# kaist-ina/BWA-MEME

Measured on AMD Instinct MI355X. Metric: seeding_reads_per_sec, higher is better.
Workload: dtype u64; 1 GPU; learned-index seeding (rounds 1-3 + hit gather), 150 bp SE reads vs 3100 Mbp synthetic genome (fwd+rc suffix array of 6200000000 entries), index and reads resident in HBM; genome_bp=3100000000, sa_entries=6200000000, read_len=150, rmi_leaves_log2=28

## Files before the change

bwa-meme_amd/csrc/meme_common.h:

```cpp
#pragma once
#include <hip/hip_runtime.h>
#include <stdint.h>
#include <stdio.h>
#include <string>
#include <type_traits>
#include <utility>
#include <vector>

#include "meme_hip.h"

typedef uint64_t u64;
typedef int64_t i64;

struct __attribute__((aligned(16))) SaEnt {
    u64 key;
    u64 pos;
};

struct RmiRec {
    double icpt;
    double slope;
    u64 err;
};

struct Rmi32 {
    double icpt;
    double slope;
    u64 err;
    u64 pad;
};

struct DevIndex {
    i64 n = 0;
    const SaEnt* sa = nullptr;
    const u64* pac = nullptr;
    const Rmi32* l2 = nullptr;
    const Rmi32* l1 = nullptr;
    i64 n_l2 = 0, n_l1 = 0;
    int shift = 64;
    const uint8_t* plcp = nullptr;
};

template <bool HOST> struct Buf {
    void* p = nullptr;
    size_t cap = 0;
    Buf() = default;
    Buf(const Buf&) = delete; Buf& operator=(const Buf&) = delete;
    ~Buf() { if (p) (void)(HOST ? hipHostFree(p) : hipFree(p)); }
    template <class T> T* as() const { return (T*)p; }
};
typedef Buf<false> DevBuf;
typedef Buf<true> HostBuf;
static_assert(!std::is_copy_constructible<DevBuf>::value && !std::is_copy_assignable<DevBuf>::value && !std::is_copy_constructible<HostBuf>::value &&
              !std::is_copy_assignable<HostBuf>::value, "a workspace owns its memory: a copy would free it twice");
template <int N> struct Events {
    hipEvent_t e[N] = {};
    Events() = default;
    Events(const Events&) = delete; Events& operator=(const Events&) = delete;
    ~Events() { for (hipEvent_t x : e) if (x) (void)hipEventDestroy(x); }
    hipEvent_t& operator[](int i) { return e[i]; }
    hipError_t ensure() { for (hipEvent_t& x : e) if (!x) { const hipError_t r = hipEventCreate(&x); if (r != hipSuccess) return r; } return hipSuccess; }
};
struct Stream {
    hipStream_t s = nullptr;
    Stream() = default;
    Stream(const Stream&) = delete; Stream& operator=(const Stream&) = delete;
    ~Stream() { if (s) (void)hipStreamDestroy(s); }
    operator hipStream_t() const { return s; }
};

struct Carve {
    unsigned char* base;
    size_t bytes = 0;
    explicit Carve(void* b) : base((unsigned char*)b) {}
    template <class T> T* take(size_t count, size_t align = 1) { bytes = (bytes + align - 1) / align * align; T* q = base ? (T*)(base + bytes) : nullptr; bytes += count * sizeof(T); return q; }
    i64* col(i64 n) { return take<i64>((size_t)n + 1); }
};
struct ContigTab {
    i64* off; int* len; unsigned char* alt; size_t bytes;
    ContigTab(void* base, i64 n) { Carve c(base); off = c.take<i64>(n); len = c.take<int>(n); alt = c.take<unsigned char>(n + 64); bytes = c.bytes; }
};
struct ChainCounts {
    i64 *chain_off, *seed_off, *nch, *nsd; int* tree; unsigned char* fb; unsigned long long* route; size_t bytes;
    ChainCounts(void* base, i64 n) { Carve c(base); chain_off = c.col(n); seed_off = c.col(n); nch = c.col(n); nsd = c.col(n); tree = c.take<int>(n); fb = c.take<unsigned char>(n + 64);
                                     route = c.take<unsigned long long>(8, 16); bytes = c.bytes; }
};
struct ChainLists {
    i64 *list[5], *work[5], *woff[5]; unsigned char* cls; size_t bytes;
    ChainLists(void* base, i64 n) { Carve c(base); for (int k = 0; k < 5; ++k) { list[k] = c.col(n); work[k] = c.col(n); woff[k] = c.col(n); } cls = c.take<unsigned char>(n + 64); bytes = c.bytes; }
};
enum { EXT_L = 0, EXT_R = 1, EXT_B = 2 };
struct ExtCounts {
    i64 *cnt[3], *off[3], *cntS, *offS; size_t bytes;
    ExtCounts(void* base, i64 n) { Carve c(base); for (i64*& q : cnt) q = c.col(n); for (i64*& q : off) q = c.col(n); cntS = c.col(n); offS = c.col(n); bytes = c.bytes; }
    bool adjacent(i64 n) const { return off[1] == off[0] + (n + 1) && off[2] == off[1] + (n + 1); }
};
struct CountScan {
    i64 *cnt, *off; size_t bytes;
    CountScan(void* base, i64 n) { Carve c(base); cnt = c.col(n); off = c.col(n); bytes = c.bytes; }
};
struct ExtRetry {
    meme_seqpair* half[2]; size_t bytes;
    ExtRetry(void* base, i64 nmax) { Carve c(base); for (meme_seqpair*& q : half) q = c.take<meme_seqpair>((size_t)nmax + 1); bytes = c.bytes; }
};
struct ExtRounds {
    int4* state; uint8_t* act; uint8_t* sel; size_t bytes;
    ExtRounds(void* base, i64 n, i64 seeds) { Carve c(base); state = c.take<int4>(n + 1); act = c.take<uint8_t>(n + 1); sel = c.take<uint8_t>(seeds + 64); bytes = c.bytes; }
};
struct GcigCols {
    i64 *zsz, *csz, *zoff, *coff, *ncig, *ooff, *msz, *moff, *psz, *poff, *isdp, *dpoff, *dplist, *is16, *o16, *is32, *o32, *is64, *o64, *bad; size_t bytes;
    GcigCols(void* base, i64 n) { Carve c(base); zsz = c.col(n); csz = c.col(n); zoff = c.col(n); coff = c.col(n); ncig = c.col(n); ooff = c.col(n); msz = c.col(n); moff = c.col(n);
        psz = c.col(n); poff = c.col(n); isdp = c.col(n); dpoff = c.col(n); dplist = c.col(n); is16 = c.col(n); o16 = c.col(n); is32 = c.col(n); o32 = c.col(n); is64 = c.col(n);
        o64 = c.col(n); bad = c.take<i64>(8); bytes = c.bytes; }
};
struct BswSort {
    int *hist, *offs, *cursor, *maxq; unsigned int* tickets; size_t bytes;
    BswSort(void* base, int keys) { Carve c(base); hist = c.take<int>(keys); offs = c.take<int>(keys + 1); cursor = c.take<int>(keys); maxq = c.take<int>(1); tickets = c.take<unsigned int>(30); bytes = c.bytes; }
};
struct MateCounts {
    i64 *cntQ, *cntJ, *cntR, *cntY, *offQ, *offJ, *offR, *offY; size_t bytes;
    MateCounts(void* base, i64 n) { Carve c(base); cntQ = c.col(n); cntJ = c.col(n); cntR = c.col(n); cntY = c.col(n); offQ = c.col(n); offJ = c.col(n); offR = c.col(n); offY = c.col(n); bytes = c.bytes; }
};
struct SamCols {
    i64 *bound, *soff, *len, *toff, *bad; size_t bytes;
    SamCols(void* base, i64 n) { Carve c(base); bound = c.col(n); soff = c.col(n); len = c.col(n); toff = c.col(n); bad = c.take<i64>(8); bytes = c.bytes; }
};
struct ResidentBatch {
    DevBuf reads, read_off, packed, smems, hits, smem_off, hit_off;
    i64 last_seed_reads = 0;
    i64 last_seed_max_len = 0;
    i64 packed_reads = 0;
    int packed_geom[3] = {0, 0, 0};
    bool reads_resident = false;
};
enum { SEED_CTR_SLOT = 0, SEED_CTR_SEARCHES = 1, SEED_CTR_OVERFLOW = 2, SEED_CTR_WINDOWS = 3, SEED_CTR_PROF = 4, SEED_CTR_LANE = 12, SEED_CTR_PEND = 13, SEED_CTR_BLK = 14, SEED_CTR_BLK_OUT = 15,
       SEED_CTR_RS_ROUND = 16, SEED_CTR_RS_STAGE = 24, SEED_CTR_RS_NOINTV = 27, SEED_CTR_RS_WALKED = 28, SEED_CTR_RS_NBPROBE = 29, SEED_CTRS = 32 };
constexpr int RESEED_MAX_ROUNDS = SEED_CTR_RS_STAGE - SEED_CTR_RS_ROUND;
enum { SEED_EV_PACK0, SEED_EV_PACK1, SEED_EV_SEARCH0, SEED_EV_SEARCH1, SEED_EV_RESEED0, SEED_EV_GATHER0, SEED_EV_GATHER1, SEED_EVS };
struct SeedWs {
    DevBuf slots[3], ovf[2];
    DevBuf slot_cnt, slot_hits, slot_loc, counters, pend, blk;
    long long reseed_counts[SEED_CTRS - SEED_CTR_RS_ROUND] = {0};
    int reseed_rounds = 0;
    HostBuf h_smems, h_hits, h_smem_off, h_hit_off;
    unsigned long long* counter_set(int cset) { return (unsigned long long*)counters.p + SEED_CTRS * cset; }
    Events<SEED_EVS> ev;
    Stream emit; Events<2> emit_ev;
};
struct ChainWs {
    DevBuf ch1, sd1, hdr, frac, counts, chains, seeds, lists;
    DevBuf wave[5];
    HostBuf h_chain_off, h_chains, h_seed_off, h_seeds, h_tree, h_frac, h_fallback;
    Events<5> ev;
    const i64* chain_off() const { return (const i64*)counts.p; }
    const i64* seed_off(i64 n) const { return ChainCounts(counts.p, n).seed_off; }
};
enum { EXT_CTR_RETRY = 0, EXT_CTR_FLT_JOBS = 2, EXT_CTR_CENSUS = 8, EXT_CTR_HEAVY = 24, EXT_CTR_BYTES = 256 };
struct ExtWs {
    DevBuf rmax, regs, order, counts, pairs_l, pairs_r, retry, seq, counters;
    DevBuf flt_sc, flt_jobs, flt_cnt, flt_seeds, flt_score, flt_hsp;
    DevBuf live_cnt, live_regs, rounds, heavy;
    HostBuf h_reg_off, h_regs; Events<2> ev;
};
struct BswWs { DevBuf pairs, refb, qerb, order, ws, hist; Events<2> ev; };
struct GcigWs {
    DevBuf jobs, cols, z, cig, res, ops, md, nm, md_packed, cjobs, cres; HostBuf h_res, h_ops, h_md; Events<2> ev;
};
struct KswvWs {
    DevBuf jobs, order, ref, qer, res, rowmax, rm_off; HostBuf h_res; Events<2> ev;
};
struct MateWs {
    DevBuf regs, reg_off, counts, gar, aux, batch_off; HostBuf h_gar, h_batch_off, h_jobs;
};
struct SamWs {
    DevBuf names, name_off, quals, recs, blob, cols, scratch, text, contigs; HostBuf h_text_off, h_text; Events<2> ev;
};

struct PrimaryWs {
    DevBuf regs, reg_off, out, n_pri, mapq, status, sorted, rank, list, counter, logtab; HostBuf h_regs, h_n_pri, h_mapq, h_status; Events<2> ev;
    bool log_ready = false;
};

struct PairWs {
    DevBuf regs, reg_off, n_pri, res, status, counter, keys, list, tab; HostBuf h_res, h_status, h_tab; Events<2> ev; Events<1> tab_ev;
    bool tab_in_flight = false;
};

struct FinishWs {
    DevBuf regs, reg_off, out, reg_off_out, ums, status, counters, stage, cnt, live, first, list, cols_l, cols_c;
    HostBuf h_regs, h_reg_off, h_ums, h_status; Events<2> ev;
};

struct ContigCache {
    DevBuf dev; HostBuf host;
    std::vector<meme_contig> from; i64 l_pac = -1;
};

struct SideStreams {
    Stream st[3];
    Events<3> done;
    Events<1> fork;
};

struct meme_ctx {
    int device = 0;
    int n_cus = 256;
    DevIndex idx;
    bool owns_index = false;
    std::vector<std::pair<void*, size_t>> owned;
    void* plcp_aux = nullptr;
    ResidentBatch batch;
    DevBuf scan_tmp;
    ContigCache contigs;
    HostBuf h_ctr;
    ChainWs chain; ExtWs ext; BswWs bsw; GcigWs gcig; KswvWs kswv; MateWs mate; SamWs sam; PrimaryWs primary; PairWs pair; FinishWs finish; SeedWs seed;
    Stream stream;
    SideStreams side;
    i64 seed_blocks = 0;
    i64 helper_blocks = 0;
    i64 smem_cap = 128;
    i64 group_lanes = 4;
    i64 seed_blocks_per_cu = 5;
    i64 max_batch = 0;
    i64 ext_slab_jobs = 8 << 20;
    i64 ext_slab_bytes = (i64)3 << 29;
    i64 ext_split = 1;
    i64 bsw_circ = 1;
    i64 sam_max_batch = 0;
    i64 primary_split = 8;
    i64 primary_blocks = 0;
    i64 pair_split = 8;
    i64 pair_blocks = 0;
    i64 pair_lds_keys = 0;
    i64 finish_blocks = 0;
    i64 finish_lds_recs = 0;
    i64 ext_live_only = 0;
    i64 ext_rounds = 1;
    i64 gcig_groups = 1;
    i64 gcig_zcap = -1;
    i64 ext_census = 0;
    i64 seed_defer = 1;
    i64 chain_light_hits = 32;
    i64 chain_lane_hits = 256;
    i64 chain_wave_tiers = 1;
    i64 sa_chunk = (i64)1 << 28;
    i64 sa_piece = (i64)1 << 28;
    i64 bsw_blocks = 0;
    i64 bsw_lane_min_pairs = 32768;
    bool sa_stats_valid = false;
    long long sa_stats[MEME_SA_STATS] = {0};
    i64 sam_text_reads = 0;
    bool sam_has_quals = false;
    meme_timings tm = {};
};

void meme_set_error(const char* fmt, ...);
int meme_buf_reserve(meme_ctx* ctx, DevBuf& b, size_t bytes);
int meme_side_stream(meme_ctx* ctx, int i);
int meme_hostbuf_reserve(meme_ctx* ctx, HostBuf& b, size_t bytes);
inline unsigned grid_blocks(i64 items, int per, i64 cap = 256 * 64) { i64 b = (items + per - 1) / per; return (unsigned)(b < cap ? (b < 1 ? 1 : b) : cap); }
int meme_contigs(meme_ctx* ctx, const char* prefix, const meme_contig* contigs, int32_t n_contigs, i64 l_pac, ContigTab* out);
int meme_scan_exclusive(meme_ctx* ctx, const i64* d_in, i64* d_out, i64 n);
int meme_scan_total(meme_ctx* ctx, const i64* d_in, i64* d_out, i64 n, i64* h_total);
inline bool meme_fits_free_hbm(size_t need, size_t have, size_t* free_b) { size_t total_b = 0; return need <= have || hipMemGetInfo(free_b, &total_b) != hipSuccess || need <= *free_b / 2 + have; }
int meme_bsw_launch(meme_ctx* ctx, meme_seqpair* d_pairs, const uint8_t* d_ref, const uint8_t* d_qer, int npairs, int w, const meme_bsw_opt* opt,
                    int host_maxq);
hipError_t meme_bsw_last_ms(meme_ctx* ctx, float* ms);
constexpr int MEME_SEEDSW_MAX = 200;
struct meme_seedsw_job { i64 rb; i64 qoff; int seed; short tlen, qlen; };
int meme_seedsw_launch(meme_ctx* ctx, const meme_seedsw_job* d_jobs, const unsigned long long* d_njobs, i64 max_jobs, int* d_sc, const meme_ext_opt* o);
int meme_kswv_run(meme_ctx* ctx, const meme_kswv_job* jobs, int64_t njobs, const uint8_t* ref, int64_t ref_bytes, const uint8_t* qer, int64_t qer_bytes, const meme_bsw_opt* opt,
                  bool staged, meme_kswv_host_result* out);
int meme_chain_reserve(meme_ctx* ctx, i64 n);
int meme_chain_run(meme_ctx* ctx, const meme_contig* contigs, int32_t n_contigs, const meme_chain_opt* opt, i64* totals);

#define HIP_TRY(expr)                                                                          \
    do {                                                                                       \
        hipError_t _e = (expr);                                                                \
        if (_e != hipSuccess) {                                                                \
            meme_set_error("%s failed: %s (%s:%d)", #expr, hipGetErrorString(_e), __FILE__, __LINE__); \
            return MEME_E_HIP;                                                                 \
        }                                                                                      \
    } while (0)

__device__ __forceinline__ u64 load_pos5(const uint8_t* pos5, i64 i) {
    const i64 bo = i * 5;
    const uint32_t* pd = reinterpret_cast<const uint32_t*>(pos5 + (bo & ~3ll));
    const u64 two = (u64)pd[0] | ((u64)pd[1] << 32);
    const u64 v5 = (two >> (8 * (int)(bo & 3))) & 0xffffffffffull;
    return ((v5 & 0xffffffffull) << 8) | (v5 >> 32);
}
__device__ __forceinline__ int text_base(const u64* pac, i64 p) { return (int)(pac[p >> 5] >> (62 - 2 * (int)(p & 31))) & 3; }
__device__ __forceinline__ u64 extract32(const u64* w, i64 s) {
    i64 k = s >> 5;
    int sh = (int)(s & 31) * 2;
    u64 a = w[k], b = w[k + 1];
    return sh ? (a << sh) | (b >> (64 - sh)) : a;
}
```

bwa-meme_amd/csrc/meme_ctx.hip:

```cpp
#include <fcntl.h>
#include <stdarg.h>
#include <stdlib.h>
#include <string.h>
#include <sys/stat.h>
#include <unistd.h>
#include <atomic>
#include <chrono>
#include <functional>
#include <thread>

#include "meme_common.h"

static thread_local char g_err[512] = "";

void meme_set_error(const char* fmt, ...) {
    va_list ap;
    va_start(ap, fmt);
    vsnprintf(g_err, sizeof(g_err), fmt, ap);
    va_end(ap);
}

extern "C" const char* meme_last_error(void) { return g_err; }

int meme_buf_reserve(meme_ctx* ctx, DevBuf& b, size_t bytes) {
    if (bytes <= b.cap) return MEME_OK;
    if (b.p) { HIP_TRY(hipStreamSynchronize(ctx->stream)); HIP_TRY(hipFree(b.p)); b.p = nullptr; b.cap = 0; }
    size_t want = bytes + bytes / 4 + 256;
    HIP_TRY(hipMalloc(&b.p, want));
    b.cap = want;
    return MEME_OK;
}

int meme_side_stream(meme_ctx* ctx, int i) {
    SideStreams& S = ctx->side;
    if (!S.st[i].s) HIP_TRY(hipStreamCreateWithFlags(&S.st[i].s, hipStreamNonBlocking));
    if (!S.done[i]) HIP_TRY(hipEventCreateWithFlags(&S.done[i], hipEventDisableTiming));
    if (!S.fork[0]) HIP_TRY(hipEventCreateWithFlags(&S.fork[0], hipEventDisableTiming));
    return MEME_OK;
}

int meme_hostbuf_reserve(meme_ctx* ctx, HostBuf& b, size_t bytes) {
    if (bytes <= b.cap) return MEME_OK;
    if (b.p) { HIP_TRY(hipStreamSynchronize(ctx->stream)); HIP_TRY(hipHostFree(b.p)); b.p = nullptr; b.cap = 0; }
    size_t want = bytes + bytes / 4 + 4096;
    HIP_TRY(hipHostMalloc(&b.p, want, hipHostMallocDefault));
    b.cap = want;
    return MEME_OK;
}

extern "C" void* meme_host_alloc(int64_t bytes) {
    void* p = nullptr;
    if (bytes <= 0) return nullptr;
    if (hipHostMalloc(&p, (size_t)bytes, hipHostMallocDefault) != hipSuccess) { meme_set_error("hipHostMalloc(%lld) failed", (long long)bytes); return nullptr; }
    return p;
}
extern "C" void meme_host_free(void* p) { if (p) (void)hipHostFree(p); }

extern "C" int meme_device_count(void) {
    int n = 0;
    if (hipGetDeviceCount(&n) != hipSuccess) return 0;
    return n;
}


extern "C" meme_ctx* meme_ctx_create(int device) {
    int n = meme_device_count();
    if (n <= 0) { meme_set_error("no HIP device visible: the MI355X backend has no CPU fallback"); return nullptr; }
    if (device < 0 || device >= n) { meme_set_error("device %d out of range (0..%d)", device, n - 1); return nullptr; }
    if (hipSetDevice(device) != hipSuccess) { meme_set_error("hipSetDevice(%d) failed", device); return nullptr; }
    meme_ctx* ctx = new meme_ctx();
    ctx->device = device;
    { hipDeviceProp_t prop; if (hipGetDeviceProperties(&prop, device) == hipSuccess && prop.multiProcessorCount > 0) ctx->n_cus = prop.multiProcessorCount; }
    if (hipStreamCreateWithFlags(&ctx->stream.s, hipStreamNonBlocking) != hipSuccess) {
        meme_set_error("hipStreamCreate failed");
        delete ctx;
        return nullptr;
    }
    return ctx;
}

extern "C" void meme_ctx_destroy(meme_ctx* ctx) {
    if (!ctx) return;
    (void)hipSetDevice(ctx->device);
    for (hipStream_t st : {ctx->stream.s, ctx->side.st[0].s, ctx->side.st[1].s, ctx->side.st[2].s, ctx->seed.emit.s})
        if (st) (void)hipStreamSynchronize(st);
    if (ctx->owns_index) for (auto& o : ctx->owned) (void)hipFree(o.first);
    if (ctx->plcp_aux) (void)hipFree(ctx->plcp_aux);
    delete ctx;
}

int meme_contigs(meme_ctx* ctx, const char* prefix, const meme_contig* contigs, int32_t n_contigs, i64 l_pac, ContigTab* out) {
    ContigCache& K = ctx->contigs;
    if (K.dev.p && K.l_pac == l_pac && (i64)K.from.size() == n_contigs && (n_contigs == 0 || !memcmp(K.from.data(), contigs, (size_t)n_contigs * sizeof(meme_contig)))) {
        *out = ContigTab(K.dev.p, n_contigs);
        return MEME_OK;
    }
    HIP_TRY(hipStreamSynchronize(ctx->stream));
    K.l_pac = -1;
    for (int i = 0; i < n_contigs; ++i)
        if (contigs[i].len < 1 || contigs[i].offset < 0 || contigs[i].offset + contigs[i].len > l_pac || (i > 0 && contigs[i].offset < contigs[i - 1].offset + contigs[i - 1].len)) {
            meme_set_error("%scontig %d (offset %lld, length %d) is not a valid reference sequence of a %lld-base genome", prefix, i, (long long)contigs[i].offset, contigs[i].len,
                           (long long)l_pac);
            return MEME_E_ARG;
        }
    const size_t bytes = ContigTab(nullptr, n_contigs).bytes;
    int rc;
    if ((rc = meme_buf_reserve(ctx, K.dev, bytes)) || (rc = meme_hostbuf_reserve(ctx, K.host, bytes))) return rc;
    memset(K.host.p, 0, bytes);
    const ContigTab t(K.host.p, n_contigs);
    for (int i = 0; i < n_contigs; ++i) { t.off[i] = contigs[i].offset; t.len[i] = contigs[i].len; t.alt[i] = contigs[i].is_alt ? 1 : 0; }
    HIP_TRY(hipMemcpyAsync(K.dev.p, K.host.p, bytes, hipMemcpyHostToDevice, ctx->stream));
    HIP_TRY(hipStreamSynchronize(ctx->stream));
    K.from.assign(contigs, contigs + n_contigs);
    K.l_pac = l_pac;
    *out = ContigTab(K.dev.p, n_contigs);
    return MEME_OK;
}

extern "C" int meme_ctx_sync(meme_ctx* ctx) {
    if (!ctx) return MEME_E_ARG;
    HIP_TRY(hipStreamSynchronize(ctx->stream));
    return MEME_OK;
}

extern "C" void* meme_ctx_stream(meme_ctx* ctx) { return ctx ? (void*)ctx->stream : nullptr; }

extern "C" int meme_get_timings(meme_ctx* ctx, meme_timings* out) {
    if (!ctx || !out) return MEME_E_ARG;
    *out = ctx->tm;
    return MEME_OK;
}

extern "C" int meme_set_tuning(meme_ctx* ctx, const char* key, int64_t value) {
    if (!ctx || !key) return MEME_E_ARG;
    if (!strcmp(key, "gcig_groups") && value != 0 && value != 1) { meme_set_error("gcig_groups must be 0 or 1"); return MEME_E_ARG; }
    if (!strcmp(key, "group_lanes") && value != 1 && value != 2 && value != 4 && value != 8 && value != 16 && value != 32) { meme_set_error("group_lanes must be 1, 2, 4, 8, 16 or 32"); return MEME_E_ARG; }
    const i64 any = INT64_MIN;
    static const struct { const char* key; i64 meme_ctx::*member; i64 at_least; } keys[] = {
        {"seed_blocks", &meme_ctx::seed_blocks, any}, {"helper_blocks", &meme_ctx::helper_blocks, 0}, {"smem_cap", &meme_ctx::smem_cap, 8}, {"seed_defer", &meme_ctx::seed_defer, any}, {"max_batch", &meme_ctx::max_batch, any},
        {"sam_max_batch", &meme_ctx::sam_max_batch, any}, {"bsw_circ", &meme_ctx::bsw_circ, any}, {"ext_split", &meme_ctx::ext_split, any}, {"ext_slab_jobs", &meme_ctx::ext_slab_jobs, 1},
        {"ext_census", &meme_ctx::ext_census, any}, {"gcig_zcap", &meme_ctx::gcig_zcap, any}, {"gcig_groups", &meme_ctx::gcig_groups, any}, {"ext_live_only", &meme_ctx::ext_live_only, any},
        {"ext_rounds", &meme_ctx::ext_rounds, 0}, {"bsw_blocks", &meme_ctx::bsw_blocks, any}, {"bsw_lane_min_pairs", &meme_ctx::bsw_lane_min_pairs, any},
        {"chain_wave_tiers", &meme_ctx::chain_wave_tiers, any}, {"chain_lane_hits", &meme_ctx::chain_lane_hits, any}, {"chain_light_hits", &meme_ctx::chain_light_hits, any},
        {"group_lanes", &meme_ctx::group_lanes, any}, {"primary_split", &meme_ctx::primary_split, 0}, {"primary_blocks", &meme_ctx::primary_blocks, 0}, {"finish_blocks", &meme_ctx::finish_blocks, 0}, {"pair_split", &meme_ctx::pair_split, 0}, {"pair_blocks", &meme_ctx::pair_blocks, 0}, {"pair_lds_keys", &meme_ctx::pair_lds_keys, 0},
        {"finish_lds_recs", &meme_ctx::finish_lds_recs, 0}, {"seed_blocks_per_cu", &meme_ctx::seed_blocks_per_cu, 1},
        {"sa_chunk", &meme_ctx::sa_chunk, 1}, {"sa_piece", &meme_ctx::sa_piece, 1}};
    for (const auto& k : keys) if (!strcmp(key, k.key)) { ctx->*k.member = value < k.at_least ? k.at_least : value; return MEME_OK; }
    meme_set_error("unknown tuning key %s", key);
    return MEME_E_ARG;
}

extern "C" int meme_index_share(meme_ctx* ctx, meme_ctx* owner);
extern "C" int64_t meme_index_pac64_words(int64_t sa_num) { return ((sa_num + 31) >> 5) + 8; }
extern "C" int64_t meme_index_pos5_bytes(int64_t sa_num) { return sa_num * 5 + 16; }

__global__ void __launch_bounds__(256) k_pack_text(const uint8_t* __restrict__ text, i64 n, u64* __restrict__ pac, i64 words) {
  for (i64 w = (i64)blockIdx.x * blockDim.x + threadIdx.x; w < words; w += (i64)gridDim.x * blockDim.x) {
    i64 base = w << 5;
    u64 v = 0;
    if (base + 32 <= n) {
        const uint4* p = reinterpret_cast<const uint4*>(text + base);
        uint4 a = p[0], b = p[1];
        uint32_t q[8] = {a.x, a.y, a.z, a.w, b.x, b.y, b.z, b.w};
#pragma unroll
        for (int k = 0; k < 8; ++k) {
            uint32_t x = q[k];
            v = (v << 8) | ((u64)(x & 3) << 6) | ((u64)((x >> 8) & 3) << 4) | ((u64)((x >> 16) & 3) << 2) |
                (u64)((x >> 24) & 3);
        }
    } else {
        for (int r = 0; r < 32; ++r) {
            i64 p = base + r;
            u64 c = p < n ? (u64)(text[p] & 3) : 3ull;
            v = (v << 2) | c;
        }
    }
    pac[w] = v;
  }
}

__global__ void __launch_bounds__(256) k_build_entries(const uint8_t* __restrict__ pos_packed, const u64* __restrict__ sa_u64,
                                                        i64 n, const u64* __restrict__ pac, SaEnt* __restrict__ ent) {
  for (i64 i = (i64)blockIdx.x * blockDim.x + threadIdx.x; i < n; i += (i64)gridDim.x * blockDim.x) {
    const u64 pos = sa_u64 ? sa_u64[i] : load_pos5(pos_packed, i);
    SaEnt e;
    e.key = extract32(pac, (i64)pos);
    e.pos = pos;
    ent[i] = e;
  }
}

__global__ void __launch_bounds__(256) k_pos5_from_sa(const u64* __restrict__ sa, i64 n, uint8_t* __restrict__ pos5) {
  for (i64 i = (i64)blockIdx.x * blockDim.x + threadIdx.x; i < n; i += (i64)gridDim.x * blockDim.x) {
    const u64 pos = sa[i];
    uint8_t* p = pos5 + i * 5;
    const uint32_t hi = (uint32_t)(pos >> 8);
    p[0] = (uint8_t)hi; p[1] = (uint8_t)(hi >> 8); p[2] = (uint8_t)(hi >> 16); p[3] = (uint8_t)(hi >> 24); p[4] = (uint8_t)(pos & 0xff);
  }
}

__global__ void __launch_bounds__(256) k_rmi32(const RmiRec* __restrict__ in, i64 n, Rmi32* __restrict__ out) {
  for (i64 i = (i64)blockIdx.x * blockDim.x + threadIdx.x; i < n; i += (i64)gridDim.x * blockDim.x) {
    const RmiRec r = in[i];
    Rmi32 o;
    o.icpt = r.icpt; o.slope = r.slope; o.err = r.err; o.pad = 0;
    out[i] = o;
  }
}

__device__ __forceinline__ int pair_lcp(const SaEnt a, const SaEnt b, i64 n, const u64* __restrict__ pac) {
    i64 lim = n - (i64)(a.pos > b.pos ? a.pos : b.pos);
    if (lim > 255) lim = 255;
    const u64 x = a.key ^ b.key;
    int l = x ? (__clzll((long long)x) >> 1) : 32;
    if (!x) {
        for (int m = 1; l < lim; ++m) {
            const u64 y = extract32(pac, (i64)a.pos + 32 * m) ^ extract32(pac, (i64)b.pos + 32 * m);
            if (y) { l += __clzll((long long)y) >> 1; break; }
            l += 32;
        }
    }
    return l < (int)lim ? l : (int)lim;
}

__global__ void __launch_bounds__(256) k_build_plcp(const SaEnt* __restrict__ ent, i64 n, const u64* __restrict__ pac, uint8_t* __restrict__ plcp) {
    __shared__ int sl[257];
    for (i64 b0 = (i64)blockIdx.x * 256; b0 < n; b0 += (i64)gridDim.x * 256) {
        const i64 i = b0 + threadIdx.x;
        SaEnt e; e.key = 0; e.pos = 0;
        int ln = 0;
        if (i < n) {
            e = ent[i];
            if (i + 1 < n) ln = pair_lcp(e, ent[i + 1], n, pac);
        }
        sl[threadIdx.x + 1] = ln;
        if (threadIdx.x == 0) sl[0] = b0 > 0 ? pair_lcp(ent[b0 - 1], e, n, pac) : 0;
        __syncthreads();
        if (i < n) {
            const int a = sl[threadIdx.x], b = sl[threadIdx.x + 1];
            plcp[e.pos] = (uint8_t)(a > b ? a : b);
        }
        __syncthreads();
    }
}

extern "C" int meme_stage_build_plcp(meme_ctx* ctx, const void* d_sa_ent, int64_t n, const void* d_pac64, void* d_plcp) {
    if (!ctx || !d_sa_ent || !d_pac64 || !d_plcp || n <= 0) return MEME_E_ARG;
    HIP_TRY(hipSetDevice(ctx->device));
    hipLaunchKernelGGL(k_build_plcp, dim3(grid_blocks(n, 256)), dim3(256), 0, ctx->stream, (const SaEnt*)d_sa_ent, (i64)n, (const u64*)d_pac64,
                       (uint8_t*)d_plcp);
    HIP_TRY(hipGetLastError());
    return MEME_OK;
}

extern "C" int meme_stage_pack_text(meme_ctx* ctx, const uint8_t* d_text, int64_t n, void* d_pac64) {
    if (!ctx || !d_text || !d_pac64 || n <= 0) return MEME_E_ARG;
    HIP_TRY(hipSetDevice(ctx->device));
    i64 words = meme_index_pac64_words(n);
    hipLaunchKernelGGL(k_pack_text, dim3(grid_blocks(words, 256)), dim3(256), 0, ctx->stream, d_text, n,
                       (u64*)d_pac64, words);
    HIP_TRY(hipGetLastError());
    return MEME_OK;
}

extern "C" int meme_stage_build_entries(meme_ctx* ctx, const uint8_t* d_pos_packed, int64_t n, const void* d_pac64,
                                        void* d_sa_ent) {
    if (!ctx || !d_pos_packed || !d_pac64 || !d_sa_ent || n <= 0) return MEME_E_ARG;
    HIP_TRY(hipSetDevice(ctx->device));
    hipLaunchKernelGGL(k_build_entries, dim3(grid_blocks(n, 256)), dim3(256), 0, ctx->stream, d_pos_packed,
                       (const u64*)nullptr, (i64)n, (const u64*)d_pac64, (SaEnt*)d_sa_ent);
    HIP_TRY(hipGetLastError());
    return MEME_OK;
}

extern "C" int meme_stage_entries_from_sa(meme_ctx* ctx, const uint64_t* d_sa, int64_t n, const void* d_pac64,
                                          void* d_sa_ent) {
    if (!ctx || !d_sa || !d_pac64 || !d_sa_ent || n <= 0) return MEME_E_ARG;
    HIP_TRY(hipSetDevice(ctx->device));
    hipLaunchKernelGGL(k_build_entries, dim3(grid_blocks(n, 256)), dim3(256), 0, ctx->stream,
                       (const uint8_t*)nullptr, (const u64*)d_sa, (i64)n, (const u64*)d_pac64, (SaEnt*)d_sa_ent);
    HIP_TRY(hipGetLastError());
    return MEME_OK;
}

extern "C" int meme_stage_pos5_from_sa(meme_ctx* ctx, const uint64_t* d_sa, int64_t n, void* d_pos5) {
    if (!ctx || !d_sa || !d_pos5 || n <= 0) return MEME_E_ARG;
    HIP_TRY(hipSetDevice(ctx->device));
    hipLaunchKernelGGL(k_pos5_from_sa, dim3(grid_blocks(n, 256)), dim3(256), 0, ctx->stream, (const u64*)d_sa, (i64)n, (uint8_t*)d_pos5);
    HIP_TRY(hipGetLastError());
    return MEME_OK;
}

// ... 308 lines not shown
```

bwa-meme_amd/csrc/meme_seed.hip:

```cpp
#include <limits.h>
#include <stdlib.h>
#include <string.h>
#include <utility>

#include "meme_seed_kernel.h"

namespace {

using namespace seedk;

constexpr int SCAN_BLOCK = 256;
constexpr int SCAN_ITEMS = 4;
constexpr int SCAN_TILE = SCAN_BLOCK * SCAN_ITEMS;

__device__ __forceinline__ i64 block_scan_excl(i64 v, i64* total) {
    __shared__ i64 wsum[SCAN_BLOCK / 64];
    const int lane = threadIdx.x & 63, wid = threadIdx.x >> 6;
    i64 x = v;
#pragma unroll
    for (int d = 1; d < 64; d <<= 1) {
        i64 y = __shfl_up(x, d);
        if (lane >= d) x += y;
    }
    if (lane == 63) wsum[wid] = x;
    __syncthreads();
    i64 off = 0, tot = 0;
    for (int w = 0; w < SCAN_BLOCK / 64; ++w) {
        if (w < wid) off += wsum[w];
        tot += wsum[w];
    }
    __syncthreads();
    *total = tot;
    return off + x - v;
}

__global__ void __launch_bounds__(SCAN_BLOCK) k_tile_sums(const int* __restrict__ cnt, const i64* __restrict__ hits, i64 n,
                                                          i64 ntiles, i64* __restrict__ tile_sums) {
  for (i64 tile = blockIdx.x; tile < ntiles; tile += gridDim.x) {
    i64 base = tile * SCAN_TILE + threadIdx.x * SCAN_ITEMS;
    i64 a = 0, b = 0;
    for (int k = 0; k < SCAN_ITEMS; ++k) {
        i64 i = base + k;
        if (i < n) {
            int c = cnt[i];
            a += c < 0 ? 0 : c;
            b += hits[i];
        }
    }
    i64 ta, tb;
    block_scan_excl(a, &ta);
    block_scan_excl(b, &tb);
    if (threadIdx.x == 0) { tile_sums[2 * tile] = ta; tile_sums[2 * tile + 1] = tb; }
  }
}

__global__ void __launch_bounds__(SCAN_BLOCK) k_scan_tiles(i64* __restrict__ tile_sums, i64 ntiles, i64* __restrict__ totals) {
    i64 ca = 0, cb = 0;
    for (i64 base = 0; base < ntiles; base += SCAN_BLOCK) {
        i64 i = base + threadIdx.x;
        i64 a = i < ntiles ? tile_sums[2 * i] : 0, b = i < ntiles ? tile_sums[2 * i + 1] : 0;
        i64 ta, tb;
        i64 ea = block_scan_excl(a, &ta);
        i64 eb = block_scan_excl(b, &tb);
        if (i < ntiles) { tile_sums[2 * i] = ca + ea; tile_sums[2 * i + 1] = cb + eb; }
        ca += ta;
        cb += tb;
    }
    if (threadIdx.x == 0) { totals[0] = ca; totals[1] = cb; }
}

__global__ void __launch_bounds__(SCAN_BLOCK) k_offsets(const int* __restrict__ cnt, const i64* __restrict__ hits, i64 n,
                                                        i64 ntiles, const i64* __restrict__ tile_sums, i64* __restrict__ smem_off,
                                                        i64* __restrict__ hit_off) {
  for (i64 tile = blockIdx.x; tile < ntiles; tile += gridDim.x) {
    i64 base = tile * SCAN_TILE + threadIdx.x * SCAN_ITEMS;
    i64 va[SCAN_ITEMS], vb[SCAN_ITEMS], a = 0, b = 0;
    for (int k = 0; k < SCAN_ITEMS; ++k) {
        i64 i = base + k;
        va[k] = vb[k] = 0;
        if (i < n) {
            int c = cnt[i];
            va[k] = c < 0 ? 0 : c;
            vb[k] = hits[i];
        }
        a += va[k];
        b += vb[k];
    }
    i64 ta, tb;
    i64 ea = block_scan_excl(a, &ta) + tile_sums[2 * tile];
    i64 eb = block_scan_excl(b, &tb) + tile_sums[2 * tile + 1];
    for (int k = 0; k < SCAN_ITEMS; ++k) {
        i64 i = base + k;
        if (i < n) { smem_off[i] = ea; hit_off[i] = eb; }
        ea += va[k];
        eb += vb[k];
    }
    if (tile == ntiles - 1 && threadIdx.x == SCAN_BLOCK - 1) { smem_off[n] = ea; hit_off[n] = eb; }
  }
}

struct TierTable {
    const SlotRec* base[N_TIERS];
    int cap[N_TIERS];
};

__global__ void __launch_bounds__(BLOCK) k_gather(const SaEnt* __restrict__ sa, TierTable tiers, const i64* __restrict__ slot_loc,
                                                   const int* __restrict__ cnt, i64 n, int hits_per_smem,
                                                   const i64* __restrict__ smem_off, const i64* __restrict__ hit_off,
                                                   meme_mem_tl* __restrict__ smems, u64* __restrict__ hits) {
    constexpr int GL = 16;
    const int lane = threadIdx.x & 63;
    const int t = lane & (GL - 1);
    const int gbase = lane - t;
    i64 gid = ((i64)blockIdx.x * BLOCK + threadIdx.x) / GL;
    const i64 ngroups = (i64)gridDim.x * BLOCK / GL;
    for (i64 r = gid; r < n; r += ngroups) {
        const int c = cnt[r];
        if (c <= 0) continue;
        const i64 loc = slot_loc[r];
        const int tier = (int)(loc >> 40);
        const SlotRec* sl = tiers.base[tier] + (loc & ((1ll << 40) - 1)) * tiers.cap[tier];
        meme_mem_tl* out = smems + smem_off[r];
        u64* hout = hits + hit_off[r];
        i64 hb0 = 0;
        for (int k0 = 0; k0 < c; k0 += GL) {
            const int k = k0 + t;
            const bool act = k < c;
            SlotRec s;
            s.start = s.end = 0; s.sa_start = 0; s.count = 0;
            if (act) s = sl[k];
            i64 h = s.count;
            if (hits_per_smem > 0 && h > hits_per_smem) h = hits_per_smem;
            i64 incl = h;
#pragma unroll
            for (int d = 1; d < GL; d <<= 1) {
                i64 y = __shfl_up(incl, d, GL);
                if (t >= d) incl += y;
            }
            const i64 hb = hb0 + incl - h;
            u64 first = 0;
            if (act) {
                first = (s.sa_start & SLOT_POS) ? (u64)(s.sa_start & SLOT_VAL) : sa[s.sa_start].pos;
                meme_mem_tl m;
                m.start = s.start;
                m.end = s.end;
                m.hitbeg = (int32_t)hb;
                m.hitcount = s.count > (i64)INT_MAX ? INT_MAX : (int32_t)s.count;
                m.cache_refpos = first;
                out[k] = m;
                if (h > 0) hout[hb] = first;
                for (i64 i = 1; i < h && i < 4; ++i) hout[hb + i] = sa[s.sa_start + i].pos;
            }
            u64 longmask = (__ballot(act && h > 4) >> gbase) & 0xffffull;
            while (longmask) {
                const int src = __ffsll((long long)longmask) - 1;
                longmask &= longmask - 1;
                const i64 lh = __shfl(h, src, GL), lhb = __shfl(hb, src, GL), lsa = __shfl(s.sa_start, src, GL);
                for (i64 i = 4 + t; i < lh; i += GL) hout[lhb + i] = sa[lsa + i].pos;
            }
            hb0 += __shfl(incl, GL - 1, GL);
        }
    }
}

template <int G>
int launch_k_seed(hipStream_t stream, const SeedArgs& A, size_t lds, i64 blocks) {
    if (lds > 64 * 1024)
        HIP_TRY(hipFuncSetAttribute((const void*)k_seed<G>, hipFuncAttributeMaxDynamicSharedMemorySize, (int)lds));
    hipLaunchKernelGGL(k_seed<G>, dim3((unsigned)blocks), dim3(BLOCK), lds, stream, A);
    HIP_TRY(hipGetLastError());
    return MEME_OK;
}

struct SeedRun {
    meme_ctx* ctx;
    const i64* d_read_off; i64 nreads;
    const meme_seed_opt* opt;
    PackGeom geo;
    TierTable tiers = {};
    bool defer = false;
    i64 n_early = -1;
    i64 n_todo = 0;
    float ms_total = 0.f, ms_reseed = 0.f;
    i64 launches = 0, searches = 0, windows = 0, lane_searches = 0;
    unsigned long long h_early[SEED_CTRS];
};

i64 helper_grid(const meme_ctx* ctx, i64 blocks) {
    if (ctx->helper_blocks > 0 && blocks > ctx->helper_blocks) blocks = ctx->helper_blocks;
    return blocks < 1 ? 1 : blocks;
}
template <typename K>
int resident_grid(const meme_ctx* ctx, K kernel, int threads, i64* blocks) {
    int per_cu = 0;
    HIP_TRY(hipOccupancyMaxActiveBlocksPerMultiprocessor(&per_cu, kernel, threads, 0));
    *blocks = (i64)ctx->n_cus * (per_cu < 1 ? 1 : per_cu);
    return MEME_OK;
}

int seed_pack(SeedRun& R, const uint8_t* d_reads, i64 max_len, i64 total_bytes) {
    meme_ctx* ctx = R.ctx;
    if (max_len > MAX_READ_LEN) {
        meme_set_error("read of %lld bases exceeds the learned-index limit of %d (LEARNED_MAX_READ_LEN)", (long long)max_len, MAX_READ_LEN);
        return MEME_E_ARG;
    }
    if (max_len < 1) max_len = 1;
    PackGeom& geo = R.geo;
    geo.W = (int)((max_len + 31) / 32) + 2;
    geo.MW = (int)((max_len + 63) / 64);
    geo.stride = 2 * geo.W + 2 * geo.MW + 1;
    int rc;
    if ((rc = meme_buf_reserve(ctx, ctx->batch.packed, (size_t)R.nreads * geo.stride * 8))) return rc;
    HIP_TRY(hipEventRecord(ctx->seed.ev[SEED_EV_PACK0], ctx->stream));
    const int rw = pack_chunk_reads(max_len);
    const i64 nchunks = (R.nreads + rw - 1) / rw;
    i64 pblocks = (nchunks + 3) / 4, pmax = 0;
    if ((rc = resident_grid(ctx, k_pack_reads, 256, &pmax))) return rc;
    pblocks = helper_grid(ctx, pblocks > pmax ? pmax : pblocks);
    hipLaunchKernelGGL(k_pack_reads, dim3((unsigned)pblocks), dim3(256), 0, ctx->stream, d_reads,
                       R.d_read_off, R.nreads, total_bytes, geo, rw, (u64*)ctx->batch.packed.p);
    HIP_TRY(hipGetLastError());
    HIP_TRY(hipEventRecord(ctx->seed.ev[SEED_EV_PACK1], ctx->stream));
    ctx->batch.packed_reads = R.nreads;
    ctx->batch.packed_geom[0] = geo.W; ctx->batch.packed_geom[1] = geo.MW; ctx->batch.packed_geom[2] = geo.stride;
    return MEME_OK;
}

int launch_tier(SeedRun& R, int tier, i64 n_todo, const i64* pending, int cset, hipStream_t stream, bool defer) {
    meme_ctx* ctx = R.ctx;
    int G = tier == 0 ? (int)ctx->group_lanes : 32;
    const int cap = tier == 0 ? (int)ctx->smem_cap : TIER_CAP[tier];
    const int lcap = cap < TIER_LCAP[tier] ? cap : TIER_LCAP[tier];
    DevBuf& sb = ctx->seed.slots[tier];
    DevBuf& ob = ctx->seed.ovf[tier & 1];
    const size_t need = (size_t)n_todo * cap * sizeof(SlotRec);
    if (tier > 0 && need > sb.cap) {
        size_t free_b = 0;
        if (!meme_fits_free_hbm(need, 0, &free_b)) {
            meme_set_error("%lld reads emitted more than %d SMEMs each: re-running them needs %.1f GB of slots, more than half of the "
                           "free HBM (%.1f GB); seed this batch in smaller pieces", (long long)n_todo, R.tiers.cap[tier - 1],
                           need / 1e9, free_b / 1e9);
            return MEME_E_CAPACITY;
        }
    }
    int rc;
    if ((rc = meme_buf_reserve(ctx, sb, need))) return rc;
    if ((rc = meme_buf_reserve(ctx, ob, (size_t)n_todo * sizeof(i64)))) return rc;
    unsigned long long* counters = ctx->seed.counter_set(cset);
    HIP_TRY(hipMemsetAsync(counters, 0, SEED_CTRS * sizeof(unsigned long long), stream));
    SeedArgs A;
    A.I = ctx->idx;
    A.packed = (const u64*)ctx->batch.packed.p;
    A.read_off = R.d_read_off;
    A.nreads = n_todo;
    A.geo = R.geo;
    A.opt = *R.opt;
    A.slots = (SlotRec*)sb.p;
    A.slot_cnt = (int*)ctx->seed.slot_cnt.p;
    A.slot_hits = (i64*)ctx->seed.slot_hits.p;
    A.slot_loc = (i64*)ctx->seed.slot_loc.p;
    A.pending = pending;
    A.ovf_list = (i64*)ob.p;
    A.cap = cap;
    A.lcap = lcap;
    A.tier = tier;
    A.counters = counters;
    A.defer = defer ? 1 : 0;
    R.tiers.base[tier] = (const SlotRec*)sb.p;
    R.tiers.cap[tier] = cap;
    while (G < 32 && seed_lds_bytes(G, R.geo, lcap) > (size_t)160 * 1024) G *= 2;
    const int groups = BLOCK / G;
    size_t lds = seed_lds_bytes(G, R.geo, lcap);
    i64 want = (n_todo + groups - 1) / groups;
    i64 blocks = ctx->seed_blocks > 0 ? ctx->seed_blocks : (i64)ctx->n_cus * ctx->seed_blocks_per_cu;
    if (blocks > want) blocks = want;
    if (blocks < 1) blocks = 1;
    if (tier == 0) HIP_TRY(hipEventRecord(ctx->seed.ev[SEED_EV_SEARCH0], stream));
    switch (G) {
    case 1: return launch_k_seed<1>(stream, A, lds, blocks);
    case 2: return launch_k_seed<2>(stream, A, lds, blocks);
    case 4: return launch_k_seed<4>(stream, A, lds, blocks);
    case 8: return launch_k_seed<8>(stream, A, lds, blocks);
    case 16: return launch_k_seed<16>(stream, A, lds, blocks);
    case 32: return launch_k_seed<32>(stream, A, lds, blocks);
    default: meme_set_error("group_lanes must be 1, 2, 4, 8, 16 or 32"); return MEME_E_ARG;
    }
}

int fetch_counters(SeedRun& R, int cset, unsigned long long* h, int nsets = 1) {
    HIP_TRY(hipMemcpyAsync(h, R.ctx->seed.counter_set(cset), (size_t)nsets * SEED_CTRS * sizeof(unsigned long long), hipMemcpyDeviceToHost, R.ctx->stream));
    HIP_TRY(hipStreamSynchronize(R.ctx->stream));
    return MEME_OK;
}
void tally(SeedRun& R, const unsigned long long* h) {
    ++R.launches;
    R.searches += (i64)h[SEED_CTR_SEARCHES];
    R.windows += (i64)h[SEED_CTR_WINDOWS];
    R.n_todo = (i64)h[SEED_CTR_OVERFLOW];
#ifdef SEED_PROF
    {
        double tot = 0; for (int k = 0; k < 8; ++k) tot += (double)h[SEED_CTR_PROF + k];
        fprintf(stderr, "[seed prof]:");
        const char* nm[6] = {"control", "request+rmi", "window+compare", "resolve", "level", "apply"};
        for (int k = 0; k < 6; ++k) fprintf(stderr, " %s %.1f%%", nm[k], 100.0 * (double)h[SEED_CTR_PROF + k] / (tot > 0 ? tot : 1));
        fprintf(stderr, "\n");
    }
#endif
}

#ifndef RESEED_ROUNDS
#define RESEED_ROUNDS 5
#endif
#ifndef RESEED_EMIT_BESIDE
#define RESEED_EMIT_BESIDE 1
#endif
int launch_reseed(SeedRun& R) {
    meme_ctx* ctx = R.ctx;
    SeedWs& S = ctx->seed;
    const i64 nreads = R.nreads;
    HIP_TRY(hipEventRecord(S.ev[SEED_EV_RESEED0], ctx->stream));
    ReseedArgs A;
    A.I = ctx->idx; A.packed = (const u64*)ctx->batch.packed.p; A.geo = R.geo; A.nreads = nreads; A.opt = *R.opt;
    A.slots = (SlotRec*)S.slots[0].p; A.cap = (int)ctx->smem_cap; A.slot_cnt = (int*)S.slot_cnt.p; A.slot_hits = (i64*)S.slot_hits.p;
    A.ovf_list = (i64*)S.ovf[0].p; A.counters = S.counter_set(0); A.pend_list = (i64*)S.pend.p;
    A.blk = (BlkRec*)S.blk.p; A.blk_out = A.blk + nreads * BLK_PER_READ; A.blk_cap = nreads * BLK_PER_READ;
    A.blk_ctr = SEED_CTR_BLK; A.blk_out_ctr = SEED_CTR_BLK_OUT;
    A.read_off = R.d_read_off; A.round = 0;
    i64 rblocks = (nreads + 255) / 256;
    if (rblocks > (i64)ctx->n_cus * 32) rblocks = (i64)ctx->n_cus * 32;
    hipLaunchKernelGGL(k_reseed, dim3((unsigned)rblocks), dim3(256), 0, ctx->stream, A);
    HIP_TRY(hipEventRecord(ctx->side.fork[0], ctx->stream));
    const unsigned sblocks = (unsigned)(rblocks < (i64)ctx->n_cus * 4 ? rblocks : (i64)ctx->n_cus * 4);
    if (!S.emit.s) HIP_TRY(hipStreamCreateWithFlags(&S.emit.s, hipStreamNonBlocking));
    for (int i = 0; i < 2; ++i) if (!S.emit_ev[i]) HIP_TRY(hipEventCreateWithFlags(&S.emit_ev[i], hipEventDisableTiming));
    if (RESEED_EMIT_BESIDE) {
        HIP_TRY(hipEventRecord(S.emit_ev[0], ctx->stream));
        HIP_TRY(hipStreamWaitEvent(S.emit, S.emit_ev[0], 0));
        hipLaunchKernelGGL(k_reseed_emit, dim3(sblocks), dim3(256), 0, S.emit, A);
        HIP_TRY(hipEventRecord(S.emit_ev[1], S.emit));
    }
    constexpr int ROUNDS = RESEED_ROUNDS;
    static_assert(ROUNDS >= 1 && ROUNDS <= RESEED_MAX_ROUNDS, "one counter per round");
    S.reseed_rounds = ROUNDS;
    for (int round = 0; round < ROUNDS; ++round) {
        A.round = round;
        hipLaunchKernelGGL(k_reseed_search, dim3(sblocks), dim3(256), 0, ctx->stream, A);
        if (round < ROUNDS - 1) {
            hipLaunchKernelGGL(k_reseed_resume<false>, dim3(sblocks), dim3(256), 0, ctx->stream, A);
            HIP_TRY(hipMemsetAsync(S.counter_set(0) + A.blk_ctr, 0, sizeof(unsigned long long), ctx->stream));
            std::swap(A.blk, A.blk_out); std::swap(A.blk_ctr, A.blk_out_ctr);
        } else hipLaunchKernelGGL(k_reseed_resume<true>, dim3(sblocks), dim3(256), 0, ctx->stream, A);
    }
    if (!RESEED_EMIT_BESIDE) {
        hipLaunchKernelGGL(k_reseed_emit, dim3(sblocks), dim3(256), 0, ctx->stream, A);
        HIP_TRY(hipEventRecord(S.emit_ev[1], ctx->stream));
    }
    HIP_TRY(hipGetLastError());
    return MEME_OK;
}

int launch_early_overflow(SeedRun& R) {
    meme_ctx* ctx = R.ctx;
    Stream& side = ctx->side.st[0];
    unsigned long long h_ovf = 0;
    HIP_TRY(hipStreamWaitEvent(side, ctx->side.fork[0], 0));
    HIP_TRY(hipMemcpyAsync(&h_ovf, ctx->seed.counter_set(0) + SEED_CTR_OVERFLOW, 8, hipMemcpyDeviceToHost, side));
    HIP_TRY(hipStreamSynchronize(side));
    if (h_ovf == 0) return MEME_OK;
    R.n_early = (i64)h_ovf;
    int rc;
    if ((rc = launch_tier(R, 1, R.n_early, (const i64*)ctx->seed.ovf[0].p, 1, side, false))) return rc;
    HIP_TRY(hipEventRecord(ctx->side.done[0], side));
    HIP_TRY(hipStreamWaitEvent(ctx->stream, ctx->side.done[0], 0));
    return MEME_OK;
}

int seed_tier0(SeedRun& R) {
    meme_ctx* ctx = R.ctx;
    SeedWs& S = ctx->seed;
    int rc;
    R.defer = ctx->seed_defer != 0 && ctx->idx.plcp != nullptr && R.opt->rounds >= 2;
    S.reseed_rounds = 0;
    if (R.defer && (rc = meme_buf_reserve(ctx, S.pend, (size_t)R.nreads * sizeof(i64)))) return rc;
    if (R.defer && (rc = meme_buf_reserve(ctx, S.blk, (size_t)R.nreads * BLK_PER_READ * 2 * sizeof(BlkRec)))) return rc;
    if ((rc = launch_tier(R, 0, R.nreads, nullptr, 0, ctx->stream, R.defer))) return rc;
    if (R.defer) {
        if ((rc = meme_side_stream(ctx, 0)) || (rc = launch_reseed(R)) || (rc = launch_early_overflow(R))) return rc;
        HIP_TRY(hipStreamWaitEvent(ctx->stream, S.emit_ev[1], 0));
    }
    HIP_TRY(hipEventRecord(S.ev[SEED_EV_SEARCH1], ctx->stream));
    unsigned long long h[2 * SEED_CTRS];
    if ((rc = fetch_counters(R, 0, h, R.n_early >= 0 ? 2 : 1))) return rc;
    if (R.n_early >= 0) memcpy(R.h_early, h + SEED_CTRS, sizeof(R.h_early));
    float ms = 0.f;
    HIP_TRY(hipEventElapsedTime(&ms, S.ev[SEED_EV_SEARCH0], S.ev[SEED_EV_SEARCH1]));
    R.ms_total += ms;
    if (R.defer) {
        float a = 0.f;
        HIP_TRY(hipEventElapsedTime(&a, S.ev[SEED_EV_RESEED0], S.ev[SEED_EV_SEARCH1]));
        R.ms_reseed += a;
        R.lane_searches += (i64)h[SEED_CTR_LANE];
        for (int k = SEED_CTR_RS_ROUND; k < SEED_CTRS; ++k) S.reseed_counts[k - SEED_CTR_RS_ROUND] = (long long)h[k];
#ifdef RESEED_PROF
        {
            const unsigned long long* c = h + SEED_CTR_PROF;
            fprintf(stderr, "[reseed prof] lists per round:");
            for (int k = 0; k < S.reseed_rounds; ++k) fprintf(stderr, " %llu", h[SEED_CTR_RS_ROUND + k]);
            fprintf(stderr, "\n[reseed prof] stage searches partition_probes run_probes\n");
            for (int k = 0; k < 3; ++k) fprintf(stderr, "[reseed prof] %d %llu %llu %llu\n", k, h[SEED_CTR_RS_STAGE + k], c[k], c[3 + k]);
            fprintf(stderr, "[reseed prof] interval read %llu, without interval %llu, walked %llu, neighbour probes %llu, last-pass searches %llu\n", c[6],
                    h[SEED_CTR_RS_NOINTV], h[SEED_CTR_RS_WALKED], h[SEED_CTR_RS_NBPROBE], h[SEED_CTR_LANE]);
        }
#endif
        if (getenv("MEME_SEED_TRACE")) fprintf(stderr, "[meme] seed tier 0: search kernel + re-seeding kernels %.2f ms, of which behind k_seed %.2f ms (%lld lane searches; %lld reads of the "
                                               "overflow tier beside them)\n", ms, a, (long long)h[SEED_CTR_LANE], (long long)(R.n_early < 0 ? 0 : R.n_early));
    }
    tally(R, h);
    return MEME_OK;
}

int seed_overflow_tiers(SeedRun& R) {
    meme_ctx* ctx = R.ctx;
    SeedWs& S = ctx->seed;
    int rc;
    unsigned long long h[SEED_CTRS];
    for (int tier = 1; R.n_todo > 0; ++tier) {
        if (tier >= N_TIERS) {
            meme_set_error("a read produced more than %d SMEMs", TIER_CAP[N_TIERS - 1]);
            return MEME_E_CAPACITY;
        }
        const int cset = tier & 1;
        if (tier == 1 && R.n_early == R.n_todo) {
            memcpy(h, R.h_early, sizeof(h));
        } else {
            HIP_TRY(hipEventRecord(S.ev[SEED_EV_SEARCH0], ctx->stream));
            if ((rc = launch_tier(R, tier, R.n_todo, (const i64*)S.ovf[(tier - 1) & 1].p, cset, ctx->stream, false))) return rc;
            HIP_TRY(hipEventRecord(S.ev[SEED_EV_SEARCH1], ctx->stream));
            if ((rc = fetch_counters(R, cset, h))) return rc;
            float ms = 0.f;
            HIP_TRY(hipEventElapsedTime(&ms, S.ev[SEED_EV_SEARCH0], S.ev[SEED_EV_SEARCH1]));
            R.ms_total += ms;
        }
        tally(R, h);
    }
    return MEME_OK;
}

int seed_gather(SeedRun& R, meme_seed_result* out) {
    meme_ctx* ctx = R.ctx;
    SeedWs& S = ctx->seed;
    ResidentBatch& B = ctx->batch;
    const i64 nreads = R.nreads;
    int rc;
    i64 ntiles = (nreads + SCAN_TILE - 1) / SCAN_TILE;
    if ((rc = meme_buf_reserve(ctx, ctx->scan_tmp, (size_t)(2 * ntiles + 2) * sizeof(i64)))) return rc;
    if ((rc = meme_buf_reserve(ctx, B.smem_off, (size_t)(nreads + 1) * sizeof(i64)))) return rc;
    if ((rc = meme_buf_reserve(ctx, B.hit_off, (size_t)(nreads + 1) * sizeof(i64)))) return rc;
    i64* tiles = (i64*)ctx->scan_tmp.p;
    i64* totals = tiles + 2 * ntiles;
    HIP_TRY(hipEventRecord(S.ev[SEED_EV_GATHER0], ctx->stream));
    const i64 sblocks = helper_grid(ctx, ntiles);
    hipLaunchKernelGGL(k_tile_sums, dim3((unsigned)sblocks), dim3(SCAN_BLOCK), 0, ctx->stream, (const int*)S.slot_cnt.p,
                       (const i64*)S.slot_hits.p, nreads, ntiles, tiles);
    hipLaunchKernelGGL(k_scan_tiles, dim3(1), dim3(SCAN_BLOCK), 0, ctx->stream, tiles, ntiles, totals);
    hipLaunchKernelGGL(k_offsets, dim3((unsigned)sblocks), dim3(SCAN_BLOCK), 0, ctx->stream, (const int*)S.slot_cnt.p,
                       (const i64*)S.slot_hits.p, nreads, ntiles, (const i64*)tiles, (i64*)B.smem_off.p, (i64*)B.hit_off.p);
    HIP_TRY(hipGetLastError());
    i64 h_tot[2];
    HIP_TRY(hipMemcpyAsync(h_tot, totals, sizeof(h_tot), hipMemcpyDeviceToHost, ctx->stream));
    HIP_TRY(hipStreamSynchronize(ctx->stream));
    if ((rc = meme_buf_reserve(ctx, B.smems, (size_t)(h_tot[0] + 1) * sizeof(meme_mem_tl)))) return rc;
    if ((rc = meme_buf_reserve(ctx, B.hits, (size_t)(h_tot[1] + 1) * sizeof(u64)))) return rc;
    i64 gblocks = (nreads + 15) / 16;
    if (gblocks > (i64)ctx->n_cus * 8) gblocks = (i64)ctx->n_cus * 8;
    gblocks = helper_grid(ctx, gblocks);
    hipLaunchKernelGGL(k_gather, dim3((unsigned)gblocks), dim3(BLOCK), 0, ctx->stream, ctx->idx.sa, R.tiers,
                       (const i64*)S.slot_loc.p, (const int*)S.slot_cnt.p, nreads, R.opt->hits_per_smem,
                       (const i64*)B.smem_off.p, (const i64*)B.hit_off.p, (meme_mem_tl*)B.smems.p, (u64*)B.hits.p);
    HIP_TRY(hipGetLastError());
    HIP_TRY(hipEventRecord(S.ev[SEED_EV_GATHER1], ctx->stream));
    HIP_TRY(hipStreamSynchronize(ctx->stream));
    HIP_TRY(hipEventElapsedTime(&ctx->tm.seed_gather_ms, S.ev[SEED_EV_GATHER0], S.ev[SEED_EV_GATHER1]));
    out->d_smems = (const meme_mem_tl*)B.smems.p;
    out->d_smem_off = (const i64*)B.smem_off.p;
    out->d_hits = (const u64*)B.hits.p;
    out->d_hit_off = (const i64*)B.hit_off.p;
    out->total_smems = h_tot[0];
    out->total_hits = h_tot[1];
    out->searches = R.searches;
    return MEME_OK;
}

int launch_seed(meme_ctx* ctx, const uint8_t* d_reads, const i64* d_read_off, i64 nreads, i64 max_len, i64 total_bytes,
                const meme_seed_opt* opt, meme_seed_result* out) {
    int rc;
    SeedWs& S = ctx->seed;
    ctx->batch.last_seed_reads = 0;
    ctx->sam_text_reads = 0;
    if ((rc = meme_buf_reserve(ctx, S.slot_cnt, (size_t)nreads * sizeof(int)))) return rc;
    if ((rc = meme_buf_reserve(ctx, S.slot_hits, (size_t)nreads * sizeof(i64)))) return rc;
    if ((rc = meme_buf_reserve(ctx, S.slot_loc, (size_t)nreads * sizeof(i64)))) return rc;
    if ((rc = meme_buf_reserve(ctx, S.counters, 2 * SEED_CTRS * sizeof(unsigned long long)))) return rc;
    HIP_TRY(S.ev.ensure());
    SeedRun R;
    R.ctx = ctx; R.d_read_off = d_read_off; R.nreads = nreads; R.opt = opt;
    if ((rc = seed_pack(R, d_reads, max_len, total_bytes)) || (rc = seed_tier0(R)) || (rc = seed_overflow_tiers(R))) return rc;
    HIP_TRY(hipEventElapsedTime(&ctx->tm.seed_pack_ms, S.ev[SEED_EV_PACK0], S.ev[SEED_EV_PACK1]));
    ctx->tm.seed_kernel_ms = R.ms_total;
    ctx->tm.seed_launches = R.launches;
    ctx->tm.seed_windows = R.windows;
    ctx->tm.seed_reseed_ms = R.ms_reseed;
    ctx->tm.seed_lane_searches = R.lane_searches;
    return seed_gather(R, out);
}

__global__ void __launch_bounds__(256) k_max_len(const i64* __restrict__ off, i64 n, int* out) {
    __shared__ int wmax[4];
    int v = 0;
    for (i64 i = (i64)blockIdx.x * blockDim.x + threadIdx.x; i < n; i += (i64)gridDim.x * blockDim.x) {
        int l = (int)(off[i + 1] - off[i]);
        v = v > l ? v : l;
    }
    for (int d = 32; d >= 1; d >>= 1) { int y = __shfl_xor(v, d); v = v > y ? v : y; }
    if ((threadIdx.x & 63) == 0) wmax[threadIdx.x >> 6] = v;
    __syncthreads();
    if (threadIdx.x == 0) {
        for (int k = 1; k < 4; ++k) v = v > wmax[k] ? v : wmax[k];
        atomicMax(out, v);
    }
}

int device_max_len(meme_ctx* ctx, const i64* d_read_off, i64 nreads, i64* max_len) {
    int rc;
    if ((rc = meme_buf_reserve(ctx, ctx->scan_tmp, 64))) return rc;
    HIP_TRY(hipMemsetAsync(ctx->scan_tmp.p, 0, 4, ctx->stream));
    i64 mblocks = (nreads + 255) / 256;
    if (mblocks > 1024) mblocks = 1024;
    hipLaunchKernelGGL(k_max_len, dim3((unsigned)mblocks), dim3(256), 0, ctx->stream, d_read_off, nreads,
                       (int*)ctx->scan_tmp.p);
    int v = 0;
    HIP_TRY(hipMemcpyAsync(&v, ctx->scan_tmp.p, 4, hipMemcpyDeviceToHost, ctx->stream));
    HIP_TRY(hipStreamSynchronize(ctx->stream));
    *max_len = v;
    return MEME_OK;
}

int check_opt(const meme_seed_opt* opt) {
    if (!opt || opt->min_seed_len < 1 || opt->rounds < 1 || opt->rounds > 3 || opt->hits_per_smem < 0) {
        meme_set_error("bad meme_seed_opt");
        return MEME_E_ARG;
    }
    return MEME_OK;
}

}

extern "C" int meme_seed_batch_device(meme_ctx* ctx, const uint8_t* d_reads, const int64_t* d_read_off, int64_t nreads,
                                      int64_t total_bases, const meme_seed_opt* opt, meme_seed_result* out) {
    if (!ctx || !d_reads || !d_read_off || !out || nreads < 0) return MEME_E_ARG;
    int rc = check_opt(opt);
    if (rc) return rc;
    if (!ctx->idx.sa) { meme_set_error("meme_seed_batch: no index loaded"); return MEME_E_STATE; }
    HIP_TRY(hipSetDevice(ctx->device));
    if (nreads == 0) { memset(out, 0, sizeof(*out)); return MEME_OK; }
    i64 max_len = 0;
    if ((rc = device_max_len(ctx, (const i64*)d_read_off, nreads, &max_len))) return rc;
    return launch_seed(ctx, d_reads, (const i64*)d_read_off, nreads, max_len, total_bases, opt, out);
}

extern "C" int meme_seed_batch(meme_ctx* ctx, const uint8_t* reads, const int64_t* read_off, int64_t nreads,
                               const meme_seed_opt* opt, meme_mem_tl* smems, int64_t smem_capacity, int64_t* smem_off,
                               uint64_t* hits, int64_t hit_capacity, int64_t* hit_off, int64_t* total_smems,
                               int64_t* total_hits) {
    if (!ctx || !reads || !read_off || !smems || !smem_off || !hits || !hit_off || nreads < 0) return MEME_E_ARG;
    int rc = check_opt(opt);
    if (rc) return rc;
    if (!ctx->idx.sa) { meme_set_error("meme_seed_batch: no index loaded"); return MEME_E_STATE; }
    HIP_TRY(hipSetDevice(ctx->device));
    if (nreads == 0) { smem_off[0] = 0; hit_off[0] = 0; if (total_smems) *total_smems = 0; if (total_hits) *total_hits = 0; return MEME_OK; }
    const i64 bases = read_off[nreads] - read_off[0];
    if (read_off[0] != 0) { meme_set_error("read_off[0] must be 0"); return MEME_E_ARG; }
    if ((rc = meme_buf_reserve(ctx, ctx->batch.reads, (size_t)bases + 16))) return rc;
    if ((rc = meme_buf_reserve(ctx, ctx->batch.read_off, (size_t)(nreads + 1) * sizeof(i64)))) return rc;
    HIP_TRY(hipMemcpyAsync(ctx->batch.reads.p, reads, (size_t)bases, hipMemcpyHostToDevice, ctx->stream));
    HIP_TRY(hipMemcpyAsync(ctx->batch.read_off.p, read_off, (size_t)(nreads + 1) * sizeof(i64), hipMemcpyHostToDevice, ctx->stream));
    meme_seed_result res;
    i64 max_len = 0;
    for (i64 i = 0; i < nreads; ++i) max_len = read_off[i + 1] - read_off[i] > max_len ? read_off[i + 1] - read_off[i] : max_len;
    rc = launch_seed(ctx, (const uint8_t*)ctx->batch.reads.p, (const i64*)ctx->batch.read_off.p, nreads, max_len, bases, opt, &res);
    if (rc) return rc;
    if (total_smems) *total_smems = res.total_smems;
    if (total_hits) *total_hits = res.total_hits;
    HIP_TRY(hipMemcpyAsync(smem_off, res.d_smem_off, (size_t)(nreads + 1) * sizeof(i64), hipMemcpyDeviceToHost, ctx->stream));
    HIP_TRY(hipMemcpyAsync(hit_off, res.d_hit_off, (size_t)(nreads + 1) * sizeof(i64), hipMemcpyDeviceToHost, ctx->stream));
    if (res.total_smems > smem_capacity || res.total_hits > hit_capacity) {
        HIP_TRY(hipStreamSynchronize(ctx->stream));
        meme_set_error("output buffers too small: need %lld SMEMs and %lld hits", (long long)res.total_smems,
                       (long long)res.total_hits);
        return MEME_E_CAPACITY;
    }
    HIP_TRY(hipMemcpyAsync(smems, res.d_smems, (size_t)res.total_smems * sizeof(meme_mem_tl), hipMemcpyDeviceToHost, ctx->stream));
    HIP_TRY(hipMemcpyAsync(hits, res.d_hits, (size_t)res.total_hits * sizeof(u64), hipMemcpyDeviceToHost, ctx->stream));
    HIP_TRY(hipStreamSynchronize(ctx->stream));
    return MEME_OK;
}

extern "C" int meme_debug_packed_reads(meme_ctx* ctx, uint64_t* out, int64_t capacity_words, int32_t* geom, int64_t* nreads) {
    if (!ctx || !geom || !nreads) return MEME_E_ARG;
    const ResidentBatch& B = ctx->batch;
    if (B.packed_reads <= 0 || !B.packed.p) { meme_set_error("meme_debug_packed_reads: no batch was packed on this ctx"); return MEME_E_STATE; }
    for (int k = 0; k < 3; ++k) geom[k] = B.packed_geom[k];
    *nreads = B.packed_reads;
    if (!out) return MEME_OK;
    const i64 words = B.packed_reads * B.packed_geom[2];
    if (capacity_words < words) { meme_set_error("meme_debug_packed_reads: %lld words needed", (long long)words); return MEME_E_CAPACITY; }
    HIP_TRY(hipSetDevice(ctx->device));
    HIP_TRY(hipMemcpyAsync(out, B.packed.p, (size_t)words * 8, hipMemcpyDeviceToHost, ctx->stream));
    HIP_TRY(hipStreamSynchronize(ctx->stream));
    return MEME_OK;
}

extern "C" int meme_debug_reseed_counts(meme_ctx* ctx, int64_t* out, int32_t capacity, int32_t* rounds) {
    if (!ctx || !out || !rounds) return MEME_E_ARG;
    const SeedWs& S = ctx->seed;
    if (S.reseed_rounds <= 0) { meme_set_error("meme_debug_reseed_counts: the last seeding call on this ctx ran no re-seeding kernels"); return MEME_E_STATE; }
    if (capacity < MEME_RESEED_COUNTS) { meme_set_error("meme_debug_reseed_counts: %d values needed", MEME_RESEED_COUNTS); return MEME_E_CAPACITY; }
    static_assert(MEME_RESEED_COUNTS == RESEED_MAX_ROUNDS + 6 && SEED_CTR_RS_NBPROBE - SEED_CTR_RS_ROUND + 1 == MEME_RESEED_COUNTS, "layout of meme_hip.h");
    for (int k = 0; k < MEME_RESEED_COUNTS; ++k) out[k] = S.reseed_counts[k];
    *rounds = S.reseed_rounds;
    return MEME_OK;
}

extern "C" int meme_seed_reserve(meme_ctx* ctx, int64_t nreads, int64_t total_bases) {
    if (!ctx || nreads < 0 || total_bases < 0) return MEME_E_ARG;
    if (nreads == 0) return MEME_OK;
    HIP_TRY(hipSetDevice(ctx->device));
    const size_t n = (size_t)nreads;
    const i64 len = total_bases / nreads + 32;
    const size_t stride = (size_t)(2 * ((len + 31) / 32 + 2) + 2 * ((len + 63) / 64) + 1);
    int rc;
    ResidentBatch& B = ctx->batch; SeedWs& S = ctx->seed;
    ChainWs& C = ctx->chain; ExtWs& E = ctx->ext;
    struct { DevBuf* b; size_t bytes; } dev[] = {
        {&B.reads, (size_t)total_bases + 16}, {&B.read_off, (n + 1) * 8}, {&S.slot_cnt, n * 4}, {&S.slot_hits, n * 8},
        {&S.slot_loc, n * 8}, {&S.counters, 2 * SEED_CTRS * 8}, {&S.pend, n * 8}, {&S.blk, n * BLK_PER_READ * 2 * sizeof(BlkRec)}, {&B.packed, n * stride * 8}, {&S.slots[0], n * (size_t)ctx->smem_cap * sizeof(SlotRec)},
        {&B.smem_off, (n + 1) * 8}, {&B.hit_off, (n + 1) * 8}, {&B.smems, n * 12 * sizeof(meme_mem_tl)}, {&B.hits, n * 24 * 8},
        {&C.chains, n * 3 * sizeof(meme_chain)}, {&C.seeds, n * 6 * sizeof(meme_chain_seed)}};
    for (auto& d : dev) if ((rc = meme_buf_reserve(ctx, *d.b, d.bytes))) return rc;
    if ((rc = meme_chain_reserve(ctx, nreads))) return rc;
    struct { HostBuf* b; size_t bytes; } host[] = {
        {&S.h_smem_off, (n + 1) * 8}, {&S.h_hit_off, (n + 1) * 8}, {&S.h_smems, n * 12 * sizeof(meme_mem_tl)}, {&S.h_hits, n * 24 * 8},
        {&C.h_chain_off, (n + 1) * 8}, {&C.h_chains, n * 3 * sizeof(meme_chain)}, {&C.h_seed_off, (n + 1) * 8},
        {&C.h_seeds, n * 6 * sizeof(meme_chain_seed)}, {&C.h_tree, n * 4}, {&C.h_frac, n * 4}, {&C.h_fallback, n}};
    for (auto& h : host) if ((rc = meme_hostbuf_reserve(ctx, *h.b, h.bytes))) return rc;
    struct { DevBuf* b; size_t bytes; } dev2[] = {
        {&E.rmax, n * 3 * 16}, {&E.regs, n * 4 * sizeof(meme_alnreg)}, {&E.order, n * 4 * 4}, {&E.counts, ExtCounts(nullptr, nreads).bytes},
        {&E.pairs_l, n * 2 * sizeof(meme_seqpair)}, {&E.pairs_r, n * 2 * sizeof(meme_seqpair)}, {&E.retry, n * 4 * sizeof(meme_seqpair)},
        {&E.seq, n * 4 * 250}};
    for (auto& d : dev2) if ((rc = meme_buf_reserve(ctx, *d.b, d.bytes))) return rc;
    if ((rc = meme_hostbuf_reserve(ctx, E.h_reg_off, (n + 1) * 8)) || (rc = meme_hostbuf_reserve(ctx, E.h_regs, n * 4 * sizeof(meme_alnreg))) ||
        (rc = meme_hostbuf_reserve(ctx, ctx->gcig.h_res, n / 2 * sizeof(meme_gres))) || (rc = meme_hostbuf_reserve(ctx, ctx->gcig.h_ops, n * 4))) return rc;
    return MEME_OK;
}

__global__ void __launch_bounds__(256) k_ascii_to_codes(uint4* __restrict__ p, i64 nvec) {
    for (i64 i = (i64)blockIdx.x * blockDim.x + threadIdx.x; i < nvec; i += (i64)gridDim.x * blockDim.x) {
        uint4 v = p[i];
        uint32_t w[4] = {v.x, v.y, v.z, v.w};
#pragma unroll
        for (int k = 0; k < 4; ++k) {
            uint32_t o = 0;
#pragma unroll
            for (int b = 0; b < 4; ++b) {
                const uint32_t c = (w[k] >> (8 * b)) & 0xffu, u = c & 0xdfu;
                const uint32_t code = c < 4 ? c : (u == 'A' ? 0u : u == 'C' ? 1u : u == 'G' ? 2u : u == 'T' ? 3u : 4u);
                o |= code << (8 * b);
            }
            w[k] = o;
        }
        v.x = w[0]; v.y = w[1]; v.z = w[2]; v.w = w[3];
        p[i] = v;
    }
}

static int seed_host_reads(meme_ctx* ctx, const uint8_t* reads, const int64_t* read_off, int64_t nreads, const meme_seed_opt* opt, const char* who,
                           meme_seed_host_result* out, int64_t* totals, bool ascii = false) {
    if (!ctx || !reads || !read_off || nreads < 0) return MEME_E_ARG;
    int rc = check_opt(opt);
    if (rc) return rc;
    if (!ctx->idx.sa) { meme_set_error("%s: no index loaded", who); return MEME_E_STATE; }
    HIP_TRY(hipSetDevice(ctx->device));
    if (out) {
        memset(out, 0, sizeof(*out));
        if ((rc = meme_hostbuf_reserve(ctx, ctx->seed.h_smem_off, (size_t)(nreads + 1) * sizeof(i64)))) return rc;
        if ((rc = meme_hostbuf_reserve(ctx, ctx->seed.h_hit_off, (size_t)(nreads + 1) * sizeof(i64)))) return rc;
        out->smem_off = (const int64_t*)ctx->seed.h_smem_off.p;
        out->hit_off = (const int64_t*)ctx->seed.h_hit_off.p;
    }
    if (totals) totals[0] = totals[1] = 0;
    ctx->batch.last_seed_reads = 0;
    if (nreads == 0) { if (out) { ((i64*)ctx->seed.h_smem_off.p)[0] = 0; ((i64*)ctx->seed.h_hit_off.p)[0] = 0; } return MEME_OK; }
    if (read_off[0] != 0) { meme_set_error("read_off[0] must be 0"); return MEME_E_ARG; }
    const i64 bases = read_off[nreads];
    if ((rc = meme_buf_reserve(ctx, ctx->batch.reads, (size_t)bases + 16))) return rc;
    if ((rc = meme_buf_reserve(ctx, ctx->batch.read_off, (size_t)(nreads + 1) * sizeof(i64)))) return rc;
    HIP_TRY(hipMemcpyAsync(ctx->batch.reads.p, reads, (size_t)bases, hipMemcpyHostToDevice, ctx->stream));
    HIP_TRY(hipMemcpyAsync(ctx->batch.read_off.p, read_off, (size_t)(nreads + 1) * sizeof(i64), hipMemcpyHostToDevice, ctx->stream));
    if (ascii) {
        const i64 nvec = (bases + 15) / 16;
        i64 cb = (nvec + 255) / 256;
        if (cb > (i64)ctx->n_cus * 16) cb = (i64)ctx->n_cus * 16;
        hipLaunchKernelGGL(k_ascii_to_codes, dim3((unsigned)(cb < 1 ? 1 : cb)), dim3(256), 0, ctx->stream, (uint4*)ctx->batch.reads.p, nvec);
        HIP_TRY(hipGetLastError());
    }
    i64 max_len = 0;
    for (i64 i = 0; i < nreads; ++i) max_len = read_off[i + 1] - read_off[i] > max_len ? read_off[i + 1] - read_off[i] : max_len;
    meme_seed_result res;
    rc = launch_seed(ctx, (const uint8_t*)ctx->batch.reads.p, (const i64*)ctx->batch.read_off.p, nreads, max_len, bases, opt, &res);
    if (rc) return rc;
    if (out) {
        if ((rc = meme_hostbuf_reserve(ctx, ctx->seed.h_smems, (size_t)(res.total_smems + 1) * sizeof(meme_mem_tl)))) return rc;
        if ((rc = meme_hostbuf_reserve(ctx, ctx->seed.h_hits, (size_t)(res.total_hits + 1) * sizeof(u64)))) return rc;
        HIP_TRY(hipMemcpyAsync(ctx->seed.h_smem_off.p, res.d_smem_off, (size_t)(nreads + 1) * sizeof(i64), hipMemcpyDeviceToHost, ctx->stream));
        HIP_TRY(hipMemcpyAsync(ctx->seed.h_hit_off.p, res.d_hit_off, (size_t)(nreads + 1) * sizeof(i64), hipMemcpyDeviceToHost, ctx->stream));
        HIP_TRY(hipMemcpyAsync(ctx->seed.h_smems.p, res.d_smems, (size_t)res.total_smems * sizeof(meme_mem_tl), hipMemcpyDeviceToHost, ctx->stream));
        HIP_TRY(hipMemcpyAsync(ctx->seed.h_hits.p, res.d_hits, (size_t)res.total_hits * sizeof(u64), hipMemcpyDeviceToHost, ctx->stream));
        out->smems = (const meme_mem_tl*)ctx->seed.h_smems.p;
        out->hits = (const uint64_t*)ctx->seed.h_hits.p;
        out->total_smems = res.total_smems;
        out->total_hits = res.total_hits;
    }
    HIP_TRY(hipStreamSynchronize(ctx->stream));
    if (totals) { totals[0] = res.total_smems; totals[1] = res.total_hits; }
    ctx->batch.last_seed_reads = nreads;
    ctx->batch.reads_resident = true;
    ctx->batch.last_seed_max_len = max_len;
    return MEME_OK;
}

extern "C" int meme_seed_batch_host(meme_ctx* ctx, const uint8_t* reads, const int64_t* read_off, int64_t nreads,
                                    const meme_seed_opt* opt, meme_seed_host_result* out) {
    if (!out) return MEME_E_ARG;
    return seed_host_reads(ctx, reads, read_off, nreads, opt, "meme_seed_batch_host", out, nullptr);
}

extern "C" int meme_seed_batch_resident(meme_ctx* ctx, const uint8_t* reads, const int64_t* read_off, int64_t nreads,
                                        const meme_seed_opt* opt, int64_t* total_smems, int64_t* total_hits) {
    int64_t tot[2] = {0, 0};
    const int rc = seed_host_reads(ctx, reads, read_off, nreads, opt, "meme_seed_batch_resident", nullptr, tot);
    if (total_smems) *total_smems = tot[0];
    if (total_hits) *total_hits = tot[1];
    return rc;
}

extern "C" int meme_seed_batch_resident_ascii(meme_ctx* ctx, const uint8_t* reads, const int64_t* read_off, int64_t nreads,
                                              const meme_seed_opt* opt, int64_t* total_smems, int64_t* total_hits) {
    int64_t tot[2] = {0, 0};
    const int rc = seed_host_reads(ctx, reads, read_off, nreads, opt, "meme_seed_batch_resident_ascii", nullptr, tot, true);
    if (total_smems) *total_smems = tot[0];
    if (total_hits) *total_hits = tot[1];
    return rc;
}
```

bwa-meme_amd/csrc/meme_seed_kernel.h:

```cpp
#pragma once
#include <limits.h>

#include "meme_common.h"

namespace seedk {

constexpr int BLOCK = 256;
constexpr int MAX_READ_LEN = 500;

struct SlotRec {
    int32_t start, end;
    i64 sa_start;
    i64 count;
};
constexpr i64 SLOT_POS = 1ll << 62;
constexpr i64 SLOT_DEFER = 1ll << 61;
constexpr i64 SLOT_PEND = 1ll << 59;
constexpr i64 SLOT_VAL = (1ll << 48) - 1;
constexpr int DEFER_MAX_K = 64;


constexpr int N_TIERS = 3;
constexpr int TIER_CAP[N_TIERS] = {64, 2048, 65536};
#ifndef LCAP0
#define LCAP0 16
#endif
constexpr int TIER_LCAP[N_TIERS] = {LCAP0, 512, 512};

struct PackGeom {
    int W;
    int MW;
    int stride;
};

struct SeedArgs {
    DevIndex I;
    const u64* packed;
    const i64* read_off;
    i64 nreads;
    PackGeom geo;
    meme_seed_opt opt;
    SlotRec* slots;
    int* slot_cnt;
    i64* slot_hits;
    i64* slot_loc;
    const i64* pending;
    i64* ovf_list;
    int cap, lcap, tier;
    unsigned long long* counters;
    int defer;
};

constexpr int PACK_CAP = 5120;
constexpr int PACK_IT = PACK_CAP / (64 * 16);
constexpr int PACK_MAX_RW = 32;
constexpr int PACK_FWC = 0, PACK_RCC = PACK_CAP / 16 + 2, PACK_NM = 2 * PACK_RCC, PACK_FLAG = PACK_NM + PACK_CAP / 32 + 2;
constexpr int PACK_SLICE = PACK_FLAG + PACK_MAX_RW;
inline int pack_chunk_reads(i64 max_len) {
    i64 rw = (PACK_CAP - 16) / (max_len < 1 ? 1 : max_len);
    return (int)(rw > PACK_MAX_RW ? PACK_MAX_RW : (rw < 1 ? 1 : rw));
}

__device__ __forceinline__ void pack_wave_sync() {
    __builtin_amdgcn_fence(__ATOMIC_RELEASE, "wavefront");
    __builtin_amdgcn_wave_barrier();
    __builtin_amdgcn_fence(__ATOMIC_ACQUIRE, "wavefront");
}

__device__ __forceinline__ void pack_dword(uint32_t a, uint32_t& fw, uint32_t& rc, uint32_t& nm) {
    const uint32_t e = ((((a & 0xFCFCFCFCu) >> 2) + 0x3F3F3F3Fu) >> 6) & 0x01010101u;
    const uint32_t keep = 0x03030303u & ~(e * 3u);
    const uint32_t c = a & keep;
    fw = (fw << 8) | ((c * 0x40100401u) >> 24);
    rc = (rc << 8) | (((c ^ 0x03030303u) & keep) * 0x40100401u >> 24);
    nm = (nm << 4) | ((e * 0x08040201u) >> 24);
}

__global__ void __launch_bounds__(256) k_pack_reads(const uint8_t* __restrict__ reads, const i64* __restrict__ read_off,
                                                     i64 nreads, i64 total_bytes, PackGeom g, int rw,
                                                     u64* __restrict__ out) {
    __shared__ uint32_t pk_lds[4 * PACK_SLICE];
    const int lane = threadIdx.x & 63;
    uint32_t* S = pk_lds + (threadIdx.x >> 6) * PACK_SLICE;
    unsigned short* S16 = reinterpret_cast<unsigned short*>(S + PACK_NM);
    const int stride = g.stride, nw = stride - 1;
    const int k0 = lane % stride, rr0 = lane / stride, dk = 64 % stride, drr = 64 / stride;
    const int mis = (int)(reinterpret_cast<uintptr_t>(reads) & 15);
    const i64 nchunks = (nreads + rw - 1) / rw, nwaves = (i64)gridDim.x * 4;
    i64 ch = (i64)blockIdx.x * 4 + (threadIdx.x >> 6);
    i64 off_next = 0;
    if (ch < nchunks && ch * rw + lane <= nreads && lane <= rw) off_next = read_off[ch * rw + lane];
    for (; ch < nchunks; ch += nwaves) {
        const i64 r0 = ch * rw;
        const int nr = (int)(nreads - r0 < rw ? nreads - r0 : rw);
        const i64 off_l = off_next;
        {
            const i64 rn = (ch + nwaves) * rw + lane;
            if (ch + nwaves < nchunks && rn <= nreads && lane <= rw) off_next = read_off[rn];
        }
        const i64 b0 = __shfl(off_l, 0), b1 = __shfl(off_l, nr);
        const i64 a0 = ((b0 + mis) & ~15ll) - mis;
        const int rel = (int)(off_l - a0);
        const i64 span = b1 - a0;
        uint4 v[PACK_IT];
#pragma unroll
        for (int it = 0; it < PACK_IT; ++it) {
            const i64 p = a0 + 16 * (it * 64 + lane);
            v[it] = make_uint4(0, 0, 0, 0);
            if (16 * (it * 64 + lane) < span) {
                if (p >= 0 && p + 16 <= total_bytes) v[it] = *reinterpret_cast<const uint4*>(reads + p);
                else {
                    uint32_t q[4] = {0, 0, 0, 0};
                    for (int bb = 0; bb < 16; ++bb)
                        if (p + bb >= 0 && p + bb < total_bytes) q[bb >> 2] |= (uint32_t)reads[p + bb] << (8 * (bb & 3));
                    v[it] = make_uint4(q[0], q[1], q[2], q[3]);
                }
            }
        }
        pack_wave_sync();
        if (lane < PACK_MAX_RW) S[PACK_FLAG + lane] = 0;
#pragma unroll
        for (int it = 0; it < PACK_IT; ++it) {
            const int i = it * 64 + lane;
            if (16 * i < span) {
                uint32_t fw = 0, rc = 0, nm = 0;
                pack_dword(v[it].x, fw, rc, nm);
                pack_dword(v[it].y, fw, rc, nm);
                pack_dword(v[it].z, fw, rc, nm);
                pack_dword(v[it].w, fw, rc, nm);
                S[PACK_FWC + i] = fw;
                S[PACK_RCC + i] = rc;
                S16[i ^ 1] = (unsigned short)nm;
            }
        }
        pack_wave_sync();
        u64* o64 = out + r0 * stride;
        const int nwords = nr * stride;
        int rr = rr0, k = k0;
        for (int wk = lane; wk - lane < nwords; wk += 64) {
            const bool in = wk < nwords;
            const int rs = in ? rr : 0;
            const int o = __shfl(rel, rs), e = __shfl(rel, rs + 1);
            const int len = e - o;
            const int lenx = (len > MAX_READ_LEN || e > PACK_CAP) ? 0 : len;
            const bool code = k < 2 * g.W;
            const int kk = code ? k : k - 2 * g.W, per = code ? g.W : g.MW;
            const bool second = kk >= per;
            const int w = second ? kk - per : kk;
            const int span_b = code ? 32 : 64;
            int nvalid = lenx - span_b * w;
            if (nvalid > span_b) nvalid = span_b;
            if (nvalid < 0 || k == nw) nvalid = 0;
            int s0 = second ? lenx - span_b * w - span_b : span_b * w;
            if (s0 < 0 || nvalid == 0) s0 = 0;
            const int bit = (nvalid == 0 ? 0 : o + s0) << (code ? 1 : 0);
            const int idx = (code ? (second ? PACK_RCC : PACK_FWC) : PACK_NM) + (bit >> 5);
            const unsigned sh = (unsigned)bit & 31u;
            const uint32_t d0 = S[idx], d1 = S[idx + 1], d2 = S[idx + 2];
            u64 u = ((u64)__funnelshift_l(d1, d0, sh) << 32) | __funnelshift_l(d2, d1, sh);
            if (code == second) u = __brevll(u);
            if (code) { if (second) u = ((u >> 1) & 0x5555555555555555ull) | ((u & 0x5555555555555555ull) << 1); }
            const int cut = (span_b - nvalid) << (code ? 1 : 0);
            u64 val;
            if (code) val = second ? u << (cut & 63) : u & (~0ull << (cut & 63));
            else val = second ? u >> (cut & 63) : u & (~0ull >> (cut & 63));
            if (nvalid == 0) val = 0;
            if (in && !code && !second && val != 0) S[PACK_FLAG + rs] = 1;
            pack_wave_sync();
            if (k == nw) val = (u64)(unsigned)len | (S[PACK_FLAG + rs] ? (1ull << 31) : 0ull);
            if (in) o64[wk] = val;
            rr += drr; k += dk;
            if (k >= stride) { k -= stride; ++rr; }
        }
    }
}

enum Pc : int {
    PC_FETCH, PC_ALLPOS_TOP, PC_ZZ_TOP, PC_ZZ_RIGHT, PC_ZZ_END, PC_AFTER_STEP1, PC_R2_LOOP, PC_R2_AFTER, PC_R3_INIT,
    PC_R3_TOP, PC_DONE, PC_EXIT
};
enum Kind : int { K_S1_RIGHT, K_ZZ_LEFT, K_ZZ_RIGHT, K_OP_MEM, K_OP_SMEM, K_R3 };
enum Phase : int { PH_CTRL, PH_PART, PH_EDGE_DN, PH_EDGE_UP };

#ifndef CMP_WORDS
#define CMP_WORDS 2
#endif
typedef const __attribute__((address_space(3))) u64* lds_u64;
typedef __attribute__((address_space(3))) int* lds_int;
typedef __attribute__((address_space(3))) unsigned short* lds_u16;
typedef const __attribute__((address_space(1))) u64* glb_u64;
typedef const __attribute__((address_space(1))) SaEnt* glb_ent;
typedef const __attribute__((address_space(1))) Rmi32* glb_rmi;

#ifndef SEED_QUERY_LDS
#define SEED_QUERY_LDS 1
#endif
#ifndef SEED_USE_ERR
#define SEED_USE_ERR 1
#endif
#ifndef SEED_ALIGN_WIN
#define SEED_ALIGN_WIN 0
#endif
#if SEED_QUERY_LDS
typedef lds_u64 q_u64;
#else
typedef const __attribute__((address_space(1))) u64* q_u64;
#endif

__device__ __forceinline__ u64 ext_l(q_u64 w, int s) {
    int k = s >> 5, sh = (s & 31) * 2;
    u64 a = w[k], b = w[k + 1];
    return sh ? (a << sh) | (b >> (64 - sh)) : a;
}

constexpr int PLCP_WIN = 64;
typedef const __attribute__((address_space(3))) uint8_t* lds_u8;
__device__ __forceinline__ i64 plcp_win_fwd(i64 T0, int mid) { const i64 a = T0 + mid - 24; return (a < 0 ? 0 : a) & ~15ll; }
__device__ __forceinline__ i64 plcp_win_rev(i64 T0, int mid, i64 n) { const i64 a = n - 1 - (T0 + mid + 24); return (a < 0 ? 0 : a) & ~15ll; }

__device__ __forceinline__ u64 lowmask(int k) { return k >= 64 ? ~0ull : (k <= 0 ? 0ull : ((1ull << k) - 1ull)); }

enum StIdx : int { ST_BEFORE, ST_AFTER, ST_R2_K, ST_R2_NEXT, ST_R2_SAVED, ST_ZZ_NEXT, ST_ZZ_SP, ST_ZZ_GUARD, ST_AP_GUARD,
                   ST_SM_BASE, ST_N_SMEMS, ST_HITS_LO, ST_HITS_HI, ST_SEARCHES, ST_FLAGS, ST_LAST_CNT_LO, ST_LAST_CNT_HI,
                   ST_LAST_S_LO, ST_LAST_S_HI, ST_WINDOWS,
                   ST_L, ST_SE_LO, ST_SE_HI, ST_EE_LO, ST_EE_HI, ST_NB_LO, ST_NB_HI, ST_LF, ST_CB_LO, ST_CB_HI,
                   ST_TICKET_LO, ST_TICKET_HI, ST_WORDS };
enum StFlag : int { F_ZZ_CHECK = 1, F_ZZ_RET_ONEPOS = 2, F_REC = 4, F_LDS_OVF = 8 };
enum LevelFlag : int { LF_NEED_LO = 1, LF_NEED_HI = 2, LF_HAVE_LAST = 4 };

#ifndef WIN_E
#define WIN_E 3
#endif
#ifndef WIN_SLOTS
#define WIN_SLOTS 12
#endif
__host__ __device__ constexpr int win_entries(int G) { return (WIN_E * G > 64) ? 64 / G : (WIN_E * G < WIN_SLOTS ? WIN_SLOTS / G : WIN_E); }

constexpr int TICKET_CHUNK = 32;

__host__ __device__ inline size_t seed_lds_group_bytes(int G, int stride, int lcap) {
    const int groups = BLOCK / G;
    const int W = win_entries(G) * G;
    return (((size_t)groups * (SEED_QUERY_LDS ? stride * 8 : 0) + (size_t)groups * (2 * lcap + ST_WORDS + (W + 1) / 2) * sizeof(int)) + 7) & ~(size_t)7;
}
inline size_t seed_lds_bytes(int G, const PackGeom& geo, int lcap) {
    return seed_lds_group_bytes(G, geo.stride, lcap) + (size_t)(BLOCK / 64) * 16;
}

template <int E>
__device__ __forceinline__ void window_compare(glb_u64 pac, i64 n, q_u64 s, u64 wq, int off, int cap, const u64 (&ek)[E],
                                               const u64 (&ep)[E], int (&lcp)[E], bool (&less)[E]) {
    int l[E], Lc[E];
    bool lt[E];
    unsigned pend = 0;
    const i64 nlimit = n - (i64)cap;
#pragma unroll
    for (int e = 0; e < E; ++e) {
        Lc[e] = cap;
        if ((i64)ep[e] > nlimit) Lc[e] = (int)(n - (i64)ep[e]);
        const u64 x = ek[e] ^ wq;
        lt[e] = ek[e] < wq;
        l[e] = x ? (__clzll((long long)x) >> 1) : 32;
        if (!x && 32 < Lc[e]) pend |= 1u << e;
    }
    while (pend) {
        const int es = __ffs((int)pend) - 1;
        pend &= pend - 1;
        u64 pos = ep[0];
        int Ls = Lc[0];
#pragma unroll
        for (int e = 1; e < E; ++e)
            if (es == e) { pos = ep[e]; Ls = Lc[e]; }
        const i64 p0 = (i64)pos + 32;
        glb_u64 pw = pac + (p0 >> 5);
        const int sh = (int)(p0 & 31) * 2;
        int ll = 32;
        bool llt = false, done = false;
        for (int k = 1; !done; k += CMP_WORDS, pw += CMP_WORDS) {
            u64 w[CMP_WORDS + 1];
#pragma unroll
            for (int j = 0; j < CMP_WORDS + 1; ++j) w[j] = pw[j];
#pragma unroll
            for (int j = 0; j < CMP_WORDS; ++j) {
                if (done) break;
                const u64 wr = sh ? (w[j] << sh) | (w[j + 1] >> (64 - sh)) : w[j];
                const u64 q = ext_l(s, off + 32 * (k + j));
                const u64 y = wr ^ q;
                if (y) { ll += __clzll((long long)y) >> 1; llt = wr < q; done = true; }
                else { ll += 32; if (ll >= Ls) done = true; }
            }
        }
#pragma unroll
        for (int e = 0; e < E; ++e)
            if (es == e) { l[e] = ll; lt[e] = llt; }
    }
#pragma unroll
    for (int e = 0; e < E; ++e) {
        if (l[e] >= Lc[e]) { lcp[e] = Lc[e]; less[e] = (i64)ep[e] < nlimit; }
        else { lcp[e] = l[e]; less[e] = lt[e]; }
    }
}

__device__ __forceinline__ i64 rmi_lookup(glb_rmi l2, glb_rmi l1, i64 n_l1, int shift, i64 n, u64 key, u64& err_out) {
    u64 m = shift >= 64 ? 0ull : key >> shift;
    double icpt = l2[m].icpt, slope = l2[m].slope;
    u64 err = l2[m].err;
    double x = (double)key;
    double f = fma(slope, x, icpt);
    if (err >> 63) {
        u64 ps = (err >> 32) & 0x7fffffffull;
        double pn = (double)(err & 0xffffffffull) - 1.0;
        double c = !(f >= 0.0) ? 0.0 : (f > pn ? pn : f);
        u64 j = ps + (u64)c;
        if (j >= (u64)n_l1) j = n_l1 > 0 ? (u64)n_l1 - 1 : 0;
        f = fma(l1[j].slope, x, l1[j].icpt);
        err = l1[j].err;
    }
    err_out = err;
    double top = (double)n - 1.0;
    if (!(f >= 0.0)) return 0;
    if (f > top) return n - 1;
    return (i64)f;
}

template <int G>
__device__ __forceinline__ int group_or(int v) {
    if constexpr (G >= 2) v |= __builtin_amdgcn_update_dpp(0, v, 0xB1, 0xF, 0xF, true);
    if constexpr (G >= 4) v |= __builtin_amdgcn_update_dpp(0, v, 0x4E, 0xF, 0xF, true);
    if constexpr (G >= 8) v |= __builtin_amdgcn_update_dpp(0, v, 0x141, 0xF, 0xF, true);
    if constexpr (G >= 16) v |= __builtin_amdgcn_update_dpp(0, v, 0x140, 0xF, 0xF, true);
    if constexpr (G >= 32) v |= __shfl_xor(v, 16);
    return v;
}

template <int G, int E>
__device__ __forceinline__ int slot_pair(const int (&v)[E], int t, int ia, int ib) {
    int x = 0;
#pragma unroll
    for (int e = 0; e < E; ++e) {
        const int j = e * G + t;
        x |= (j == ia) ? (v[e] << 16) : 0;
        x |= (j == ib) ? v[e] : 0;
    }
    return group_or<G>(x);
}

__device__ __forceinline__ bool is_n(q_u64 mask, int i) { return (mask[i >> 6] >> (i & 63)) & 1ull; }

__device__ __forceinline__ int first_n(q_u64 mask, bool has_n, int from, int l_seq) {
    if (!has_n) return l_seq;
    int w = from >> 6;
    u64 m = mask[w] & (~0ull << (from & 63));
    const int nw = (l_seq + 63) >> 6;
    for (;;) {
        if (m) {
            int p = w * 64 + __ffsll((long long)m) - 1;
            return p < l_seq ? p : l_seq;
        }
        if (++w >= nw) return l_seq;
        m = mask[w];
    }
}

template <int G>
#ifndef SEED_MIN_WAVES
#define SEED_MIN_WAVES 5
#endif
__global__ void __launch_bounds__(BLOCK, (G >= 4 ? SEED_MIN_WAVES : G)) k_seed(SeedArgs A) {
    extern __shared__ __attribute__((aligned(16))) unsigned char smem_raw[];
    constexpr int GROUPS = BLOCK / G;
    constexpr int E = win_entries(G);
    constexpr int W = E * G;
    constexpr u64 GFULL = (G == 64) ? ~0ull : ((1ull << G) - 1ull);
    constexpr u64 WFULL = (W == 64) ? ~0ull : ((1ull << W) - 1ull);
    const int lane = threadIdx.x & 63;
    const int gib = threadIdx.x / G;
    const int t = threadIdx.x & (G - 1);
    const int gbase = lane & ~(G - 1);
    const int stride = A.geo.stride, PW = A.geo.W, MW = A.geo.MW;
    const int cap = A.cap, lcap = A.lcap;
#if SEED_QUERY_LDS
    u64* rd = reinterpret_cast<u64*>(smem_raw) + (size_t)gib * stride;
    const q_u64 fw = (lds_u64)rd;
#else
    q_u64 fw = (q_u64)A.packed;
#endif
#define rcs (fw + PW)
#define nfw (fw + 2 * PW)
#define nrc (fw + 2 * PW + MW)
    const lds_int ring = (lds_int)(reinterpret_cast<int*>(smem_raw + (SEED_QUERY_LDS ? (size_t)GROUPS * stride * 8 : 0)) +
                                   (size_t)gib * (2 * lcap + ST_WORDS + (W + 1) / 2));
    const lds_int sm_se = ring;
    const lds_int sm_cnt = ring + lcap;
    const lds_int st = ring + 2 * lcap;
    const lds_u16 wl = (lds_u16)(st + ST_WORDS);
    const lds_int wv = (lds_int)(reinterpret_cast<int*>(smem_raw + seed_lds_group_bytes(G, stride, lcap)) + (threadIdx.x >> 6) * 4);
    const glb_ent sa = (glb_ent)A.I.sa;
    const glb_u64 pac = (glb_u64)A.I.pac;
    const glb_rmi l2 = (glb_rmi)A.I.l2, l1 = (glb_rmi)A.I.l1;
    const i64 n = A.I.n;
    const int hits_per_smem = A.opt.hits_per_smem;
#define GBALLOT(p_) ((__ballot(p_) >> gbase) & GFULL)
#define LD64(lo_) (((i64)st[(lo_) + 1] << 32) | (u64)(unsigned)st[lo_])
#define ST64(lo_, v_) do { const i64 v__ = (v_); st[lo_] = (int)(unsigned)(v__ & 0xffffffffll); st[(lo_) + 1] = (int)(v__ >> 32); } while (0)
#define FLAG(f_) ((st[ST_FLAGS] & (f_)) != 0)
#define SETFLAG(f_, v_) do { st[ST_FLAGS] = (v_) ? (st[ST_FLAGS] | (f_)) : (st[ST_FLAGS] & ~(f_)); } while (0)
#define LDS_HANDOFF() do { __builtin_amdgcn_fence(__ATOMIC_RELEASE, "wavefront"); __builtin_amdgcn_wave_barrier(); \
                           __builtin_amdgcn_fence(__ATOMIC_ACQUIRE, "wavefront"); } while (0)

    int pc = PC_FETCH, phase = PH_CTRL;
    int pivot = 0, l_seq = 0, msl = A.opt.min_seed_len, min_intv = 1;
    bool has_n = false;
    int q_kind = 0, q_mode = 0, off = 0, vlen = 0, capc = 0;
    bool q_rc = false, q_exact = false;
    i64 base = 0, lo = -1, hi = n;
    int stepk = 0;
    u64 wq = 0;
    unsigned acc_searches = 0, acc_windows = 0;
    if (lane == 0) wv[0] = TICKET_CHUNK;
    LDS_HANDOFF();

#ifdef SEED_PROF
    unsigned prof[8] = {0, 0, 0, 0, 0, 0, 0, 0};
    unsigned long long prof_t = wall_clock64();
#define PROF_MARK(i_) do { asm volatile("s_waitcnt vmcnt(0) lgkmcnt(0)" ::: "memory"); const unsigned long long now__ = wall_clock64(); prof[i_] += (unsigned)(now__ - prof_t); prof_t = now__; } while (0)
#else
#define PROF_MARK(i_) do { } while (0)
#endif
    for (;;) {
        bool newreq = false;
        if (phase == PH_CTRL) {
            bool have = false;
#define AT(pc_) (!have && pc == (pc_))
            do {
                if (AT(PC_ZZ_TOP)) {
                    if (st[ST_ZZ_SP] >= st[ST_ZZ_NEXT] || ++st[ST_ZZ_GUARD] > 4 * l_seq + 16) pc = PC_ZZ_END;
                    else if (FLAG(F_ZZ_CHECK) && has_n && is_n(nfw, st[ST_ZZ_SP])) {
                        if (l_seq - st[ST_ZZ_SP] < msl) { pivot = l_seq; st[ST_ZZ_SP] = l_seq; }
                        else { st[ST_ZZ_SP] += 1; pivot = pivot + 1; }
                    } else { q_kind = K_ZZ_LEFT; have = true; }
                }
                if (AT(PC_ZZ_RIGHT)) { q_kind = K_ZZ_RIGHT; have = true; }
                if (AT(PC_ZZ_END)) {
                    pivot = st[ST_ZZ_NEXT];
                    pc = FLAG(F_ZZ_RET_ONEPOS) ? PC_R2_AFTER : PC_AFTER_STEP1;
                }
                if (AT(PC_AFTER_STEP1)) {
                    SETFLAG(F_REC, false);
                    st[ST_AFTER] = st[ST_N_SMEMS];
                    if (A.opt.rounds < 2) pc = PC_ALLPOS_TOP;
                    else if (FLAG(F_LDS_OVF)) pc = PC_DONE;
                    else { st[ST_R2_K] = st[ST_BEFORE]; pc = PC_R2_LOOP; }
                }
                if (AT(PC_R2_AFTER)) {
                    min_intv = st[ST_R2_SAVED];
                    pivot = st[ST_R2_NEXT];
                    pc = PC_R2_LOOP;
                }
                if (AT(PC_R2_LOOP)) {
                    int k = st[ST_R2_K];
                    const int kb = st[ST_BEFORE], ke = st[ST_AFTER];
                    int qbeg = 0, qend = 0, cnt = 0;
                    bool take = false;
                    while (k < ke) {
                        const int se = sm_se[k - kb];
                        cnt = sm_cnt[k - kb];
                        qbeg = se & 0xffff; qend = (int)((unsigned)se >> 16);
                        ++k;
                        if (!(qend - qbeg < A.opt.split_len || cnt > A.opt.split_width)) { take = true; break; }
                    }
                    st[ST_R2_K] = k;
                    if (!take) pc = PC_ALLPOS_TOP;
                    else {
                        st[ST_R2_NEXT] = pivot; st[ST_R2_SAVED] = min_intv;
                        pivot = (qbeg + qend) >> 1;
                        min_intv = cnt + 1;
                        if (has_n && is_n(nfw, pivot)) {
                            pivot = (l_seq - pivot < msl) ? l_seq : pivot + 1;
                            pc = PC_R2_AFTER;
                        } else if (pivot != 0 && !(has_n && is_n(nfw, pivot - 1))) { q_kind = K_OP_MEM; have = true; }
                        else { q_kind = K_OP_SMEM; have = true; }
                    }
                }
                if (AT(PC_ALLPOS_TOP)) {
                    if (pivot >= l_seq || ++st[ST_AP_GUARD] > 4 * l_seq + 16) pc = PC_R3_INIT;
                    else {
                        st[ST_BEFORE] = st[ST_N_SMEMS]; st[ST_SM_BASE] = st[ST_BEFORE]; SETFLAG(F_REC, true);
                        if (has_n && is_n(nfw, pivot)) {
                            pivot = (l_seq - pivot < msl) ? l_seq : pivot + 1;
                            pc = PC_AFTER_STEP1;
                        } else if (pivot != 0 && !(has_n && is_n(nfw, pivot - 1))) {
                            st[ST_ZZ_NEXT] = l_seq; SETFLAG(F_ZZ_CHECK, true); SETFLAG(F_ZZ_RET_ONEPOS, false); st[ST_ZZ_SP] = pivot; st[ST_ZZ_GUARD] = 1;
                            q_kind = K_ZZ_LEFT; have = true;
                        } else { q_kind = K_S1_RIGHT; have = true; }
                    }
                }
                if (AT(PC_R3_INIT)) {
                    if (A.opt.rounds >= 3 && A.opt.max_mem_intv > 0 && !FLAG(F_LDS_OVF)) {
                        min_intv = A.opt.max_mem_intv;
                        msl = A.opt.min_seed_len + 1;
                        pivot = 0;
                        pc = PC_R3_TOP;
                    } else pc = PC_DONE;
                }
                if (AT(PC_R3_TOP)) {
                    for (;;) {
                        if (!(pivot < l_seq - msl + 1)) { pc = PC_DONE; break; }
                        if (has_n && is_n(nfw, pivot)) { pivot = pivot + 1; continue; }
                        const int valid = first_n(nfw, has_n, pivot, l_seq) - pivot;
                        if (valid < msl) { pivot = pivot + valid; continue; }
                        q_kind = K_R3; have = true;
                        break;
                    }
                }
                if (AT(PC_DONE)) {
                    const unsigned long long ticket = ((unsigned long long)(unsigned)st[ST_TICKET_HI] << 32) | (unsigned)st[ST_TICKET_LO];
                    const bool ovf = st[ST_N_SMEMS] > cap || FLAG(F_LDS_OVF);
                    if (t == 0) {
                        const i64 rid = A.pending ? A.pending[ticket] : (i64)ticket;
                        A.slot_cnt[rid] = ovf ? 0 : st[ST_N_SMEMS];
                        A.slot_hits[rid] = ovf ? 0 : LD64(ST_HITS_LO);
                        A.slot_loc[rid] = ((i64)A.tier << 40) | (i64)ticket;
                        if (ovf) A.ovf_list[atomicAdd(&A.counters[SEED_CTR_OVERFLOW], 1ull)] = rid;
                    }
                    if (!ovf) { acc_searches += (unsigned)st[ST_SEARCHES]; acc_windows += (unsigned)st[ST_WINDOWS]; }
                    pc = PC_FETCH;
                }
                if (AT(PC_FETCH)) {
                    int idx = TICKET_CHUNK;
                    if (t == 0) idx = __hip_atomic_fetch_add(wv, 1, __ATOMIC_RELAXED, __HIP_MEMORY_SCOPE_WAVEFRONT);
                    const u64 old_base = ((u64)(unsigned)wv[3] << 32) | (unsigned)wv[2];
                    const bool over = t == 0 && idx >= TICKET_CHUNK;
                    const unsigned long long mo = __ballot(over);
                    unsigned long long ticket = old_base + (unsigned)idx;
                    if (mo) {
                        const int first = __ffsll((long long)mo) - 1;
                        const int kreq = __popcll(mo), alloc = kreq > TICKET_CHUNK ? kreq : TICKET_CHUNK;
                        unsigned long long nb = 0;
                        if (lane == first) {
                            nb = atomicAdd(&A.counters[SEED_CTR_SLOT], (unsigned long long)alloc);
                            const unsigned long long wb = nb + (unsigned)(alloc - TICKET_CHUNK);
                            wv[0] = kreq - (alloc - TICKET_CHUNK); wv[2] = (int)(unsigned)(wb & 0xffffffffull); wv[3] = (int)(wb >> 32);
                        }
                        nb = __shfl(nb, first);
                        if (over) ticket = nb + (unsigned)__popcll(mo & ((1ull << lane) - 1ull));
                    }
                    ticket = __shfl(ticket, gbase);
                    if (ticket >= (unsigned long long)A.nreads) pc = PC_EXIT;
                    else {
                        const i64 rid = A.pending ? A.pending[ticket] : (i64)ticket;
                        const u64* src = A.packed + rid * stride;
#if SEED_QUERY_LDS
                        const int lw = (stride - 1) % G;
                        u64 lenw = 0;
                        for (int k = t; k < stride; k += G) {
                            u64 v = src[k];
                            rd[k] = v;
                            if (k == stride - 1) lenw = v;
                        }
                        lenw = (u64)(unsigned)__shfl((int)lenw, gbase + lw);
#else
                        fw = (q_u64)src;
                        const u64 lenw = fw[stride - 1];
#endif
                        l_seq = (int)(lenw & 0x7fffffffull);
                        has_n = ((lenw >> 31) & 1ull) != 0;
                        for (int k = t; k < ST_WORDS; k += G) st[k] = 0;
                        LDS_HANDOFF();
                        if (l_seq <= 0 || l_seq > MAX_READ_LEN) {
                            if (t == 0) { A.slot_cnt[rid] = l_seq > MAX_READ_LEN ? -1 : 0; A.slot_hits[rid] = 0; A.slot_loc[rid] = 0; }
                        } else {
                            st[ST_TICKET_LO] = (int)(unsigned)(ticket & 0xffffffffull);
                            st[ST_TICKET_HI] = (int)(ticket >> 32);
                            pivot = 0; msl = A.opt.min_seed_len; min_intv = 1;
                            pc = PC_ALLPOS_TOP;
                            if (!(has_n && is_n(nfw, 0))) {
                                st[ST_AP_GUARD] = 1; SETFLAG(F_REC, true);
                                q_kind = K_S1_RIGHT; have = true;
                            }
                        }
                    }
                }
            } while (!have && pc != PC_EXIT);
#undef AT
            if (pc == PC_EXIT) {
                if (t == 0) {
                    atomicAdd(&A.counters[SEED_CTR_SEARCHES], (unsigned long long)acc_searches); atomicAdd(&A.counters[SEED_CTR_WINDOWS], (unsigned long long)acc_windows);
#ifdef SEED_PROF
                    for (int k = 0; k < 8; ++k) atomicAdd(&A.counters[SEED_CTR_PROF + k], (unsigned long long)prof[k]);
#endif
                }
                break;
            }
            newreq = true;
        }
        PROF_MARK(0);
        if (newreq) {
            q_rc = q_kind == K_ZZ_LEFT;
            off = q_rc ? l_seq - 1 - pivot : pivot;
            vlen = first_n(q_rc ? nrc : nfw, has_n, off, l_seq) - off;
            q_exact = q_kind == K_S1_RIGHT || q_kind == K_ZZ_RIGHT || q_kind == K_OP_SMEM;
            q_mode = q_kind == K_R3 ? 2 : ((q_exact || min_intv != 1) ? 1 : 0);
            st[ST_SEARCHES] = st[ST_SEARCHES] + 1;
            wq = ext_l(q_rc ? rcs : fw, off);
            u64 key = wq;
            if (vlen < 32) key |= (~0ull) >> (2 * vlen);
            u64 err;
            const i64 pos = rmi_lookup(l2, l1, A.I.n_l1, A.I.shift, n, key, err);
#if SEED_USE_ERR
            const i64 below = (i64)((err >> 32) & 0x3fffffffull) + 1, above = (i64)(err & 0x7fffffffull);
            const i64 span = below + above + 1;
            base = span <= W ? pos - below - (W - span) / 2 : pos - (below * W) / span;
#else
            base = pos - W / 2;
#endif
#if SEED_ALIGN_WIN
            if constexpr (W % 4 == 0) base = (base + 2) & ~3ll;
#endif
            if (base < 0) base = 0;
            if (base > n - W) base = n - W;
            lo = -1; hi = n; stepk = 0; capc = vlen;
            phase = PH_PART;
        }
        PROF_MARK(1);

        const q_u64 s = q_rc ? rcs : fw;
        int lcp[E];
        bool less[E];
        u64 ep[E];
        {
            u64 ek[E];
#pragma unroll
            for (int e = 0; e < E; ++e) { ek[e] = sa[base + e * G + t].key; ep[e] = sa[base + e * G + t].pos; }
            st[ST_WINDOWS] = st[ST_WINDOWS] + 1;
            window_compare<E>(pac, n, s, wq, off, capc, ek, ep, lcp, less);
        }
        PROF_MARK(2);
        u64 m = 0;
#pragma unroll
        for (int e = 0; e < E; ++e) {
            const bool p = phase == PH_PART ? less[e] : ((lcp[e] >= capc) == (phase == PH_EDGE_UP));
            m |= GBALLOT(p) << (e * G);
        }
        if (stepk != 0)
            m = (m | lowmask((int)((lo - base + 1 > W) ? W : (lo - base + 1 < 0 ? 0 : lo - base + 1)))) &
                lowmask((int)((hi - base > W) ? W : (hi - base < 0 ? 0 : hi - base)));
        const int P = __popcll(m);
        const bool at_lo = base == 0 || (phase == PH_EDGE_UP && base == lo + 1);
        const bool at_hi = base + W == n || (phase == PH_EDGE_DN && base + W == hi);
        const bool found = (P > 0 && P < W) || (P == 0 && at_lo) || (P == W && at_hi);

        bool go_level = false, finished = false;
        int L = 0, nb_lo = 0, nb_hi = 0, lf = 0;
        i64 s_edge = 0, e_edge = 0, cb = base;
        int r_L = 0;
        i64 r_start = 0, r_count = 1, r_T = -1;
        bool r_emit = false;
        int cl[E];
        bool cache_in_lds = phase != PH_PART;
        if (found) {
            const int v2 = slot_pair<G, E>(lcp, t, P - 1, P);
            const int lm = P > 0 ? (v2 >> 16) : -1;
            const int lp = P < W ? (v2 & 0xffff) : -1;
            if (phase == PH_PART) {
                const int c = (lm >= lp) ? P - 1 : P;
                L = lm >= lp ? lm : lp;
                r_L = L; r_start = base + c; r_count = 1;
                if (q_exact || q_kind == K_R3) {
                    u64 tc = 0;
#pragma unroll
                    for (int e = 0; e < E; ++e) tc = (e * G + t == c) ? ep[e] : tc;
                    r_T = (i64)(((u64)(unsigned)group_or<G>((int)(tc >> 32)) << 32) | (u64)(unsigned)group_or<G>((int)(unsigned)tc));
                }
                if (q_mode == 0 || (q_mode == 2 && L < msl)) finished = true;
                else {
                    s_edge = e_edge = base + c;
                    lf = LF_NEED_LO | LF_NEED_HI;
                    go_level = true;
                }
            } else {
                L = st[ST_L]; nb_lo = st[ST_NB_LO]; nb_hi = st[ST_NB_HI]; lf = st[ST_LF];
                s_edge = LD64(ST_SE_LO); e_edge = LD64(ST_EE_LO); cb = LD64(ST_CB_LO);
                if (phase == PH_EDGE_DN) { s_edge = base + P; nb_lo = P > 0 ? lm : 0; lf &= ~LF_NEED_LO; }
                else { e_edge = base + P - 1; nb_hi = P < W ? lp : 0; lf &= ~LF_NEED_HI; }
                go_level = true;
            }
        } else {
            if (P == W) lo = base + W - 1; else hi = base;
            bool stop = false;
            if (phase != PH_PART && !q_exact) {
                s_edge = LD64(ST_SE_LO); e_edge = LD64(ST_EE_LO);
                if (phase == PH_EDGE_DN ? (e_edge - hi + 1 >= (i64)min_intv) : (lo - s_edge + 1 >= (i64)min_intv)) {
                    L = st[ST_L]; nb_lo = st[ST_NB_LO]; nb_hi = st[ST_NB_HI]; lf = st[ST_LF]; cb = LD64(ST_CB_LO);
                    if (phase == PH_EDGE_DN) { s_edge = hi; nb_lo = L; lf &= ~LF_NEED_LO; }
                    else { e_edge = lo; nb_hi = L; lf &= ~LF_NEED_HI; }
                    stop = go_level = true;
                }
            }
            if (!stop) {
                if (lo < 0) { base = hi - ((i64)W << stepk); ++stepk; if (base < 0) base = 0; }
                else if (hi >= n) { base = lo + 1 + (((i64)W << stepk) - W); ++stepk; if (base > n - W) base = n - W; }
                else if (hi - lo <= W - 1) { base = lo; if (base > n - W) base = n - W; }
                else base = lo + (hi - lo) / 2 - W / 2;
            }
        }
        PROF_MARK(3);
        if (go_level) {
#pragma unroll
            for (int e = 0; e < E; ++e) cl[e] = cache_in_lds ? (int)wl[e * G + t] : lcp[e];
            for (;;) {
                if (lf & (LF_NEED_LO | LF_NEED_HI)) {
                    u64 ge = 0;
#pragma unroll
                    for (int e = 0; e < E; ++e) ge |= GBALLOT(cl[e] >= L) << (e * G);
                    const u64 nz = ~ge & WFULL;
                    const i64 klo = s_edge - cb;
                    const i64 khi = e_edge - cb;
                    const bool in_lo = (lf & LF_NEED_LO) && klo > 0 && klo <= W;
                    const bool in_hi = (lf & LF_NEED_HI) && khi >= -1 && khi < W - 1;
                    const u64 zlo = in_lo ? (nz & lowmask((int)klo)) : 0ull;
                    const u64 zhi = in_hi ? (nz & ~lowmask((int)khi + 1)) : 0ull;
                    const int hz = zlo ? 63 - __clzll((long long)zlo) : -1;
                    const int lz = zhi ? __ffsll((long long)zhi) - 1 : -1;
                    const int nb2 = slot_pair<G, E>(cl, t, hz, lz);
                    if (lf & LF_NEED_LO) {
                        if (in_lo) {
                            if (zlo) { s_edge = cb + hz + 1; nb_lo = nb2 >> 16; lf &= ~LF_NEED_LO; }
                            else { s_edge = cb; if (cb == 0) { nb_lo = 0; lf &= ~LF_NEED_LO; } }
                        } else if (s_edge == 0) { nb_lo = 0; lf &= ~LF_NEED_LO; }
                    }
                    if (lf & LF_NEED_HI) {
                        if (in_hi) {
                            if (zhi) { e_edge = cb + lz - 1; nb_hi = nb2 & 0xffff; lf &= ~LF_NEED_HI; }
                            else { e_edge = cb + W - 1; if (cb + W >= n) { nb_hi = 0; lf &= ~LF_NEED_HI; } }
                        } else if (e_edge == n - 1) { nb_hi = 0; lf &= ~LF_NEED_HI; }
                    }
                    if (lf & LF_NEED_LO) {
                        phase = PH_EDGE_DN; lo = -1; hi = s_edge; stepk = 1;
                        base = s_edge - W; if (base < 0) base = 0;
                        break;
                    }
                    if (lf & LF_NEED_HI) {
                        phase = PH_EDGE_UP; lo = e_edge; hi = n; stepk = 1;
                        base = e_edge + 1; if (base > n - W) base = n - W;
                        break;
                    }
                }
                const i64 cnt = e_edge - s_edge + 1;
                const int nxt = nb_lo > nb_hi ? nb_lo : nb_hi;
                if (q_mode == 1) {
                    if (cnt >= (i64)min_intv) { r_L = L; r_start = s_edge; r_count = cnt; finished = true; break; }
                } else {
                    if (cnt >= (i64)min_intv) {
                        if (lf & LF_HAVE_LAST) { r_count = LD64(ST_LAST_CNT_LO); r_start = LD64(ST_LAST_S_LO); }
                        else { r_count = cnt; r_start = s_edge; }
                        r_L = L + 1;
                        finished = true;
                        break;
                    }
                    if (nxt < msl) { r_L = msl; r_start = s_edge; r_count = cnt; finished = true; break; }
                    lf |= LF_HAVE_LAST;
                    ST64(ST_LAST_CNT_LO, cnt);
                    ST64(ST_LAST_S_LO, s_edge);
                }
                L = nxt;
                lf = (lf & LF_HAVE_LAST) | ((nb_lo >= L && s_edge > 0) ? LF_NEED_LO : 0) | ((nb_hi >= L && e_edge < n - 1) ? LF_NEED_HI : 0);
            }
            if (finished) {
                if (q_mode == 2) {
                    r_emit = r_count < (i64)min_intv;
                    if (r_L < msl) r_L = msl;
                }
            } else {
                capc = L;
                st[ST_L] = L; st[ST_NB_LO] = nb_lo; st[ST_NB_HI] = nb_hi; st[ST_LF] = lf;
                ST64(ST_SE_LO, s_edge); ST64(ST_EE_LO, e_edge); ST64(ST_CB_LO, cb);
                if (!cache_in_lds) {
#pragma unroll
                    for (int e = 0; e < E; ++e) wl[e * G + t] = (unsigned short)cl[e];
                }
            }
        }
        PROF_MARK(4);
        if (finished) {
            bool emit = false;
            const int e_start = pivot;
            int e_end = pivot;
            switch (q_kind) {
            case K_S1_RIGHT:
            case K_ZZ_RIGHT:
            case K_OP_SMEM:
                emit = r_L >= msl; e_end = pivot + r_L;
                break;
            case K_ZZ_LEFT:
                pivot = pivot - r_L + 1;
                pc = (st[ST_ZZ_NEXT] - pivot < msl) ? PC_ZZ_END : PC_ZZ_RIGHT;
                break;
            case K_OP_MEM:
                st[ST_ZZ_NEXT] = pivot + r_L; SETFLAG(F_ZZ_CHECK, false); SETFLAG(F_ZZ_RET_ONEPOS, true); st[ST_ZZ_SP] = pivot; st[ST_ZZ_GUARD] = 0;
                pc = PC_ZZ_TOP;
                break;
            default:
                emit = r_emit; e_end = pivot + r_L;
                break;
            }
            if (emit) {
                const int ns = st[ST_N_SMEMS];
                const bool have_pos = r_count == 1 && r_T >= 0 && !cache_in_lds;
                const bool defer = have_pos && A.defer != 0 && FLAG(F_REC) && ns < DEFER_MAX_K && ns < cap && A.opt.rounds >= 2 &&
                                   e_end - e_start >= A.opt.split_len && A.opt.split_width >= 1 && nb_lo < msl && nb_hi < msl;
                if (ns < cap && t == 0) {
                    const unsigned long long ticket = ((unsigned long long)(unsigned)st[ST_TICKET_HI] << 32) | (unsigned)st[ST_TICKET_LO];
                    SlotRec sr;
                    sr.start = e_start; sr.end = e_end; sr.count = r_count;
                    sr.sa_start = have_pos ? (SLOT_POS | (defer ? SLOT_DEFER : 0ll) | r_T) : r_start;
                    A.slots[(i64)ticket * cap + ns] = sr;
                }
                if (FLAG(F_REC)) {
                    const int k = ns - st[ST_SM_BASE];
                    if (k < lcap) {
                        sm_se[k] = e_start | (e_end << 16);
                        sm_cnt[k] = (defer || r_count > (i64)INT_MAX) ? INT_MAX : (int)r_count;
                    } else SETFLAG(F_LDS_OVF, true);
                }
                st[ST_N_SMEMS] = ns + 1;
                i64 h = r_count;
                if (hits_per_smem > 0 && h > hits_per_smem) h = hits_per_smem;
                h += LD64(ST_HITS_LO);
                ST64(ST_HITS_LO, h);
            }
            switch (q_kind) {
            case K_S1_RIGHT: pivot = pivot + r_L; pc = PC_AFTER_STEP1; break;
            case K_ZZ_RIGHT: pivot = pivot + r_L; st[ST_ZZ_SP] = pivot; pc = PC_ZZ_TOP; break;
            case K_OP_SMEM: pivot = pivot + r_L; pc = PC_R2_AFTER; break;
            case K_R3: pivot = pivot + (r_L < msl ? msl : r_L); pc = PC_R3_TOP; break;
            default: break;
            }
            phase = PH_CTRL;
        }
        PROF_MARK(5);
    }
#undef PROF_MARK
#undef rcs
#undef nfw
#undef nrc
#undef GBALLOT
#undef LD64
#undef ST64
#undef FLAG
#undef SETFLAG
#undef LDS_HANDOFF
}


__device__ __forceinline__ u64 ext_g(const u64* __restrict__ w, int s) {
    const int k = s >> 5, sh = (s & 31) * 2;
    const u64 a = w[k], b = w[k + 1];
    return sh ? (a << sh) | (b >> (64 - sh)) : a;
}

struct LaneQuery {
    const u64* s;
    int off, vlen;
    u64 wq;
};

__device__ __forceinline__ void lane_compare_ent(const DevIndex& I, const LaneQuery& q, int cap, const SaEnt e, int& lcp, bool& less) {
    const i64 nlimit = I.n - (i64)cap;
    int Lc = cap;
    if ((i64)e.pos > nlimit) Lc = (int)(I.n - (i64)e.pos);
    const u64 x = e.key ^ q.wq;
    bool lt = e.key < q.wq;
    int l = x ? (__clzll((long long)x) >> 1) : 32;
    if (!x && 32 < Lc) {
        const i64 p0 = (i64)e.pos + 32;
        for (int k = 1;; ++k) {
            const u64 wr = extract32(I.pac, p0 + 32 * (k - 1));
            const u64 qq = ext_g(q.s, q.off + 32 * k);
            const u64 y = wr ^ qq;
            if (y) { l += __clzll((long long)y) >> 1; lt = wr < qq; break; }
            l += 32;
            if (l >= Lc) break;
        }
    }
    if (l >= Lc) { lcp = Lc; less = (i64)e.pos < nlimit; }
    else { lcp = l; less = lt; }
}
__device__ __forceinline__ void lane_compare(const DevIndex& I, const LaneQuery& q, int cap, i64 slot, int& lcp, bool& less) {
    lane_compare_ent(I, q, cap, I.sa[slot], lcp, less);
}

constexpr int LANE_W = 16;
struct LaneWin {
    uint32_t* lw;
    i64 base;
    i64 ms0, ms1;
    int mv0, mv1;
    __device__ __forceinline__ bool has(i64 slot) const { return base >= 0 && slot >= base && slot < base + LANE_W; }
    __device__ __forceinline__ int get(i64 slot) const { const int i = (int)(slot - base); return (int)((lw[(i >> 1) * 256] >> (16 * (i & 1))) & 0xffffu); }
};
struct LaneTally {
    unsigned no_intv, walked, nb_probes;
#ifdef RESEED_PROF
    unsigned part_probes, run_probes;
#endif
};
#ifdef RESEED_PROF
#define RESEED_COUNT(x_) (++(x_))
#else
#define RESEED_COUNT(x_) do { } while (0)
#endif
#if defined(RESEED_PROF) && RESEED_PROF == 2
#define RESEED_EARLY_STOP 0
#else
#define RESEED_EARLY_STOP 1
#endif
#ifndef RESEED_TALLY
#define RESEED_TALLY 1
#endif
__device__ __forceinline__ int lane_lcp(const DevIndex& I, const LaneQuery& q, const LaneWin& C, int cap, i64 slot, LaneTally& T) {
    if (C.has(slot)) return C.get(slot);
    if (slot == C.ms0) return C.mv0;
    if (slot == C.ms1) return C.mv1;
    int lc; bool ls;
    lane_compare(I, q, cap, slot, lc, ls);
    RESEED_COUNT(T.run_probes);
    return lc;
}

template <int J> __device__ __forceinline__ int quad_bcast(int v) { return __builtin_amdgcn_update_dpp(0, v, J * 0x55, 0xF, 0xF, true); }
template <int J> __device__ __forceinline__ u64 quad_bcast64(u64 v) {
    return ((u64)(unsigned)quad_bcast<J>((int)(v >> 32)) << 32) | (u64)(unsigned)quad_bcast<J>((int)(unsigned)v);
}
__device__ __forceinline__ void lds_handoff() {
    __builtin_amdgcn_fence(__ATOMIC_RELEASE, "wavefront"); __builtin_amdgcn_wave_barrier(); __builtin_amdgcn_fence(__ATOMIC_ACQUIRE, "wavefront");
}
template <int J>
__device__ __forceinline__ void quad_window_load(const SaEnt* __restrict__ sa, i64 base, int t, SaEnt (&ent)[LANE_W / 4]) {
    const i64 bo = (i64)quad_bcast64<J>((u64)base);
#pragma unroll
    for (int i = 0; i < LANE_W / 4; ++i) ent[i] = sa[bo + 4 * i + t];
}
template <int J>
__device__ __forceinline__ unsigned quad_window_compare(const DevIndex& I, const LaneQuery& q, bool active, int t, const SaEnt (&ent)[LANE_W / 4], uint32_t* lwq) {
    LaneQuery qo;
    qo.s = reinterpret_cast<const u64*>(quad_bcast64<J>((u64)reinterpret_cast<uintptr_t>(q.s)));
    const int ov = quad_bcast<J>(q.off | (q.vlen << 16));
    qo.off = ov & 0xffff; qo.vlen = (int)((unsigned)ov >> 16);
    qo.wq = quad_bcast64<J>(q.wq);
    const bool ao = quad_bcast<J>(active ? 1 : 0) != 0;
    unsigned m = 0;
    if (ao) {
        unsigned short* col = reinterpret_cast<unsigned short*>(lwq + J) + (t & 1);
#pragma unroll
        for (int i = 0; i < LANE_W / 4; ++i) {
            int lc; bool ls;
            lane_compare_ent(I, qo, qo.vlen, ent[i], lc, ls);
            m |= (ls ? 1u : 0u) << (4 * i + t);
            col[(2 * i + (t >> 1)) * 512] = (unsigned short)lc;
        }
    }
    return (unsigned)group_or<4>((int)m);
}

__device__ __forceinline__ void lane_search(const DevIndex& I, const LaneQuery& q, bool active, int min_intv, bool want_intv, int msl, uint32_t* lw,
                                            LaneTally& T, int& r_L, i64& r_start, i64& r_count) {
    const i64 n = I.n;
    const int t = threadIdx.x & 3;
    i64 p = 0, base = 0;
    if (active) {
        u64 key = q.wq;
        if (q.vlen < 32) key |= (~0ull) >> (2 * q.vlen);
        u64 err;
        p = rmi_lookup((glb_rmi)I.l2, (glb_rmi)I.l1, I.n_l1, I.shift, n, key, err);
        const i64 below = (i64)((err >> 32) & 0x3fffffffull) + 1, above = (i64)(err & 0x7fffffffull);
        const i64 span = below + above + 1;
        base = span <= LANE_W ? p - below - (LANE_W - span) / 2 : p - (below * LANE_W) / span;
        if (base < 0) base = 0;
        if (base > n - LANE_W) base = n - LANE_W;
    }
    unsigned lessm;
    {
        lds_handoff();
        SaEnt e0[LANE_W / 4], e1[LANE_W / 4], e2[LANE_W / 4], e3[LANE_W / 4];
        quad_window_load<0>(I.sa, base, t, e0); quad_window_load<1>(I.sa, base, t, e1);
        quad_window_load<2>(I.sa, base, t, e2); quad_window_load<3>(I.sa, base, t, e3);
        uint32_t* lwq = lw - t;
        const unsigned m0 = quad_window_compare<0>(I, q, active, t, e0, lwq), m1 = quad_window_compare<1>(I, q, active, t, e1, lwq);
// ... 591 lines not shown
```

bwa-meme_amd/pymeme/hipapi.py:

```python
from __future__ import annotations

import ctypes as C
import os

import numpy as np

PKG = os.path.dirname(os.path.dirname(os.path.abspath(__file__)))
LIB_PATH = os.environ.get("MEME_HIP_LIB") or os.path.join(PKG, "libmeme_hip.so")

MEM_TL = np.dtype([("start", "<i4"), ("end", "<i4"), ("hitbeg", "<i4"), ("hitcount", "<i4"),
                   ("cache_refpos", "<u8")])
SEQPAIR = np.dtype([(n, "<i4") for n in ("idr", "idq", "id", "len1", "len2", "h0", "seqid", "regid", "score",
                                         "tle", "gtle", "qle", "gscore", "max_off")])


class SeedOpt(C.Structure):
    _fields_ = [(n, C.c_int32) for n in ("min_seed_len", "split_len", "split_width", "max_mem_intv", "rounds",
                                         "hits_per_smem")]


class BswOpt(C.Structure):
    _fields_ = [(n, C.c_int32) for n in ("o_del", "e_del", "o_ins", "e_ins", "zdrop", "end_bonus", "a", "b")]


# ... 45 lines not shown

def records_equal(a, b):
    return a.dtype == b.dtype and a.shape == b.shape and all(np.array_equal(a[f], b[f]) for f in a.dtype.names)


GJOB = np.dtype([("rb", "<i8"), ("read", "<i4"), ("qb", "<i4"), ("qlen", "<i4"), ("tlen", "<i4"), ("w", "<i4"), ("rev", "<i4")])
GRES = np.dtype([("score", "<i4"), ("n_cigar", "<i4"), ("cigar_off", "<i8")])
assert GJOB.itemsize == 32 and GRES.itemsize == 16


class GresHost(C.Structure):
    _fields_ = [("njobs", C.c_int64), ("res", C.c_void_p), ("cigars", C.c_void_p), ("total_ops", C.c_int64), ("kernel_ms", C.c_float)]


CJOB = np.dtype([("rb", "<i8"), ("read", "<i4"), ("qb", "<i4"), ("qlen", "<i4"), ("tlen", "<i4"), ("w_", "<i4"), ("pad", "<i4")])
CRES = np.dtype([("score", "<i4"), ("n_cigar", "<i4"), ("nm", "<i4"), ("md_len", "<i4"), ("cigar_off", "<i8"), ("md_off", "<i8")])
assert CJOB.itemsize == 32 and CRES.itemsize == 32


class CresHost(C.Structure):
    _fields_ = [("njobs", C.c_int64), ("res", C.c_void_p), ("cigars", C.c_void_p), ("total_ops", C.c_int64), ("md", C.c_void_p), ("md_bytes", C.c_int64),
                ("kernel_ms", C.c_float)]


SAM_REC = np.dtype([("pos", "<i8"), ("m_pos", "<i8"), ("cigar_off", "<i8"), ("m_cigar_off", "<i8"), ("xa_off", "<i8")] +
                   [(n, "<i4") for n in ("read", "flag", "rid", "is_rev", "is_alt", "mapq", "NM", "score", "sub", "n_cigar", "has_mate", "m_rid", "m_is_rev", "m_is_alt",
                                         "m_n_cigar", "which")])
assert SAM_REC.itemsize == 104


class SamHost(C.Structure):
    _fields_ = [("nrecs", C.c_int64), ("text_off", C.c_void_p), ("text", C.c_void_p), ("text_bytes", C.c_int64), ("kernel_ms", C.c_float)]


class KswvHost(C.Structure):
    _fields_ = [("njobs", C.c_int64), ("res", C.c_void_p), ("kernel_ms", C.c_float)]


class MateHost(C.Structure):
    _fields_ = [("nreads", C.c_int64), ("nbatches", C.c_int64), ("njobs", C.c_int64), ("n_gar", C.c_int64), ("gar", C.c_void_p), ("gar_off", C.c_void_p), ("job_off", C.c_void_p),
                ("jobs", C.c_void_p), ("res", C.c_void_p), ("pose_ms", C.c_float), ("kernel_ms", C.c_float)]


class PrimaryOpt(C.Structure):
    _fields_ = [(n, C.c_int32) for n in ("a", "b", "o_del", "e_del", "o_ins", "e_ins", "min_seed_len", "T")] + [("mask_level", C.c_float), ("mapQ_coef_len", C.c_float)] + \
               [("mapQ_coef_fac", C.c_int32), ("primary5", C.c_int32)]


class PrimaryHost(C.Structure):
    _fields_ = [("nreads", C.c_int64), ("total_regs", C.c_int64), ("regs", C.c_void_p), ("n_pri", C.c_void_p), ("mapq", C.c_void_p), ("status", C.c_void_p), ("n_heavy", C.c_int64),
                ("kernel_ms", C.c_float)]


class PrimaryDeviceOut(C.Structure):
    _fields_ = [(n, C.c_void_p) for n in ("d_regs_out", "d_n_pri", "d_mapq", "d_status", "d_n_heavy")]


def default_primary_opt(**kw):
    o = PrimaryOpt(1, 4, 6, 1, 6, 1, 19, 30, 0.5, 50.0, 3, 0)
    for k, v in kw.items():
        assert hasattr(o, k), k
        setattr(o, k, v)
    return o


class PairPes(C.Structure):
    _fields_ = [(n, C.c_int32) for n in ("low", "high", "failed", "pad")] + [("avg", C.c_double), ("std", C.c_double)]


class PairOpt(C.Structure):
    _fields_ = [(n, C.c_int32) for n in ("a", "b", "o_del", "e_del", "o_ins", "e_ins")]


class PairHost(C.Structure):
    _fields_ = [("npairs", C.c_int64), ("score", C.c_void_p), ("sub", C.c_void_p), ("n_sub", C.c_void_p), ("n_cand", C.c_void_p), ("z", C.c_void_p), ("status", C.c_void_p),
                ("n_heavy", C.c_int64), ("kernel_ms", C.c_float)]


class PairDeviceOut(C.Structure):
    _fields_ = [(n, C.c_void_p) for n in ("d_score", "d_sub", "d_n_sub", "d_n_cand", "d_z", "d_status", "d_n_heavy")]


def default_pair_opt(**kw):
    o = PairOpt(1, 4, 6, 1, 6, 1)
    for k, v in kw.items():
        assert hasattr(o, k), k
        setattr(o, k, v)
    return o


def pair_pes(pes):
    assert len(pes) == 4
    return (PairPes * 4)(*[PairPes(int(lo), int(hi), int(failed), 0, float(avg), float(std)) for lo, hi, failed, avg, std in pes])


class FinishOpt(C.Structure):
    _fields_ = [(n, C.c_int32) for n in ("a", "b", "o_del", "e_del", "o_ins", "e_ins", "w", "max_chain_gap")] + [("mask_level_redun", C.c_float), ("pad", C.c_int32)]


class FinishHost(C.Structure):
    _fields_ = [("nreads", C.c_int64), ("total_regs", C.c_int64), ("regs", C.c_void_p), ("reg_off", C.c_void_p), ("use_mate_sort", C.c_void_p), ("status", C.c_void_p),
                ("n_wave", C.c_int64), ("n_patch_jobs", C.c_int64), ("n_patched", C.c_int64), ("kernel_ms", C.c_float)]


class FinishDeviceOut(C.Structure):
    _fields_ = [(n, C.c_void_p) for n in ("d_regs_out", "d_reg_off_out", "d_use_mate_sort", "d_status", "d_counters")]


def default_finish_opt(**kw):
    o = FinishOpt(1, 4, 6, 1, 6, 1, 100, 10000, 0.95, 0)
    for k, v in kw.items():
        assert hasattr(o, k), k
        setattr(o, k, v)
    return o


class MateOpt(C.Structure):
    _fields_ = [(n, C.c_int32) for n in ("a", "b", "o_del", "e_del", "o_ins", "e_ins", "pen_unpaired", "max_matesw", "min_seed_len", "batch_reads")]


MATE_REG = np.dtype([("rb", "<i8"), ("rid", "<i4"), ("score", "<i4")])
KSWV_JOB = np.dtype([("idr", "<i8"), ("idq", "<i8"), ("len1", "<i4"), ("len2", "<i4"), ("xtra", "<i4"), ("pad", "<i4")])
KSWR = np.dtype([(n, "<i4") for n in ("score", "te", "qe", "score2", "te2", "tb", "qb")])
CHAIN = np.dtype({"names": ["pos", "rid", "n_seeds", "w", "first", "kept", "is_alt", "seed_beg"],
                  "formats": ["<i8", "<i4", "<i4", "<i4", "<i4", "<i2", "<i2", "<i4"], "offsets": [0, 8, 12, 16, 20, 24, 26, 28], "itemsize": 40})
CHAIN_SEED = np.dtype([("rbeg", "<i8"), ("qbeg", "<i4"), ("len", "<i4")])


def default_chain_opt(l_pac):
    return ChainOpt(100, 10000, 500, 19, 0, 1 << 30, 0.5, 0.5, l_pac)


class SeedResult(C.Structure):
    _fields_ = [("d_smems", C.c_void_p), ("d_smem_off", C.c_void_p), ("d_hits", C.c_void_p),
                ("d_hit_off", C.c_void_p), ("total_smems", C.c_int64), ("total_hits", C.c_int64),
                ("searches", C.c_int64)]


class Timings(C.Structure):
    _fields_ = [("seed_kernel_ms", C.c_float), ("seed_gather_ms", C.c_float), ("bsw_kernel_ms", C.c_float),
                ("seed_launches", C.c_int64), ("bsw_launches", C.c_int64), ("seed_pack_ms", C.c_float),
                ("seed_windows", C.c_int64), ("chain_kernel_ms", C.c_float), ("chain_pass2_ms", C.c_float), ("chain_tier3_ms", C.c_float),
                ("chain_tier2_reads", C.c_int64), ("chain_tier3_reads", C.c_int64),
                ("seed_reseed_ms", C.c_float), ("seed_lane_searches", C.c_int64), ("gcig_class_jobs", C.c_int64 * 6)]


EXPORTS = ["meme_device_count", "meme_ctx_create", "meme_ctx_destroy", "meme_last_error", "meme_ctx_sync",
           "meme_ctx_stream", "meme_index_load_host", "meme_index_load_files", "meme_index_pac64_words",
           "meme_index_pos5_bytes",
           "meme_index_attach", "meme_index_describe", "meme_index_share", "meme_index_replicate", "meme_host_alloc",
           "meme_host_free", "meme_stage_pack_text", "meme_stage_pos5_from_sa", "meme_stage_build_entries", "meme_stage_build_plcp",
           "meme_stage_entries_from_sa", "meme_stage_rmi32", "meme_sa_build_device", "meme_prmi_train_device", "meme_seed_batch", "meme_seed_batch_host", "meme_seed_batch_resident", "meme_seed_batch_resident_ascii", "meme_seed_reserve", "meme_chain_last_batch_host", "meme_chain_batch_host", "meme_extend_last_batch_host", "meme_global_batch_host", "meme_gen_cigar_batch_host", "meme_sam_stage_text", "meme_sam_format_batch_host", "meme_kswv_batch_host", "meme_matesw_batch_host", "meme_primary_batch_host", "meme_primary_batch_device", "meme_finish_batch_host", "meme_finish_batch_device", "meme_pair_batch_host", "meme_pair_batch_device", "meme_seed_batch_device",
           "meme_bsw_batch", "meme_bsw_batch_device", "meme_get_timings", "meme_set_tuning", "meme_debug_packed_reads",
           "meme_debug_reseed_counts", "meme_debug_sa_stats", "meme_debug_scan_exclusive"]

RESEED_MAX_ROUNDS = 8
RESEED_COUNTS = RESEED_MAX_ROUNDS + 6
SA_STATS = ("k_pad", "groups", "largest_group", "tied", "rounds", "pieces", "pad_pieces")

_lib = None


def default_seed_opt(rounds=3, hits_per_smem=0):
    return SeedOpt(19, 28, 10, 20, rounds, hits_per_smem)


def default_bsw_opt(end_bonus=5):
    return BswOpt(6, 1, 6, 1, 100, end_bonus, 1, 4)


def lib():
    global _lib
    if _lib is None:
        if not os.path.exists(LIB_PATH):
            raise RuntimeError("%s is missing: build it with `make -C bwa-meme_amd hip` "
                               "(or __graft_entry__.build())" % LIB_PATH)
        try:
            import torch
        except ImportError:
            pass
        L = C.CDLL(LIB_PATH)
        L.meme_ctx_create.restype = C.c_void_p
        L.meme_ctx_create.argtypes = [C.c_int]
        L.meme_ctx_destroy.argtypes = [C.c_void_p]
        L.meme_ctx_destroy.restype = None
        L.meme_last_error.restype = C.c_char_p
        L.meme_ctx_stream.restype = C.c_void_p
        L.meme_ctx_stream.argtypes = [C.c_void_p]
        for f in ("meme_index_pac64_words", "meme_index_pos5_bytes"):
            getattr(L, f).restype = C.c_int64
            getattr(L, f).argtypes = [C.c_int64]
        L.meme_host_alloc.restype = C.c_void_p
        L.meme_host_alloc.argtypes = [C.c_int64]
        L.meme_host_free.argtypes = [C.c_void_p]
        L.meme_host_free.restype = None
        _lib = L
    return _lib


class MemeError(RuntimeError):
    pass


def _check(rc):
    if rc != 0:
        raise MemeError("meme_hip error %d: %s" % (rc, lib().meme_last_error().decode()))


def _p(a):
    return C.c_void_p(a.ctypes.data)


def _view(ptr, count, dtype):
    if count == 0 or not ptr:
        return np.zeros(0, dtype=dtype)
    buf = (C.c_char * (count * np.dtype(dtype).itemsize)).from_address(ptr)
    return np.frombuffer(buf, dtype=dtype, count=count).copy()


def _contig_array(contigs):
    return (Contig * len(contigs))(*[Contig(int(o), int(l), int(a)) for o, l, a in contigs])


class Context:

    def __init__(self, device=0):
        L = lib()
        if L.meme_device_count() <= 0:
            raise MemeError("no HIP device visible -- the MI355X backend has no CPU fallback")
        self.h = L.meme_ctx_create(device)
        if not self.h:
            raise MemeError(L.meme_last_error().decode())
        self.device = device
        for kv in filter(None, os.environ.get("MEME_TUNING", "").split(",")):
            k, v = kv.split("=")
            self.set_tuning(k.strip(), int(v))

    def close(self):
        if getattr(self, "h", None):
            lib().meme_ctx_destroy(C.c_void_p(self.h))
            self.h = None

    def __del__(self):
        try:
            self.close()
        except Exception:
            pass

    def load_index_files(self, prefix):
        _check(lib().meme_index_load_files(C.c_void_p(self.h), prefix.encode()))

    def load_index_host(self, pos_packed, text, l1, l2):
        pos_packed = np.ascontiguousarray(pos_packed, dtype=np.uint8)
        text = np.ascontiguousarray(text, dtype=np.uint8)
        l1 = np.ascontiguousarray(l1).view(np.uint8)
        l2 = np.ascontiguousarray(l2).view(np.uint8)
        _check(lib().meme_index_load_host(C.c_void_p(self.h), _p(pos_packed), C.c_int64(text.shape[0]), _p(text),
                                          _p(l1), C.c_int64(l1.shape[0]), _p(l2), C.c_int64(l2.shape[0])))

    def attach_index(self, arrays: IndexArrays):
        _check(lib().meme_index_attach(C.c_void_p(self.h), C.byref(arrays)))

    def describe_index(self) -> IndexArrays:
        a = IndexArrays()
        _check(lib().meme_index_describe(C.c_void_p(self.h), C.byref(a)))
        return a

    def replicate_index_from(self, src: "Context"):
        _check(lib().meme_index_replicate(C.c_void_p(self.h), C.c_void_p(src.h)))

    def set_tuning(self, key, value):
        _check(lib().meme_set_tuning(C.c_void_p(self.h), key.encode(), C.c_int64(value)))

    def timings(self) -> Timings:
        t = Timings()
        _check(lib().meme_get_timings(C.c_void_p(self.h), C.byref(t)))
        return t

    def sync(self):
        _check(lib().meme_ctx_sync(C.c_void_p(self.h)))

    def seed_batch(self, reads, read_off, opt=None, smem_capacity=None, hit_capacity=None):
        opt = opt or default_seed_opt()
        reads = np.ascontiguousarray(reads, dtype=np.uint8).reshape(-1)
        read_off = np.ascontiguousarray(read_off, dtype=np.int64)
        n = read_off.shape[0] - 1
        smem_capacity = smem_capacity or max(64 * n, 1024)
        hit_capacity = hit_capacity or max(1024 * n, 1 << 16)
        while True:
            smems = np.zeros(smem_capacity, dtype=MEM_TL)
            hits = np.zeros(hit_capacity, dtype=np.uint64)
            smem_off = np.zeros(n + 1, dtype=np.int64)
            hit_off = np.zeros(n + 1, dtype=np.int64)
            ts, th = C.c_int64(0), C.c_int64(0)
            rc = lib().meme_seed_batch(C.c_void_p(self.h), _p(reads), _p(read_off), C.c_int64(n), C.byref(opt),
                                       _p(smems), C.c_int64(smem_capacity), _p(smem_off), _p(hits),
                                       C.c_int64(hit_capacity), _p(hit_off), C.byref(ts), C.byref(th))
            if rc == -4:
                smem_capacity = max(smem_capacity, ts.value + 1)
                hit_capacity = max(hit_capacity, th.value + 1)
                continue
            _check(rc)
            return smems[:ts.value], smem_off, hits[:th.value], hit_off

    def seed_batch_host(self, reads, read_off, opt=None):
        opt = opt or default_seed_opt()
        reads = np.ascontiguousarray(reads, dtype=np.uint8).reshape(-1)
        read_off = np.ascontiguousarray(read_off, dtype=np.int64)
        n = read_off.shape[0] - 1
        res = SeedHostResult()
        _check(lib().meme_seed_batch_host(C.c_void_p(self.h), _p(reads), _p(read_off), C.c_int64(n), C.byref(opt),
                                          C.byref(res)))
        return (_view(res.smems, res.total_smems, MEM_TL), _view(res.smem_off, n + 1, np.int64),
                _view(res.hits, res.total_hits, np.uint64), _view(res.hit_off, n + 1, np.int64))

    def seed_batch_resident(self, reads, read_off, opt=None):
        opt = opt or default_seed_opt()
        reads = np.ascontiguousarray(reads, dtype=np.uint8).reshape(-1)
        read_off = np.ascontiguousarray(read_off, dtype=np.int64)
        ts, th = C.c_int64(0), C.c_int64(0)
        _check(lib().meme_seed_batch_resident(C.c_void_p(self.h), _p(reads), _p(read_off), C.c_int64(read_off.shape[0] - 1), C.byref(opt),
                                              C.byref(ts), C.byref(th)))
        return ts.value, th.value

    def seed_batch_resident_ascii(self, reads_ascii, read_off, opt=None):
        opt = opt or default_seed_opt()
        reads = np.ascontiguousarray(reads_ascii, dtype=np.uint8).reshape(-1)
        read_off = np.ascontiguousarray(read_off, dtype=np.int64)
        ts, th = C.c_int64(0), C.c_int64(0)
        _check(lib().meme_seed_batch_resident_ascii(C.c_void_p(self.h), _p(reads), _p(read_off), C.c_int64(read_off.shape[0] - 1), C.byref(opt),
                                                    C.byref(ts), C.byref(th)))
        return ts.value, th.value

    def debug_packed_reads(self):
        geom, n = (C.c_int32 * 3)(), C.c_int64(0)
        _check(lib().meme_debug_packed_reads(C.c_void_p(self.h), None, C.c_int64(0), geom, C.byref(n)))
        words = np.zeros((n.value, geom[2]), dtype=np.uint64)
        _check(lib().meme_debug_packed_reads(C.c_void_p(self.h), _p(words), C.c_int64(words.size), geom, C.byref(n)))
        return words, int(geom[0]), int(geom[1])

    def debug_reseed_counts(self):
        out, rounds = np.zeros(RESEED_COUNTS, dtype=np.int64), C.c_int32(0)
        _check(lib().meme_debug_reseed_counts(C.c_void_p(self.h), _p(out), C.c_int32(out.size), C.byref(rounds)))
        st = RESEED_MAX_ROUNDS
        return {"rounds": [int(v) for v in out[:rounds.value]], "stage": [int(v) for v in out[st:st + 3]], "no_interval": int(out[st + 3]),
                "walked": int(out[st + 4]), "neighbour_probes": int(out[st + 5])}

    def debug_sa_stats(self):
        out = np.zeros(len(SA_STATS), dtype=np.int64)
        _check(lib().meme_debug_sa_stats(C.c_void_p(self.h), _p(out), C.c_int32(out.size)))
        return {k: int(v) for k, v in zip(SA_STATS, out)}

    def debug_scan_exclusive(self, d_in_ptr, d_out_ptr, n):
        _check(lib().meme_debug_scan_exclusive(C.c_void_p(self.h), C.c_void_p(d_in_ptr), C.c_void_p(d_out_ptr), C.c_int64(n)))

    def seed_reserve(self, nreads, total_bases):
        _check(lib().meme_seed_reserve(C.c_void_p(self.h), C.c_int64(nreads), C.c_int64(total_bases)))

    def chain_last_batch_host(self, contigs, opt):
        arr = _contig_array(contigs)
        res = ChainHostResult()
        _check(lib().meme_chain_last_batch_host(C.c_void_p(self.h), arr, C.c_int32(len(contigs)), C.byref(opt), C.byref(res)))
        return self._chain_result(res)

    def extend_last_batch_host(self, contigs, chain_opt, ext_opt=None):
        ext_opt = ext_opt or default_ext_opt()
        arr = _contig_array(contigs)
        res = ExtHostResult()
        _check(lib().meme_extend_last_batch_host(C.c_void_p(self.h), arr, C.c_int32(len(contigs)), C.byref(chain_opt), C.byref(ext_opt), C.byref(res)))
        n = res.nreads
        return {"reg_off": _view(res.reg_off, n + 1, np.int64), "regs": _view(res.regs, res.total_regs, ALNREG), "total_chains": int(res.total_chains),
                "n_pairs": int(res.n_pairs), "n_retried": int(res.n_retried), "n_bsw_calls": int(res.n_bsw_calls), "n_tier2": int(res.n_tier2),
                "chain_ms": float(res.chain_ms), "ext_ms": float(res.ext_ms), "bsw_ms": float(res.bsw_ms),
                "n_flt_jobs": int(res.n_flt_jobs), "n_flt_dropped": int(res.n_flt_dropped), "n_exact_prefix": int(res.n_exact_prefix),
                "census_band_cells": int(res.census_band_cells), "census_class": [int(x) for x in res.census_class], "total_seeds": int(res.total_seeds), "n_ext_seeds": int(res.n_ext_seeds)}

    def global_batch_host(self, jobs, opt=None):
        opt = opt or default_bsw_opt()
        jobs = np.ascontiguousarray(jobs, dtype=GJOB)
        res = GresHost()
        _check(lib().meme_global_batch_host(C.c_void_p(self.h), _p(jobs), C.c_int64(jobs.shape[0]), C.byref(opt), C.byref(res)))
        return _view(res.res, res.njobs, GRES), _view(res.cigars, res.total_ops, np.uint32), float(res.kernel_ms)

    def gen_cigar_batch_host(self, jobs, opt=None):
        opt = opt or default_bsw_opt()
        jobs = np.ascontiguousarray(jobs, dtype=CJOB)
        res = CresHost()
        _check(lib().meme_gen_cigar_batch_host(C.c_void_p(self.h), _p(jobs), C.c_int64(jobs.shape[0]), C.byref(opt), C.byref(res)))
        return _view(res.res, res.njobs, CRES), _view(res.cigars, res.total_ops, np.uint32), _view(res.md, res.md_bytes, np.uint8), float(res.kernel_ms)

    def sam_stage_text(self, names, quals=None):
        blob = np.frombuffer(b"".join(names), dtype=np.uint8).copy() if names else np.zeros(1, np.uint8)
        if blob.shape[0] == 0:
            blob = np.zeros(1, np.uint8)
        off = np.zeros(len(names) + 1, np.int64)
        off[1:] = np.cumsum([len(x) for x in names])
        q = np.frombuffer(quals, dtype=np.uint8).copy() if quals is not None else None
        _check(lib().meme_sam_stage_text(C.c_void_p(self.h), _p(blob), _p(off), _p(q) if q is not None else C.c_void_p(0)))

    def sam_format_batch_host(self, recs, blob, contig_names, softclip=0, rg_id=b""):
        recs = np.ascontiguousarray(recs, dtype=SAM_REC)
        blob = np.ascontiguousarray(blob, dtype=np.uint8)
        cn = b"".join(n.encode() if isinstance(n, str) else n for n in contig_names)
        cb = np.frombuffer(cn, dtype=np.uint8).copy() if cn else np.zeros(1, np.uint8)
        co = np.zeros(len(contig_names) + 1, np.int32)
        co[1:] = np.cumsum([len(n) for n in contig_names])
        res = SamHost()
        _check(lib().meme_sam_format_batch_host(C.c_void_p(self.h), _p(recs), C.c_int64(recs.shape[0]), _p(blob), C.c_int64(blob.shape[0]), _p(cb), _p(co),
                                                 C.c_int32(len(contig_names)), C.c_int32(int(softclip)), C.c_char_p(rg_id), C.byref(res)))
        if res.nrecs == 0:
            return b"", np.zeros(1, np.int64), 0.0
        return _view(res.text, res.text_bytes, np.uint8).tobytes(), _view(res.text_off, res.nrecs + 1, np.int64), float(res.kernel_ms)

    def kswv_batch_host(self, jobs, ref, qer, opt=None):
        opt = opt or default_bsw_opt()
        jobs = np.ascontiguousarray(jobs, dtype=KSWV_JOB)
        ref = np.ascontiguousarray(ref, dtype=np.uint8)
        qer = np.ascontiguousarray(qer, dtype=np.uint8)
        res = KswvHost()
        _check(lib().meme_kswv_batch_host(C.c_void_p(self.h), _p(jobs), C.c_int64(jobs.shape[0]), _p(ref), C.c_int64(ref.shape[0]), _p(qer),
                                          C.c_int64(qer.shape[0]), C.byref(opt), C.byref(res)))
        return _view(res.res, res.njobs, KSWR), float(res.kernel_ms)

    def matesw_batch_host(self, regs, reg_off, pes, contigs, l_pac, a=1, b=4, o_del=6, e_del=1, o_ins=6, e_ins=1, pen_unpaired=17, max_matesw=50, min_seed_len=19,
                          batch_reads=512, reads_of=None, first_read=0):
        regs = np.ascontiguousarray(regs, dtype=MATE_REG)
        reg_off = np.ascontiguousarray(reg_off, dtype=np.int64)
        pes4 = np.zeros((4, 4), np.int32)
        pes4[:, :3] = np.asarray(pes, np.int32).reshape(4, 3)
        arr = _contig_array(contigs)
        opt = MateOpt(a, b, o_del, e_del, o_ins, e_ins, pen_unpaired, max_matesw, min_seed_len, batch_reads)
        res = MateHost()
        _check(lib().meme_matesw_batch_host(C.c_void_p(self.h), C.c_void_p(reads_of.h if reads_of is not None else None), _p(regs), _p(reg_off), C.c_int64(first_read), C.c_int64(reg_off.shape[0] - 1), _p(pes4), arr, C.c_int32(len(contigs)), C.c_int64(l_pac),
                                            C.byref(opt), C.byref(res)))
        return {"gar": _view(res.gar, res.n_gar, np.int32), "gar_off": _view(res.gar_off, res.nbatches + 1, np.int64), "job_off": _view(res.job_off, res.nbatches + 1, np.int64),
                "jobs": _view(res.jobs, res.njobs, KSWV_JOB), "res": _view(res.res, res.njobs, KSWR), "pose_ms": float(res.pose_ms), "kernel_ms": float(res.kernel_ms)}

    def primary_batch_host(self, regs, reg_off, id_base=0, opt=None):
        opt = opt or default_primary_opt()
        assert regs.dtype == ALNREG and regs.flags.c_contiguous
        reg_off = np.ascontiguousarray(reg_off, dtype=np.int64)
        n = reg_off.shape[0] - 1
        res = PrimaryHost()
        _check(lib().meme_primary_batch_host(C.c_void_p(self.h), _p(regs), _p(reg_off), C.c_int64(n), C.c_int64(int(id_base)), C.byref(opt), C.byref(res)))
        return {"regs": _view(res.regs, res.total_regs, ALNREG), "n_pri": _view(res.n_pri, res.nreads, np.int32), "mapq": _view(res.mapq, res.total_regs, np.uint8),
                "status": _view(res.status, res.nreads, np.uint8), "n_heavy": int(res.n_heavy), "kernel_ms": float(res.kernel_ms)}

    def primary_batch_device(self, d_regs_ptr, d_reg_off_ptr, nreads, total_regs, id_base, opt, d_regs_out_ptr, d_n_pri_ptr, d_mapq_ptr, d_status_ptr, d_n_heavy_ptr):
        out = PrimaryDeviceOut(d_regs_out_ptr, d_n_pri_ptr, d_mapq_ptr, d_status_ptr, d_n_heavy_ptr)
        _check(lib().meme_primary_batch_device(C.c_void_p(self.h), C.c_void_p(d_regs_ptr), C.c_void_p(d_reg_off_ptr), C.c_int64(nreads), C.c_int64(total_regs), C.c_int64(int(id_base)),
                                               C.byref(opt or default_primary_opt()), C.byref(out)))

    def pair_batch_host(self, regs, reg_off, n_pri, contigs, l_pac, pes, id_base=0, opt=None):
        opt = opt or default_pair_opt()
        assert regs.dtype == ALNREG and regs.flags.c_contiguous
        reg_off = np.ascontiguousarray(reg_off, dtype=np.int64)
        n_pri = np.ascontiguousarray(n_pri, dtype=np.int32)
        n = reg_off.shape[0] - 1
        assert n_pri.shape[0] == n
        arr = _contig_array(contigs)
        res = PairHost()
        _check(lib().meme_pair_batch_host(C.c_void_p(self.h), _p(regs), _p(reg_off), _p(n_pri), C.c_int64(n), arr, C.c_int32(len(contigs)), C.c_int64(int(l_pac)), pair_pes(pes),
                                          C.c_int64(int(id_base)), C.byref(opt), C.byref(res)))

        m = int(res.npairs)
        return {"score": _view(res.score, m, np.int32), "sub": _view(res.sub, m, np.int32), "n_sub": _view(res.n_sub, m, np.int32), "n_cand": _view(res.n_cand, m, np.int32),
                "z": _view(res.z, 2 * m, np.int32).reshape(m, 2), "status": _view(res.status, m, np.uint8), "n_heavy": int(res.n_heavy), "kernel_ms": float(res.kernel_ms)}

    def pair_batch_device(self, d_regs_ptr, d_reg_off_ptr, d_n_pri_ptr, nreads, total_regs, contigs, l_pac, pes, id_base, opt, d_score_ptr, d_sub_ptr, d_n_sub_ptr, d_n_cand_ptr, d_z_ptr,
                          d_status_ptr, d_n_heavy_ptr):
        arr = _contig_array(contigs)
        out = PairDeviceOut(d_score_ptr, d_sub_ptr, d_n_sub_ptr, d_n_cand_ptr, d_z_ptr, d_status_ptr, d_n_heavy_ptr)
        _check(lib().meme_pair_batch_device(C.c_void_p(self.h), C.c_void_p(d_regs_ptr), C.c_void_p(d_reg_off_ptr), C.c_void_p(d_n_pri_ptr), C.c_int64(nreads), C.c_int64(total_regs), arr,
                                            C.c_int32(len(contigs)), C.c_int64(int(l_pac)), pair_pes(pes), C.c_int64(int(id_base)), C.byref(opt or default_pair_opt()), C.byref(out)))

    def finish_batch_host(self, regs, reg_off, contigs, l_pac, opt=None):
        opt = opt or default_finish_opt()
        assert regs.dtype == ALNREG and regs.flags.c_contiguous
        reg_off = np.ascontiguousarray(reg_off, dtype=np.int64)
        n = reg_off.shape[0] - 1
        arr = _contig_array(contigs)
        res = FinishHost()
        _check(lib().meme_finish_batch_host(C.c_void_p(self.h), _p(regs), _p(reg_off), C.c_int64(n), arr, C.c_int32(len(contigs)), C.c_int64(int(l_pac)), C.byref(opt), C.byref(res)))
        return {"regs": _view(res.regs, res.total_regs, ALNREG), "reg_off": _view(res.reg_off, res.nreads + 1, np.int64), "use_mate_sort": _view(res.use_mate_sort, res.nreads, np.uint8),
                "status": _view(res.status, res.nreads, np.uint8), "n_wave": int(res.n_wave), "n_patch_jobs": int(res.n_patch_jobs), "n_patched": int(res.n_patched),
                "kernel_ms": float(res.kernel_ms)}

    def finish_batch_device(self, d_regs_ptr, d_reg_off_ptr, nreads, total_regs, contigs, l_pac, opt, d_regs_out_ptr, d_reg_off_out_ptr, d_use_mate_sort_ptr, d_status_ptr, d_counters_ptr):
        arr = _contig_array(contigs)
        out = FinishDeviceOut(d_regs_out_ptr, d_reg_off_out_ptr, d_use_mate_sort_ptr, d_status_ptr, d_counters_ptr)
        _check(lib().meme_finish_batch_device(C.c_void_p(self.h), C.c_void_p(d_regs_ptr), C.c_void_p(d_reg_off_ptr), C.c_int64(nreads), C.c_int64(total_regs), arr, C.c_int32(len(contigs)),
                                              C.c_int64(int(l_pac)), C.byref(opt or default_finish_opt()), C.byref(out)))

    def chain_batch_host(self, smems, smem_off, hits, hit_off, read_len, contigs, opt):
        arr = _contig_array(contigs)
        smems = np.ascontiguousarray(smems, dtype=MEM_TL)
        smem_off = np.ascontiguousarray(smem_off, dtype=np.int64)
        hits = np.ascontiguousarray(hits, dtype=np.uint64)
        hit_off = np.ascontiguousarray(hit_off, dtype=np.int64)
        read_len = np.ascontiguousarray(read_len, dtype=np.int32)
# ... 133 lines not shown
```

include/meme_hip.h:

```cpp
#ifndef MEME_HIP_H
#define MEME_HIP_H
#include <stdint.h>

#ifdef __cplusplus
extern "C" {
#endif

#define MEME_OK 0
#define MEME_E_HIP (-1)
#define MEME_E_ARG (-2)
#define MEME_E_IO (-3)
#define MEME_E_CAPACITY (-4)
#define MEME_E_STATE (-5)

typedef struct meme_ctx meme_ctx;

typedef struct {
    int32_t start, end;
    int32_t hitbeg, hitcount;
    uint64_t cache_refpos;
} meme_mem_tl;

typedef struct {
    int32_t idr, idq, id;
// ... 127 lines not shown
    int64_t census_band_cells;
    int64_t census_class[9];
    int64_t total_seeds;
    int64_t n_ext_seeds;
} meme_ext_host_result;
int meme_extend_last_batch_host(meme_ctx* ctx, const meme_contig* contigs, int32_t n_contigs, const meme_chain_opt* chain_opt,
                                const meme_ext_opt* ext_opt, meme_ext_host_result* out);

typedef struct {
    const meme_mem_tl* d_smems;
    const int64_t* d_smem_off;
    const uint64_t* d_hits;
    const int64_t* d_hit_off;
    int64_t total_smems, total_hits;
    int64_t searches;
} meme_seed_result;
int meme_seed_batch_device(meme_ctx* ctx, const uint8_t* d_reads, const int64_t* d_read_off,
                           int64_t nreads, int64_t total_bases, const meme_seed_opt* opt,
                           meme_seed_result* out);

int meme_bsw_batch(meme_ctx* ctx, meme_seqpair* pairs, const uint8_t* ref_buf, int64_t ref_bytes,
                   const uint8_t* qer_buf, int64_t qer_bytes, int32_t npairs, int32_t w,
                   const meme_bsw_opt* opt);
int meme_bsw_batch_device(meme_ctx* ctx, meme_seqpair* d_pairs, const uint8_t* d_ref, const uint8_t* d_qer,
                          int32_t npairs, int32_t w, const meme_bsw_opt* opt);

typedef struct { int64_t rb; int32_t read, qb, qlen, tlen, w, rev; } meme_gjob;
typedef struct { int32_t score, n_cigar; int64_t cigar_off;  } meme_gres;
typedef struct { int64_t njobs; const meme_gres* res; const uint32_t* cigars; int64_t total_ops; float kernel_ms; } meme_gres_host;
int meme_global_batch_host(meme_ctx* ctx, const meme_gjob* jobs, int64_t njobs, const meme_bsw_opt* opt ,
                           meme_gres_host* out);

typedef struct { int64_t rb; int32_t read, qb, qlen, tlen, w_, pad; } meme_cjob;
typedef struct { int32_t score, n_cigar, nm, md_len; int64_t cigar_off, md_off; } meme_cres;
typedef struct { int64_t njobs; const meme_cres* res; const uint32_t* cigars; int64_t total_ops; const char* md; int64_t md_bytes; float kernel_ms; } meme_cres_host;
int meme_gen_cigar_batch_host(meme_ctx* ctx, const meme_cjob* jobs, int64_t njobs, const meme_bsw_opt* opt ,
                              meme_cres_host* out);

typedef struct {
    int64_t pos, m_pos;
    int64_t cigar_off;
    int64_t m_cigar_off;
    int64_t xa_off;
    int32_t read;
    int32_t flag;
    int32_t rid, is_rev, is_alt, mapq, NM, score, sub, n_cigar;
    int32_t has_mate, m_rid, m_is_rev, m_is_alt, m_n_cigar;
    int32_t which;
} meme_sam_rec;
typedef struct { int64_t nrecs; const int64_t* text_off; const char* text; int64_t text_bytes; float kernel_ms; } meme_sam_host_result;
int meme_sam_stage_text(meme_ctx* ctx, const char* names, const int64_t* name_off , const char* quals);
int meme_sam_format_batch_host(meme_ctx* ctx, const meme_sam_rec* recs, int64_t nrecs, const uint8_t* blob, int64_t blob_bytes,
                               const char* contig_names, const int32_t* contig_name_off , int32_t n_contigs,
                               int32_t softclip , const char* rg_id ,
                               meme_sam_host_result* out);

typedef struct { int64_t idr, idq; int32_t len1, len2, xtra, pad; } meme_kswv_job;
typedef struct { int32_t score, te, qe, score2, te2, tb, qb; } meme_kswr;
typedef struct { int64_t njobs; const meme_kswr* res;  float kernel_ms; } meme_kswv_host_result;
int meme_kswv_batch_host(meme_ctx* ctx, const meme_kswv_job* jobs, int64_t njobs, const uint8_t* ref, int64_t ref_bytes, const uint8_t* qer, int64_t qer_bytes,
                         const meme_bsw_opt* opt, meme_kswv_host_result* out);

typedef struct { int64_t rb; int32_t rid, score; } meme_mate_reg;
typedef struct { int32_t low, high, failed, pad; } meme_pestat;
typedef struct { int32_t a, b, o_del, e_del, o_ins, e_ins, pen_unpaired, max_matesw, min_seed_len, batch_reads; } meme_mate_opt;
typedef struct {
    int64_t nreads, nbatches, njobs, n_gar;
    const int32_t* gar; const int64_t* gar_off; const int64_t* job_off;
    const meme_kswv_job* jobs; const meme_kswr* res;
    float pose_ms, kernel_ms;
} meme_mate_host_result;
int meme_matesw_batch_host(meme_ctx* ctx, meme_ctx* reads_of ,
                           const meme_mate_reg* regs, const int64_t* reg_off , int64_t first_read, int64_t nreads, const meme_pestat* pes ,
                           const meme_contig* contigs, int32_t n_contigs, int64_t l_pac, const meme_mate_opt* opt, meme_mate_host_result* out);

typedef struct {
    int32_t a, b, o_del, e_del, o_ins, e_ins, min_seed_len, T;
    float mask_level, mapQ_coef_len;
    int32_t mapQ_coef_fac;
    int32_t primary5;
} meme_primary_opt;
typedef struct {
    int64_t nreads, total_regs;
    const meme_alnreg* regs;
    const int32_t* n_pri;
    const uint8_t* mapq;
    const uint8_t* status;
    int64_t n_heavy;
    float kernel_ms;
} meme_primary_host_result;
int meme_primary_batch_host(meme_ctx* ctx, const meme_alnreg* regs, const int64_t* reg_off , int64_t nreads, int64_t id_base,
                            const meme_primary_opt* opt, meme_primary_host_result* out);
typedef struct { meme_alnreg* d_regs_out; int32_t* d_n_pri; uint8_t* d_mapq; uint8_t* d_status; uint64_t* d_n_heavy; } meme_primary_device_out;
int meme_primary_batch_device(meme_ctx* ctx, const meme_alnreg* d_regs, const int64_t* d_reg_off, int64_t nreads, int64_t total_regs, int64_t id_base,
                              const meme_primary_opt* opt, const meme_primary_device_out* out);

typedef struct { int32_t low, high, failed, pad; double avg, std; } meme_pair_pes;
typedef struct { int32_t a, b, o_del, e_del, o_ins, e_ins; } meme_pair_opt;
typedef struct {
    int64_t npairs;
    const int32_t *score, *sub, *n_sub, *n_cand;
    const int32_t* z;
    const uint8_t* status;
    int64_t n_heavy;
    float kernel_ms;
} meme_pair_host_result;
int meme_pair_batch_host(meme_ctx* ctx, const meme_alnreg* regs, const int64_t* reg_off , const int32_t* n_pri , int64_t nreads,
                         const meme_contig* contigs, int32_t n_contigs, int64_t l_pac, const meme_pair_pes* pes , int64_t id_base, const meme_pair_opt* opt,
                         meme_pair_host_result* out);
typedef struct { int32_t *d_score, *d_sub, *d_n_sub, *d_n_cand, *d_z; uint8_t* d_status; uint64_t* d_n_heavy; } meme_pair_device_out;
int meme_pair_batch_device(meme_ctx* ctx, const meme_alnreg* d_regs, const int64_t* d_reg_off, const int32_t* d_n_pri, int64_t nreads, int64_t total_regs,
                           const meme_contig* contigs, int32_t n_contigs, int64_t l_pac, const meme_pair_pes* pes , int64_t id_base, const meme_pair_opt* opt,
                           const meme_pair_device_out* out);

typedef struct { int32_t a, b, o_del, e_del, o_ins, e_ins, w, max_chain_gap; float mask_level_redun; int32_t pad; } meme_finish_opt;
typedef struct {
    int64_t nreads, total_regs;
    const meme_alnreg* regs;
    const int64_t* reg_off;
    const uint8_t* use_mate_sort;
    const uint8_t* status;
    int64_t n_wave, n_patch_jobs, n_patched;
    float kernel_ms;
} meme_finish_host_result;
int meme_finish_batch_host(meme_ctx* ctx, const meme_alnreg* regs, const int64_t* reg_off , int64_t nreads,
                           const meme_contig* contigs, int32_t n_contigs, int64_t l_pac, const meme_finish_opt* opt, meme_finish_host_result* out);
typedef struct { meme_alnreg* d_regs_out; int64_t* d_reg_off_out; uint8_t* d_use_mate_sort; uint8_t* d_status; uint64_t* d_counters; } meme_finish_device_out;
int meme_finish_batch_device(meme_ctx* ctx, const meme_alnreg* d_regs, const int64_t* d_reg_off, int64_t nreads, int64_t total_regs,
                             const meme_contig* contigs, int32_t n_contigs, int64_t l_pac, const meme_finish_opt* opt, const meme_finish_device_out* out);

typedef struct {
    float seed_kernel_ms;
    float seed_gather_ms;
    float bsw_kernel_ms;
    int64_t seed_launches, bsw_launches;
    float seed_pack_ms;
    int64_t seed_windows;
    float chain_kernel_ms;
    float chain_pass2_ms;
    float chain_tier3_ms;
    int64_t chain_tier2_reads, chain_tier3_reads;
    float seed_reseed_ms;
    int64_t seed_lane_searches;
    int64_t gcig_class_jobs[6];
} meme_timings;
int meme_get_timings(meme_ctx* ctx, meme_timings* out);
int meme_set_tuning(meme_ctx* ctx, const char* key, int64_t value);

int meme_debug_packed_reads(meme_ctx* ctx, uint64_t* out, int64_t capacity_words, int32_t* geom, int64_t* nreads);

#define MEME_RESEED_COUNTS 14
int meme_debug_reseed_counts(meme_ctx* ctx, int64_t* out, int32_t capacity, int32_t* rounds);

#define MEME_SA_STATS 7
int meme_debug_sa_stats(meme_ctx* ctx, int64_t* out, int32_t capacity);

int meme_debug_scan_exclusive(meme_ctx* ctx, const int64_t* d_in, int64_t* d_out, int64_t n);

#ifdef __cplusplus
}
#endif
#endif
```

Before: 158.2 million reads/s.

## Split seeding kernel into rounds 1-2 and round-3 launches with capped round-3 search

Templates the seed kernel on a round selector so rounds 1-2 and round 3 run as separate launches, with a carry buffer passing per-read state between them. The round-3 kernel drops the LDS SMEM ring and keeps only the forward query words in LDS, which shrinks its LDS footprint and register/branch load and should raise occupancy. It also caps round-3 forward extension at 32 bases and redoes the search uncapped only when that cap is hit. The cost is an extra kernel launch, a second pass over the packed reads, and added code complexity, including a repeat path.

```diff
diff --git a/bwa-meme_amd/csrc/meme_common.h b/bwa-meme_amd/csrc/meme_common.h
--- a/bwa-meme_amd/csrc/meme_common.h
+++ b/bwa-meme_amd/csrc/meme_common.h
@@ -134,12 +134,15 @@
     bool reads_resident = false;
 };
 enum { SEED_CTR_SLOT = 0, SEED_CTR_SEARCHES = 1, SEED_CTR_OVERFLOW = 2, SEED_CTR_WINDOWS = 3, SEED_CTR_PROF = 4, SEED_CTR_LANE = 12, SEED_CTR_PEND = 13, SEED_CTR_BLK = 14, SEED_CTR_BLK_OUT = 15,
-       SEED_CTR_RS_ROUND = 16, SEED_CTR_RS_STAGE = 24, SEED_CTR_RS_NOINTV = 27, SEED_CTR_RS_WALKED = 28, SEED_CTR_RS_NBPROBE = 29, SEED_CTRS = 32 };
+       SEED_CTR_RS_ROUND = 16, SEED_CTR_RS_STAGE = 24, SEED_CTR_RS_NOINTV = 27, SEED_CTR_RS_WALKED = 28, SEED_CTR_RS_NBPROBE = 29, SEED_CTR_SLOT3 = 30, SEED_CTR_R3_REPEAT = 31, SEED_CTRS = 32 };
 constexpr int RESEED_MAX_ROUNDS = SEED_CTR_RS_STAGE - SEED_CTR_RS_ROUND;
 enum { SEED_EV_PACK0, SEED_EV_PACK1, SEED_EV_SEARCH0, SEED_EV_SEARCH1, SEED_EV_RESEED0, SEED_EV_GATHER0, SEED_EV_GATHER1, SEED_EVS };
 struct SeedWs {
     DevBuf slots[3], ovf[2];
     DevBuf slot_cnt, slot_hits, slot_loc, counters, pend, blk;
+    DevBuf carry;
+    long long r3_counts[MEME_R3_COUNTS] = {0};
+    bool r3_valid = false;
     long long reseed_counts[SEED_CTRS - SEED_CTR_RS_ROUND] = {0};
     int reseed_rounds = 0;
     HostBuf h_smems, h_hits, h_smem_off, h_hit_off;
@@ -240,6 +243,7 @@
     i64 gcig_zcap = -1;
     i64 ext_census = 0;
     i64 seed_defer = 1;
+    i64 seed_r3_split = 1;
     i64 chain_light_hits = 32;
     i64 chain_lane_hits = 256;
     i64 chain_wave_tiers = 1;
diff --git a/bwa-meme_amd/csrc/meme_ctx.hip b/bwa-meme_amd/csrc/meme_ctx.hip
--- a/bwa-meme_amd/csrc/meme_ctx.hip
+++ b/bwa-meme_amd/csrc/meme_ctx.hip
@@ -134,10 +134,11 @@
 extern "C" int meme_set_tuning(meme_ctx* ctx, const char* key, int64_t value) {
     if (!ctx || !key) return MEME_E_ARG;
     if (!strcmp(key, "gcig_groups") && value != 0 && value != 1) { meme_set_error("gcig_groups must be 0 or 1"); return MEME_E_ARG; }
+    if (!strcmp(key, "seed_r3_split") && value != 0 && value != 1) { meme_set_error("seed_r3_split must be 0 or 1"); return MEME_E_ARG; }
     if (!strcmp(key, "group_lanes") && value != 1 && value != 2 && value != 4 && value != 8 && value != 16 && value != 32) { meme_set_error("group_lanes must be 1, 2, 4, 8, 16 or 32"); return MEME_E_ARG; }
     const i64 any = INT64_MIN;
     static const struct { const char* key; i64 meme_ctx::*member; i64 at_least; } keys[] = {
-        {"seed_blocks", &meme_ctx::seed_blocks, any}, {"helper_blocks", &meme_ctx::helper_blocks, 0}, {"smem_cap", &meme_ctx::smem_cap, 8}, {"seed_defer", &meme_ctx::seed_defer, any}, {"max_batch", &meme_ctx::max_batch, any},
+        {"seed_blocks", &meme_ctx::seed_blocks, any}, {"helper_blocks", &meme_ctx::helper_blocks, 0}, {"smem_cap", &meme_ctx::smem_cap, 8}, {"seed_defer", &meme_ctx::seed_defer, any}, {"seed_r3_split", &meme_ctx::seed_r3_split, 0}, {"max_batch", &meme_ctx::max_batch, any},
         {"sam_max_batch", &meme_ctx::sam_max_batch, any}, {"bsw_circ", &meme_ctx::bsw_circ, any}, {"ext_split", &meme_ctx::ext_split, any}, {"ext_slab_jobs", &meme_ctx::ext_slab_jobs, 1},
         {"ext_census", &meme_ctx::ext_census, any}, {"gcig_zcap", &meme_ctx::gcig_zcap, any}, {"gcig_groups", &meme_ctx::gcig_groups, any}, {"ext_live_only", &meme_ctx::ext_live_only, any},
         {"ext_rounds", &meme_ctx::ext_rounds, 0}, {"bsw_blocks", &meme_ctx::bsw_blocks, any}, {"bsw_lane_min_pairs", &meme_ctx::bsw_lane_min_pairs, any},
diff --git a/bwa-meme_amd/csrc/meme_seed.hip b/bwa-meme_amd/csrc/meme_seed.hip
--- a/bwa-meme_amd/csrc/meme_seed.hip
+++ b/bwa-meme_amd/csrc/meme_seed.hip
@@ -163,13 +163,21 @@
     }
 }
 
+template <int G, int RND>
+int launch_k_seed_rounds(hipStream_t stream, const SeedArgs& A, size_t lds, i64 blocks) {
+    if (lds > 64 * 1024)
+        HIP_TRY(hipFuncSetAttribute((const void*)k_seed<G, RND>, hipFuncAttributeMaxDynamicSharedMemorySize, (int)lds));
+    hipLaunchKernelGGL((k_seed<G, RND>), dim3((unsigned)blocks), dim3(BLOCK), lds, stream, A);
+    HIP_TRY(hipGetLastError());
+    return MEME_OK;
+}
 template <int G>
-int launch_k_seed(hipStream_t stream, const SeedArgs& A, size_t lds, i64 blocks) {
-    if (lds > 64 * 1024)
-        HIP_TRY(hipFuncSetAttribute((const void*)k_seed<G>, hipFuncAttributeMaxDynamicSharedMemorySize, (int)lds));
-    hipLaunchKernelGGL(k_seed<G>, dim3((unsigned)blocks), dim3(BLOCK), lds, stream, A);
-    HIP_TRY(hipGetLastError());
-    return MEME_OK;
+int launch_k_seed(hipStream_t stream, const SeedArgs& A, size_t lds, i64 blocks, int rnd) {
+    switch (rnd) {
+    case SEED_R12: return launch_k_seed_rounds<G, SEED_R12>(stream, A, lds, blocks);
+    case SEED_R3: return launch_k_seed_rounds<G, SEED_R3>(stream, A, lds, blocks);
+    default: return launch_k_seed_rounds<G, SEED_ALL>(stream, A, lds, blocks);
+    }
 }
 
 struct SeedRun {
@@ -179,6 +187,7 @@
     PackGeom geo;
     TierTable tiers = {};
     bool defer = false;
+    bool split = false;
     i64 n_early = -1;
     i64 n_todo = 0;
     float ms_total = 0.f, ms_reseed = 0.f;
@@ -226,7 +235,7 @@
     return MEME_OK;
 }
 
-int launch_tier(SeedRun& R, int tier, i64 n_todo, const i64* pending, int cset, hipStream_t stream, bool defer) {
+int launch_tier(SeedRun& R, int tier, i64 n_todo, const i64* pending, int cset, hipStream_t stream, bool defer, int rnd = SEED_ALL) {
     meme_ctx* ctx = R.ctx;
     int G = tier == 0 ? (int)ctx->group_lanes : 32;
     const int cap = tier == 0 ? (int)ctx->smem_cap : TIER_CAP[tier];
@@ -244,10 +253,12 @@
         }
     }
     int rc;
-    if ((rc = meme_buf_reserve(ctx, sb, need))) return rc;
-    if ((rc = meme_buf_reserve(ctx, ob, (size_t)n_todo * sizeof(i64)))) return rc;
     unsigned long long* counters = ctx->seed.counter_set(cset);
-    HIP_TRY(hipMemsetAsync(counters, 0, SEED_CTRS * sizeof(unsigned long long), stream));
+    if (rnd != SEED_R3) {
+        if ((rc = meme_buf_reserve(ctx, sb, need))) return rc;
+        if ((rc = meme_buf_reserve(ctx, ob, (size_t)n_todo * sizeof(i64)))) return rc;
+        HIP_TRY(hipMemsetAsync(counters, 0, SEED_CTRS * sizeof(unsigned long long), stream));
+    }
     SeedArgs A;
     A.I = ctx->idx;
     A.packed = (const u64*)ctx->batch.packed.p;
@@ -266,23 +277,26 @@
     A.tier = tier;
     A.counters = counters;
     A.defer = defer ? 1 : 0;
+    A.carry = rnd == SEED_ALL ? nullptr : (u64*)ctx->seed.carry.p;
+    A.r3cap = (rnd == SEED_R3 && SEED_R3_CAP && R.opt->min_seed_len + 1 <= 32) ? 1 : 0;
     R.tiers.base[tier] = (const SlotRec*)sb.p;
     R.tiers.cap[tier] = cap;
-    while (G < 32 && seed_lds_bytes(G, R.geo, lcap) > (size_t)160 * 1024) G *= 2;
+    const bool r3 = rnd == SEED_R3;
+    while (G < 32 && seed_lds_bytes(G, R.geo, lcap, r3) > (size_t)160 * 1024) G *= 2;
     const int groups = BLOCK / G;
-    size_t lds = seed_lds_bytes(G, R.geo, lcap);
+    size_t lds = seed_lds_bytes(G, R.geo, lcap, r3);
     i64 want = (n_todo + groups - 1) / groups;
     i64 blocks = ctx->seed_blocks > 0 ? ctx->seed_blocks : (i64)ctx->n_cus * ctx->seed_blocks_per_cu;
     if (blocks > want) blocks = want;
     if (blocks < 1) blocks = 1;
-    if (tier == 0) HIP_TRY(hipEventRecord(ctx->seed.ev[SEED_EV_SEARCH0], stream));
+    if (tier == 0 && rnd != SEED_R3) HIP_TRY(hipEventRecord(ctx->seed.ev[SEED_EV_SEARCH0], stream));
     switch (G) {
-    case 1: return launch_k_seed<1>(stream, A, lds, blocks);
-    case 2: return launch_k_seed<2>(stream, A, lds, blocks);
-    case 4: return launch_k_seed<4>(stream, A, lds, blocks);
-    case 8: return launch_k_seed<8>(stream, A, lds, blocks);
-    case 16: return launch_k_seed<16>(stream, A, lds, blocks);
-    case 32: return launch_k_seed<32>(stream, A, lds, blocks);
+    case 1: return launch_k_seed<1>(stream, A, lds, blocks, rnd);
+    case 2: return launch_k_seed<2>(stream, A, lds, blocks, rnd);
+    case 4: return launch_k_seed<4>(stream, A, lds, blocks, rnd);
+    case 8: return launch_k_seed<8>(stream, A, lds, blocks, rnd);
+    case 16: return launch_k_seed<16>(stream, A, lds, blocks, rnd);
+    case 32: return launch_k_seed<32>(stream, A, lds, blocks, rnd);
     default: meme_set_error("group_lanes must be 1, 2, 4, 8, 16 or 32"); return MEME_E_ARG;
     }
 }
@@ -383,7 +397,12 @@
     S.reseed_rounds = 0;
     if (R.defer && (rc = meme_buf_reserve(ctx, S.pend, (size_t)R.nreads * sizeof(i64)))) return rc;
     if (R.defer && (rc = meme_buf_reserve(ctx, S.blk, (size_t)R.nreads * BLK_PER_READ * 2 * sizeof(BlkRec)))) return rc;
-    if ((rc = launch_tier(R, 0, R.nreads, nullptr, 0, ctx->stream, R.defer))) return rc;
+    R.split = ctx->seed_r3_split != 0 && R.opt->rounds >= 3 && R.opt->max_mem_intv > 0;
+    if (R.split) {
+        if ((rc = meme_buf_reserve(ctx, S.carry, (size_t)R.nreads * sizeof(u64)))) return rc;
+        if ((rc = launch_tier(R, 0, R.nreads, nullptr, 0, ctx->stream, R.defer, SEED_R12))) return rc;
+        if ((rc = launch_tier(R, 0, R.nreads, nullptr, 0, ctx->stream, R.defer, SEED_R3))) return rc;
+    } else if ((rc = launch_tier(R, 0, R.nreads, nullptr, 0, ctx->stream, R.defer))) return rc;
     if (R.defer) {
         if ((rc = meme_side_stream(ctx, 0)) || (rc = launch_reseed(R)) || (rc = launch_early_overflow(R))) return rc;
         HIP_TRY(hipStreamWaitEvent(ctx->stream, S.emit_ev[1], 0));
@@ -415,6 +434,8 @@
         if (getenv("MEME_SEED_TRACE")) fprintf(stderr, "[meme] seed tier 0: search kernel + re-seeding kernels %.2f ms, of which behind k_seed %.2f ms (%lld lane searches; %lld reads of the "
                                                "overflow tier beside them)\n", ms, a, (long long)h[SEED_CTR_LANE], (long long)(R.n_early < 0 ? 0 : R.n_early));
     }
+    S.r3_counts[0] = R.split ? 1 : 0;
+    S.r3_counts[1] = (long long)h[SEED_CTR_R3_REPEAT];
     tally(R, h);
     return MEME_OK;
 }
@@ -511,6 +532,7 @@
     ctx->tm.seed_windows = R.windows;
     ctx->tm.seed_reseed_ms = R.ms_reseed;
     ctx->tm.seed_lane_searches = R.lane_searches;
+    S.r3_valid = true;
     return seed_gather(R, out);
 }
 
@@ -631,6 +653,15 @@
     return MEME_OK;
 }
 
+extern "C" int meme_debug_seed_r3_counts(meme_ctx* ctx, int64_t* out, int32_t capacity) {
+    if (!ctx || !out) return MEME_E_ARG;
+    const SeedWs& S = ctx->seed;
+    if (!S.r3_valid) { meme_set_error("meme_debug_seed_r3_counts: no seeding call on this ctx yet"); return MEME_E_STATE; }
+    if (capacity < MEME_R3_COUNTS) { meme_set_error("meme_debug_seed_r3_counts: %d values needed", MEME_R3_COUNTS); return MEME_E_CAPACITY; }
+    for (int k = 0; k < MEME_R3_COUNTS; ++k) out[k] = S.r3_counts[k];
+    return MEME_OK;
+}
+
 extern "C" int meme_seed_reserve(meme_ctx* ctx, int64_t nreads, int64_t total_bases) {
     if (!ctx || nreads < 0 || total_bases < 0) return MEME_E_ARG;
     if (nreads == 0) return MEME_OK;
@@ -643,7 +674,7 @@
     ChainWs& C = ctx->chain; ExtWs& E = ctx->ext;
     struct { DevBuf* b; size_t bytes; } dev[] = {
         {&B.reads, (size_t)total_bases + 16}, {&B.read_off, (n + 1) * 8}, {&S.slot_cnt, n * 4}, {&S.slot_hits, n * 8},
-        {&S.slot_loc, n * 8}, {&S.counters, 2 * SEED_CTRS * 8}, {&S.pend, n * 8}, {&S.blk, n * BLK_PER_READ * 2 * sizeof(BlkRec)}, {&B.packed, n * stride * 8}, {&S.slots[0], n * (size_t)ctx->smem_cap * sizeof(SlotRec)},
+        {&S.slot_loc, n * 8}, {&S.carry, n * 8}, {&S.counters, 2 * SEED_CTRS * 8}, {&S.pend, n * 8}, {&S.blk, n * BLK_PER_READ * 2 * sizeof(BlkRec)}, {&B.packed, n * stride * 8}, {&S.slots[0], n * (size_t)ctx->smem_cap * sizeof(SlotRec)},
         {&B.smem_off, (n + 1) * 8}, {&B.hit_off, (n + 1) * 8}, {&B.smems, n * 12 * sizeof(meme_mem_tl)}, {&B.hits, n * 24 * 8},
         {&C.chains, n * 3 * sizeof(meme_chain)}, {&C.seeds, n * 6 * sizeof(meme_chain_seed)}};
     for (auto& d : dev) if ((rc = meme_buf_reserve(ctx, *d.b, d.bytes))) return rc;
diff --git a/bwa-meme_amd/csrc/meme_seed_kernel.h b/bwa-meme_amd/csrc/meme_seed_kernel.h
--- a/bwa-meme_amd/csrc/meme_seed_kernel.h
+++ b/bwa-meme_amd/csrc/meme_seed_kernel.h
@@ -49,7 +49,14 @@
     int cap, lcap, tier;
     unsigned long long* counters;
     int defer;
+    u64* carry;
+    int r3cap;
 };
+enum SeedRounds : int { SEED_ALL = 0, SEED_R12 = 1, SEED_R3 = 2 };
+#ifndef SEED_R3_CAP
+#define SEED_R3_CAP 1
+#endif
+constexpr u64 CARRY_OVF = ~0ull;
 
 constexpr int PACK_CAP = 5120;
 constexpr int PACK_IT = PACK_CAP / (64 * 16);
@@ -238,13 +245,13 @@
 
 constexpr int TICKET_CHUNK = 32;
 
-__host__ __device__ inline size_t seed_lds_group_bytes(int G, int stride, int lcap) {
+__host__ __device__ inline size_t seed_lds_group_bytes(int G, int qwords, int lcap) {
     const int groups = BLOCK / G;
     const int W = win_entries(G) * G;
-    return (((size_t)groups * (SEED_QUERY_LDS ? stride * 8 : 0) + (size_t)groups * (2 * lcap + ST_WORDS + (W + 1) / 2) * sizeof(int)) + 7) & ~(size_t)7;
-}
-inline size_t seed_lds_bytes(int G, const PackGeom& geo, int lcap) {
-    return seed_lds_group_bytes(G, geo.stride, lcap) + (size_t)(BLOCK / 64) * 16;
+    return (((size_t)groups * (SEED_QUERY_LDS ? qwords * 8 : 0) + (size_t)groups * (2 * lcap + ST_WORDS + (W + 1) / 2) * sizeof(int)) + 7) & ~(size_t)7;
+}
+inline size_t seed_lds_bytes(int G, const PackGeom& geo, int lcap, bool r3 = false) {
+    return seed_lds_group_bytes(G, r3 ? geo.W + geo.MW : geo.stride, r3 ? 0 : lcap) + (size_t)(BLOCK / 64) * 16;
 }
 
 template <int E>
@@ -362,7 +369,7 @@
     }
 }
 
-template <int G>
+template <int G, int RND = SEED_ALL>
 #ifndef SEED_MIN_WAVES
 #define SEED_MIN_WAVES 5
 #endif
@@ -378,23 +385,24 @@
     const int t = threadIdx.x & (G - 1);
     const int gbase = lane & ~(G - 1);
     const int stride = A.geo.stride, PW = A.geo.W, MW = A.geo.MW;
-    const int cap = A.cap, lcap = A.lcap;
+    const int cap = A.cap, lcap = RND == SEED_R3 ? 0 : A.lcap;
+    const int qwords = RND == SEED_R3 ? PW + MW : stride;
 #if SEED_QUERY_LDS
-    u64* rd = reinterpret_cast<u64*>(smem_raw) + (size_t)gib * stride;
+    u64* rd = reinterpret_cast<u64*>(smem_raw) + (size_t)gib * qwords;
     const q_u64 fw = (lds_u64)rd;
 #else
     q_u64 fw = (q_u64)A.packed;
 #endif
 #define rcs (fw + PW)
-#define nfw (fw + 2 * PW)
+#define nfw (fw + ((RND == SEED_R3 && SEED_QUERY_LDS) ? PW : 2 * PW))
 #define nrc (fw + 2 * PW + MW)
-    const lds_int ring = (lds_int)(reinterpret_cast<int*>(smem_raw + (SEED_QUERY_LDS ? (size_t)GROUPS * stride * 8 : 0)) +
+    const lds_int ring = (lds_int)(reinterpret_cast<int*>(smem_raw + (SEED_QUERY_LDS ? (size_t)GROUPS * qwords * 8 : 0)) +
                                    (size_t)gib * (2 * lcap + ST_WORDS + (W + 1) / 2));
     const lds_int sm_se = ring;
     const lds_int sm_cnt = ring + lcap;
     const lds_int st = ring + 2 * lcap;
     const lds_u16 wl = (lds_u16)(st + ST_WORDS);
-    const lds_int wv = (lds_int)(reinterpret_cast<int*>(smem_raw + seed_lds_group_bytes(G, stride, lcap)) + (threadIdx.x >> 6) * 4);
+    const lds_int wv = (lds_int)(reinterpret_cast<int*>(smem_raw + seed_lds_group_bytes(G, qwords, lcap)) + (threadIdx.x >> 6) * 4);
     const glb_ent sa = (glb_ent)A.I.sa;
     const glb_u64 pac = (glb_u64)A.I.pac;
     const glb_rmi l2 = (glb_rmi)A.I.l2, l1 = (glb_rmi)A.I.l1;
@@ -411,8 +419,10 @@
     int pc = PC_FETCH, phase = PH_CTRL;
     int pivot = 0, l_seq = 0, msl = A.opt.min_seed_len, min_intv = 1;
     bool has_n = false;
-    int q_kind = 0, q_mode = 0, off = 0, vlen = 0, capc = 0;
+    int q_kind = RND == SEED_R3 ? K_R3 : 0, q_mode = RND == SEED_R3 ? 2 : 0, off = 0, vlen = 0, capc = 0;
     bool q_rc = false, q_exact = false;
+    bool capped = false, redo = false, r3full = false;
+    unsigned acc_repeats = 0;
     i64 base = 0, lo = -1, hi = n;
     int stepk = 0;
     u64 wq = 0;
@@ -433,6 +443,7 @@
             bool have = false;
 #define AT(pc_) (!have && pc == (pc_))
             do {
+              if constexpr (RND != SEED_R3) {
                 if (AT(PC_ZZ_TOP)) {
                     if (st[ST_ZZ_SP] >= st[ST_ZZ_NEXT] || ++st[ST_ZZ_GUARD] > 4 * l_seq + 16) pc = PC_ZZ_END;
                     else if (FLAG(F_ZZ_CHECK) && has_n && is_n(nfw, st[ST_ZZ_SP])) {
@@ -483,7 +494,7 @@
                     }
                 }
                 if (AT(PC_ALLPOS_TOP)) {
-                    if (pivot >= l_seq || ++st[ST_AP_GUARD] > 4 * l_seq + 16) pc = PC_R3_INIT;
+                    if (pivot >= l_seq || ++st[ST_AP_GUARD] > 4 * l_seq + 16) pc = RND == SEED_R12 ? PC_DONE : PC_R3_INIT;
                     else {
                         st[ST_BEFORE] = st[ST_N_SMEMS]; st[ST_SM_BASE] = st[ST_BEFORE]; SETFLAG(F_REC, true);
                         if (has_n && is_n(nfw, pivot)) {
@@ -495,8 +506,10 @@
                         } else { q_kind = K_S1_RIGHT; have = true; }
                     }
                 }
+              }
+              if constexpr (RND != SEED_R12) {
                 if (AT(PC_R3_INIT)) {
-                    if (A.opt.rounds >= 3 && A.opt.max_mem_intv > 0 && !FLAG(F_LDS_OVF)) {
+                    if (RND == SEED_R3 || (A.opt.rounds >= 3 && A.opt.max_mem_intv > 0 && !FLAG(F_LDS_OVF))) {
                         min_intv = A.opt.max_mem_intv;
                         msl = A.opt.min_seed_len + 1;
                         pivot = 0;
@@ -513,17 +526,20 @@
                         break;
                     }
                 }
+              }
                 if (AT(PC_DONE)) {
                     const unsigned long long ticket = ((unsigned long long)(unsigned)st[ST_TICKET_HI] << 32) | (unsigned)st[ST_TICKET_LO];
-                    const bool ovf = st[ST_N_SMEMS] > cap || FLAG(F_LDS_OVF);
+                    const bool ovf = st[ST_N_SMEMS] > cap || (RND != SEED_R3 && FLAG(F_LDS_OVF));
                     if (t == 0) {
                         const i64 rid = A.pending ? A.pending[ticket] : (i64)ticket;
                         A.slot_cnt[rid] = ovf ? 0 : st[ST_N_SMEMS];
                         A.slot_hits[rid] = ovf ? 0 : LD64(ST_HITS_LO);
-                        A.slot_loc[rid] = ((i64)A.tier << 40) | (i64)ticket;
+                        if constexpr (RND != SEED_R3) A.slot_loc[rid] = ((i64)A.tier << 40) | (i64)ticket;
+                        if constexpr (RND == SEED_R12) A.carry[rid] = ovf ? CARRY_OVF : ((u64)(unsigned)st[ST_SEARCHES] | ((u64)(unsigned)st[ST_WINDOWS] << 32));
                         if (ovf) A.ovf_list[atomicAdd(&A.counters[SEED_CTR_OVERFLOW], 1ull)] = rid;
                     }
-                    if (!ovf) { acc_searches += (unsigned)st[ST_SEARCHES]; acc_windows += (unsigned)st[ST_WINDOWS]; }
+                    if constexpr (RND != SEED_R12)
+                        if (!ovf) { acc_searches += (unsigned)st[ST_SEARCHES]; acc_windows += (unsigned)st[ST_WINDOWS]; }
                     pc = PC_FETCH;
                 }
                 if (AT(PC_FETCH)) {
@@ -538,7 +554,7 @@
                         const int kreq = __popcll(mo), alloc = kreq > TICKET_CHUNK ? kreq : TICKET_CHUNK;
                         unsigned long long nb = 0;
                         if (lane == first) {
-                            nb = atomicAdd(&A.counters[SEED_CTR_SLOT], (unsigned long long)alloc);
+                            nb = atomicAdd(&A.counters[RND == SEED_R3 ? SEED_CTR_SLOT3 : SEED_CTR_SLOT], (unsigned long long)alloc);
                             const unsigned long long wb = nb + (unsigned)(alloc - TICKET_CHUNK);
                             wv[0] = kreq - (alloc - TICKET_CHUNK); wv[2] = (int)(unsigned)(wb & 0xffffffffull); wv[3] = (int)(wb >> 32);
                         }
@@ -550,15 +566,29 @@
                     else {
                         const i64 rid = A.pending ? A.pending[ticket] : (i64)ticket;
                         const u64* src = A.packed + rid * stride;
+                        u64 carry = 0;
+                        int c0 = 0;
+                        i64 h0 = 0;
+                        if constexpr (RND == SEED_R3) { carry = A.carry[rid]; c0 = A.slot_cnt[rid]; h0 = A.slot_hits[rid]; }
 #if SEED_QUERY_LDS
-                        const int lw = (stride - 1) % G;
                         u64 lenw = 0;
-                        for (int k = t; k < stride; k += G) {
-                            u64 v = src[k];
-                            rd[k] = v;
-                            if (k == stride - 1) lenw = v;
+                        if constexpr (RND == SEED_R3) {
+                            const int lw = qwords % G;
+                            for (int j = t; j <= qwords; j += G) {
+                                const int k = j < PW ? j : (j < qwords ? j + PW : stride - 1);
+                                u64 v = src[k];
+                                if (j < qwords) rd[j] = v; else lenw = v;
+                            }
+                            lenw = (u64)(unsigned)__shfl((int)lenw, gbase + lw);
+                        } else {
+                            const int lw = (stride - 1) % G;
+                            for (int k = t; k < stride; k += G) {
+                                u64 v = src[k];
+                                rd[k] = v;
+                                if (k == stride - 1) lenw = v;
+                            }
+                            lenw = (u64)(unsigned)__shfl((int)lenw, gbase + lw);
                         }
-                        lenw = (u64)(unsigned)__shfl((int)lenw, gbase + lw);
 #else
                         fw = (q_u64)src;
                         const u64 lenw = fw[stride - 1];
@@ -568,15 +598,24 @@
                         for (int k = t; k < ST_WORDS; k += G) st[k] = 0;
                         LDS_HANDOFF();
                         if (l_seq <= 0 || l_seq > MAX_READ_LEN) {
-                            if (t == 0) { A.slot_cnt[rid] = l_seq > MAX_READ_LEN ? -1 : 0; A.slot_hits[rid] = 0; A.slot_loc[rid] = 0; }
+                            if constexpr (RND != SEED_R3)
+                                if (t == 0) { A.slot_cnt[rid] = l_seq > MAX_READ_LEN ? -1 : 0; A.slot_hits[rid] = 0; A.slot_loc[rid] = 0; }
+                        } else if (RND == SEED_R3 && carry == CARRY_OVF) {
                         } else {
                             st[ST_TICKET_LO] = (int)(unsigned)(ticket & 0xffffffffull);
                             st[ST_TICKET_HI] = (int)(ticket >> 32);
-                            pivot = 0; msl = A.opt.min_seed_len; min_intv = 1;
-                            pc = PC_ALLPOS_TOP;
-                            if (!(has_n && is_n(nfw, 0))) {
-                                st[ST_AP_GUARD] = 1; SETFLAG(F_REC, true);
-                                q_kind = K_S1_RIGHT; have = true;
+                            if constexpr (RND == SEED_R3) {
+                                st[ST_N_SMEMS] = c0; ST64(ST_HITS_LO, h0);
+                                st[ST_SEARCHES] = (int)(unsigned)(carry & 0xffffffffull); st[ST_WINDOWS] = (int)(unsigned)(carry >> 32);
+                                r3full = false;
+                                pc = PC_R3_INIT;
+                            } else {
+                                pivot = 0; msl = A.opt.min_seed_len; min_intv = 1;
+                                pc = PC_ALLPOS_TOP;
+                                if (!(has_n && is_n(nfw, 0))) {
+                                    st[ST_AP_GUARD] = 1; SETFLAG(F_REC, true);
+                                    q_kind = K_S1_RIGHT; have = true;
+                                }
                             }
                         }
                     }
@@ -585,7 +624,8 @@
 #undef AT
             if (pc == PC_EXIT) {
                 if (t == 0) {
-                    atomicAdd(&A.counters[SEED_CTR_SEARCHES], (unsigned long long)acc_searches); atomicAdd(&A.counters[SEED_CTR_WINDOWS], (unsigned long long)acc_windows);
+                    if constexpr (RND != SEED_R12) { atomicAdd(&A.counters[SEED_CTR_SEARCHES], (unsigned long long)acc_searches); atomicAdd(&A.counters[SEED_CTR_WINDOWS], (unsigned long long)acc_windows); }
+                    if constexpr (RND == SEED_R3) if (acc_repeats) atomicAdd(&A.counters[SEED_CTR_R3_REPEAT], (unsigned long long)acc_repeats);
 #ifdef SEED_PROF
                     for (int k = 0; k < 8; ++k) atomicAdd(&A.counters[SEED_CTR_PROF + k], (unsigned long long)prof[k]);
 #endif
@@ -595,14 +635,21 @@
             newreq = true;
         }
         PROF_MARK(0);
-        if (newreq) {
-            q_rc = q_kind == K_ZZ_LEFT;
-            off = q_rc ? l_seq - 1 - pivot : pivot;
-            vlen = first_n(q_rc ? nrc : nfw, has_n, off, l_seq) - off;
-            q_exact = q_kind == K_S1_RIGHT || q_kind == K_ZZ_RIGHT || q_kind == K_OP_SMEM;
-            q_mode = q_kind == K_R3 ? 2 : ((q_exact || min_intv != 1) ? 1 : 0);
-            st[ST_SEARCHES] = st[ST_SEARCHES] + 1;
-            wq = ext_l(q_rc ? rcs : fw, off);
+        if (newreq || (RND == SEED_R3 && redo)) {
+            if constexpr (RND == SEED_R3) {
+                off = pivot;
+                vlen = first_n(nfw, has_n, off, l_seq) - off;
+                if (redo) ++acc_repeats; else st[ST_SEARCHES] = st[ST_SEARCHES] + 1;
+                wq = ext_l(fw, off);
+            } else {
+                q_rc = q_kind == K_ZZ_LEFT;
+                off = q_rc ? l_seq - 1 - pivot : pivot;
+                vlen = first_n(q_rc ? nrc : nfw, has_n, off, l_seq) - off;
+                q_exact = q_kind == K_S1_RIGHT || q_kind == K_ZZ_RIGHT || q_kind == K_OP_SMEM;
+                q_mode = (RND == SEED_ALL && q_kind == K_R3) ? 2 : ((q_exact || min_intv != 1) ? 1 : 0);
+                st[ST_SEARCHES] = st[ST_SEARCHES] + 1;
+                wq = ext_l(q_rc ? rcs : fw, off);
+            }
             u64 key = wq;
             if (vlen < 32) key |= (~0ull) >> (2 * vlen);
             u64 err;
@@ -620,11 +667,20 @@
             if (base < 0) base = 0;
             if (base > n - W) base = n - W;
             lo = -1; hi = n; stepk = 0; capc = vlen;
+            if constexpr (RND == SEED_R3) {
+                if (redo) r3full = true;
+                capped = A.r3cap != 0 && !r3full && vlen > 32;
+                if (capped) capc = 32;
+                redo = false;
+            }
             phase = PH_PART;
         }
+        const bool exact = RND != SEED_R3 && q_exact;
+        const bool kind_r3 = RND == SEED_R3 || (RND == SEED_ALL && q_kind == K_R3);
+        const bool mode2 = RND == SEED_R3 || (RND == SEED_ALL && q_mode == 2);
         PROF_MARK(1);
 
-        const q_u64 s = q_rc ? rcs : fw;
+        const q_u64 s = (RND != SEED_R3 && q_rc) ? rcs : fw;
         int lcp[E];
         bool less[E];
         u64 ep[E];
@@ -666,13 +722,13 @@
                 const int c = (lm >= lp) ? P - 1 : P;
                 L = lm >= lp ? lm : lp;
                 r_L = L; r_start = base + c; r_count = 1;
-                if (q_exact || q_kind == K_R3) {
+                if (exact || kind_r3) {
                     u64 tc = 0;
 #pragma unroll
                     for (int e = 0; e < E; ++e) tc = (e * G + t == c) ? ep[e] : tc;
                     r_T = (i64)(((u64)(unsigned)group_or<G>((int)(tc >> 32)) << 32) | (u64)(unsigned)group_or<G>((int)(unsigned)tc));
                 }
-                if (q_mode == 0 || (q_mode == 2 && L < msl)) finished = true;
+                if ((RND != SEED_R3 && q_mode == 0) || (mode2 && L < msl)) finished = true;
                 else {
                     s_edge = e_edge = base + c;
                     lf = LF_NEED_LO | LF_NEED_HI;
@@ -688,7 +744,7 @@
         } else {
             if (P == W) lo = base + W - 1; else hi = base;
             bool stop = false;
-            if (phase != PH_PART && !q_exact) {
+            if (phase != PH_PART && !exact) {
                 s_edge = LD64(ST_SE_LO); e_edge = LD64(ST_EE_LO);
                 if (phase == PH_EDGE_DN ? (e_edge - hi + 1 >= (i64)min_intv) : (lo - s_edge + 1 >= (i64)min_intv)) {
                     L = st[ST_L]; nb_lo = st[ST_NB_LO]; nb_hi = st[ST_NB_HI]; lf = st[ST_LF]; cb = LD64(ST_CB_LO);
@@ -748,10 +804,12 @@
                 }
                 const i64 cnt = e_edge - s_edge + 1;
                 const int nxt = nb_lo > nb_hi ? nb_lo : nb_hi;
-                if (q_mode == 1) {
+                if (!mode2) {
                     if (cnt >= (i64)min_intv) { r_L = L; r_start = s_edge; r_count = cnt; finished = true; break; }
                 } else {
                     if (cnt >= (i64)min_intv) {
+                        if constexpr (RND == SEED_R3)
+                            if (capped && L >= 32) { redo = true; break; }
                         if (lf & LF_HAVE_LAST) { r_count = LD64(ST_LAST_CNT_LO); r_start = LD64(ST_LAST_S_LO); }
                         else { r_count = cnt; r_start = s_edge; }
                         r_L = L + 1;
@@ -767,11 +825,11 @@
                 lf = (lf & LF_HAVE_LAST) | ((nb_lo >= L && s_edge > 0) ? LF_NEED_LO : 0) | ((nb_hi >= L && e_edge < n - 1) ? LF_NEED_HI : 0);
             }
             if (finished) {
-                if (q_mode == 2) {
+                if (mode2) {
                     r_emit = r_count < (i64)min_intv;
                     if (r_L < msl) r_L = msl;
                 }
-            } else {
+            } else if (!(RND == SEED_R3 && redo)) {
                 capc = L;
                 st[ST_L] = L; st[ST_NB_LO] = nb_lo; st[ST_NB_HI] = nb_hi; st[ST_LF] = lf;
                 ST64(ST_SE_LO, s_edge); ST64(ST_EE_LO, e_edge); ST64(ST_CB_LO, cb);
@@ -786,7 +844,8 @@
             bool emit = false;
             const int e_start = pivot;
             int e_end = pivot;
-            switch (q_kind) {
+            if constexpr (RND == SEED_R3) { emit = r_emit; e_end = pivot + r_L; }
+            else switch (q_kind) {
             case K_S1_RIGHT:
             case K_ZZ_RIGHT:
             case K_OP_SMEM:
@@ -801,13 +860,13 @@
                 pc = PC_ZZ_TOP;
                 break;
             default:
-                emit = r_emit; e_end = pivot + r_L;
+                if constexpr (RND == SEED_ALL) { emit = r_emit; e_end = pivot + r_L; }
                 break;
             }
             if (emit) {
                 const int ns = st[ST_N_SMEMS];
                 const bool have_pos = r_count == 1 && r_T >= 0 && !cache_in_lds;
-                const bool defer = have_pos && A.defer != 0 && FLAG(F_REC) && ns < DEFER_MAX_K && ns < cap && A.opt.rounds >= 2 &&
+                const bool defer = RND != SEED_R3 && have_pos && A.defer != 0 && FLAG(F_REC) && ns < DEFER_MAX_K && ns < cap && A.opt.rounds >= 2 &&
                                    e_end - e_start >= A.opt.split_len && A.opt.split_width >= 1 && nb_lo < msl && nb_hi < msl;
                 if (ns < cap && t == 0) {
                     const unsigned long long ticket = ((unsigned long long)(unsigned)st[ST_TICKET_HI] << 32) | (unsigned)st[ST_TICKET_LO];
@@ -816,7 +875,7 @@
                     sr.sa_start = have_pos ? (SLOT_POS | (defer ? SLOT_DEFER : 0ll) | r_T) : r_start;
                     A.slots[(i64)ticket * cap + ns] = sr;
                 }
-                if (FLAG(F_REC)) {
+                if constexpr (RND != SEED_R3) if (FLAG(F_REC)) {
                     const int k = ns - st[ST_SM_BASE];
                     if (k < lcap) {
                         sm_se[k] = e_start | (e_end << 16);
@@ -829,11 +888,12 @@
                 h += LD64(ST_HITS_LO);
                 ST64(ST_HITS_LO, h);
             }
-            switch (q_kind) {
+            if constexpr (RND == SEED_R3) { pivot = pivot + (r_L < msl ? msl : r_L); pc = PC_R3_TOP; }
+            else switch (q_kind) {
             case K_S1_RIGHT: pivot = pivot + r_L; pc = PC_AFTER_STEP1; break;
             case K_ZZ_RIGHT: pivot = pivot + r_L; st[ST_ZZ_SP] = pivot; pc = PC_ZZ_TOP; break;
             case K_OP_SMEM: pivot = pivot + r_L; pc = PC_R2_AFTER; break;
-            case K_R3: pivot = pivot + (r_L < msl ? msl : r_L); pc = PC_R3_TOP; break;
+            case K_R3: if constexpr (RND == SEED_ALL) { pivot = pivot + (r_L < msl ? msl : r_L); pc = PC_R3_TOP; } break;
             default: break;
             }
             phase = PH_CTRL;
diff --git a/bwa-meme_amd/pymeme/hipapi.py b/bwa-meme_amd/pymeme/hipapi.py
--- a/bwa-meme_amd/pymeme/hipapi.py
+++ b/bwa-meme_amd/pymeme/hipapi.py
@@ -221,7 +221,7 @@
            "meme_host_free", "meme_stage_pack_text", "meme_stage_pos5_from_sa", "meme_stage_build_entries", "meme_stage_build_plcp",
            "meme_stage_entries_from_sa", "meme_stage_rmi32", "meme_sa_build_device", "meme_prmi_train_device", "meme_seed_batch", "meme_seed_batch_host", "meme_seed_batch_resident", "meme_seed_batch_resident_ascii", "meme_seed_reserve", "meme_chain_last_batch_host", "meme_chain_batch_host", "meme_extend_last_batch_host", "meme_global_batch_host", "meme_gen_cigar_batch_host", "meme_sam_stage_text", "meme_sam_format_batch_host", "meme_kswv_batch_host", "meme_matesw_batch_host", "meme_primary_batch_host", "meme_primary_batch_device", "meme_finish_batch_host", "meme_finish_batch_device", "meme_pair_batch_host", "meme_pair_batch_device", "meme_seed_batch_device",
            "meme_bsw_batch", "meme_bsw_batch_device", "meme_get_timings", "meme_set_tuning", "meme_debug_packed_reads",
-           "meme_debug_reseed_counts", "meme_debug_sa_stats", "meme_debug_scan_exclusive"]
+           "meme_debug_reseed_counts", "meme_debug_seed_r3_counts", "meme_debug_sa_stats", "meme_debug_scan_exclusive"]
 
 RESEED_MAX_ROUNDS = 8
 RESEED_COUNTS = RESEED_MAX_ROUNDS + 6
@@ -415,6 +415,11 @@
         return {"rounds": [int(v) for v in out[:rounds.value]], "stage": [int(v) for v in out[st:st + 3]], "no_interval": int(out[st + 3]),
                 "walked": int(out[st + 4]), "neighbour_probes": int(out[st + 5])}
 
+    def debug_seed_r3_counts(self):
+        out = np.zeros(2, dtype=np.int64)
+        _check(lib().meme_debug_seed_r3_counts(C.c_void_p(self.h), _p(out), C.c_int32(out.size)))
+        return {"split": bool(out[0]), "repeats": int(out[1])}
+
     def debug_sa_stats(self):
         out = np.zeros(len(SA_STATS), dtype=np.int64)
         _check(lib().meme_debug_sa_stats(C.c_void_p(self.h), _p(out), C.c_int32(out.size)))
diff --git a/include/meme_hip.h b/include/meme_hip.h
--- a/include/meme_hip.h
+++ b/include/meme_hip.h
@@ -303,6 +303,9 @@
 #define MEME_RESEED_COUNTS 14
 int meme_debug_reseed_counts(meme_ctx* ctx, int64_t* out, int32_t capacity, int32_t* rounds);
 
+#define MEME_R3_COUNTS 2
+int meme_debug_seed_r3_counts(meme_ctx* ctx, int64_t* out, int32_t capacity);
+
 #define MEME_SA_STATS 7
 int meme_debug_sa_stats(meme_ctx* ctx, int64_t* out, int32_t capacity);
 
```

Result: faster. 163.6 million reads/s (median of 6 runs) (+3.4%).
